# mjq11302010044/TATT

Measured on AMD Instinct MI355X. Metric: LR images/s (train fwd+bwd+clip+Adam) at 16x64->32x128, higher is better.
Workload: dtype fp32 (split-bf16 MFMA operands in conv3 / conv3-wgrad / conv9 / tokgemm / gru-wgrad / query-GRU recurrence and dW_hh / TP-layer backward)

## Files before the change

include/tatt_hip.h:

```cpp
#ifndef TATT_HIP_H
#define TATT_HIP_H

#ifdef __cplusplus
extern "C" {
#endif

typedef struct ihipStream_t* hipStream_t;


int tatt_gemm(const float* A, long sam, long sak, const float* A2, long sa2m, long sa2k, int K1,
              const float* B, long sbk, long sbn, const float* bias, float* C, long scm, long scn,
              int M, int N, int K, int Z, long bsA, long bsA2, long bsB, long bsC, long bsBias,
              float alpha, float beta, int act, int splitk, float* ws, float* rowsum, hipStream_t st);

int tatt_conv2d_fwd(const float* x, long xsn, long xsh, long xsw, long xsc, const float* wpacked,
                    const float* bias, float* y, long ldy, int Bn, int H, int W, int Cin, int Cout,
                    int KH, int KW, int act, float beta, int splitk, float* ws, hipStream_t st);

int tatt_conv2d_fwd_partials(const float* x, long xsn, long xsh, long xsw, long xsc, const float* wpacked, int Bn, int H,
                             int W, int Cin, int Cout, int KH, int KW, int splitk, float* ws, int* splits, hipStream_t st);

int tatt_conv2d_wgrad(const float* x, long xsn, long xsh, long xsw, long xsc, const float* dy,
                      long lddy, float* dw_oihw, int Bn, int H, int W, int Cin, int Cout, int KH,
                      int KW, float beta, int splitk, float* ws, hipStream_t st);

int tatt_repack_conv_weight(const float* w_oihw, float* out, int Cout, int Cin, int KH, int KW,
                            int mode, hipStream_t st);
int tatt_repack_words(int Cout, int Cin, int KH, int KW, int mode);
int tatt_repack_conv_weight_batch(const float* const* ws, float* const* outs, const int* dims, int n, hipStream_t st);

int tatt_gru_wgrad_sb(const float* dgi, const float* dgh, const float* x, const float* xb, const float* hprev,
                      float* ws1, float* ws2, int M, int G, hipStream_t st);

int tatt_splitk_reduce(const float* partial, float* C, int M, int N, int S, int remap_cin, int remap_taps,
                       float beta, float* vec, int vec_len, hipStream_t st);
int tatt_reduce_defer(int on, hipStream_t st);
int tatt_reduce_flush(hipStream_t st);

int tatt_conv3_c64_fwd_t(const float* x, const float* wt, const float* bias, float* y, int B, int H, int W, int Cin,
                         int Cout, int act, float beta, hipStream_t st);
int tatt_conv3_c64_fwd_ws16(const float* x, const float* wl, const float* bias, float* y, int B, int H, int W,
                            int Cout, int act, float beta, hipStream_t st);
int tatt_conv3_c64_fwd_ws16_bn(const float* x, const float* wl, const float* bias, float* y, int B, int H, int W,
                               int Cout, int act, float beta, const float* in_scale, const float* in_shift, int in_act,
                               double* stats, hipStream_t st);
int tatt_conv3_c64_fwd_sb(const float* x, int cin_total, int ci0, const float* wl, const float* bias, float* y, int B, int H,
                          int W, int Cout, int act, float beta, const float* in_scale, const float* in_shift, int in_act,
                          double* stats, hipStream_t st);
int tatt_conv3_c64_dgrad_bn_sb(const float* x, const float* x2, const float* in_scale, const float* in_scale2,
                               const float* in_shift, const float* wl, float* y, int B, int H, int W, const float* ep_x,
                               const float* ep_mean, const float* ep_rstd, const float* ep_gamma, const float* ep_beta,
                               int ep_act, double* stats, hipStream_t st);
int tatt_conv3_sb_generation(int gen);
int tatt_conv3_sb_packing(int B, int H, int W, int cin_total, int Cout, int act, int ep_act);
int tatt_conv3_sb_route(int B, int H, int W, int cin_total, int Cout, int act, int ep_act);
int tatt_conv3_c64_wgrad_partial(const float* x, const float* dy, float* part, float* pdb, int B, int H, int W,
                                 int Cin, int Cout, int G, hipStream_t st);
int tatt_conv3_c64_wgrad_partial_sb(const float* x, const float* dy, float* part, float* pdb, int B, int H, int W,
                                    int Cin, int Cout, int G, hipStream_t st);
int tatt_conv3_wgrad_sb_generation(int gen);
int tatt_conv3_wgrad_sb_route(int B, int H, int W, int Cin, int Cout);

int tatt_conv9_c64_to_c4(const float* x, const float* wpacked, const float* bias, float* y, int B, int H, int W,
                         int C, hipStream_t st);
int tatt_conv9_c64_to_c4_mfma(const float* x, const float* wt, const float* bias, float* y, int B, int H, int W,
                              hipStream_t st);
int tatt_conv9_c64_to_c4_sb(const float* x, const float* wt, const float* bias, float* y, int B, int H, int W,
                            hipStream_t st);
int tatt_conv9_c4_to_c64(const float* in, const float* wp, const float* bias, float* out, int B, int H, int W, int act,
                         hipStream_t st);
int tatt_conv9_c4_to_c64_sb(const float* in, const float* wp, const float* bias, float* out, int B, int H, int W, int act,
                            hipStream_t st);
int tatt_conv9_c64_c4_wgrad(const float* x, const float* dy, float* dw, float* part, int B, int H, int W,
                            hipStream_t st);
int tatt_conv9_c4_c64_wgrad(const float* x, const float* dy, float* dw, float* part, int B, int H, int W,
                            hipStream_t st);
int tatt_conv9_c64_c4_wgrad_sb(const float* x, const float* dy, float* dw, float* part, int B, int H, int W,
                               hipStream_t st);
int tatt_conv9_c4_c64_wgrad_sb(const float* x, const float* dy, float* dw, float* part, int B, int H, int W,
                               hipStream_t st);


int tatt_colsum(const float* X, long ld, int M, int C, float* out, float scale, float beta,
                double* ws, hipStream_t st);

int tatt_bn_stats(const float* X, long ld, int M, int C, float eps, float momentum, float* mean,
                  float* rstd, float* running_mean, float* running_var, double* ws, hipStream_t st);
int tatt_bn_stats_finish(const double* part, int G, int C, int M, float eps, float momentum, const float* gamma,
                         const float* beta, float* mean, float* rstd, float* running_mean, float* running_var, float* scale,
                         float* shift, hipStream_t st);
int tatt_bn_rstd(const float* var, float* rstd, int C, float eps, hipStream_t st);
int tatt_bn_apply(const float* X, long ldx, float* Y, long ldy, int M, int C, const float* mean,
                  const float* rstd, const float* gamma, const float* beta, int act, hipStream_t st);
int tatt_bn_bwd(const float* X, long ldx, const float* dY, long lddy, float* dX, long lddx, int M, int C,
                const float* mean, const float* rstd, const float* gamma, const float* beta, int act,
                int training, float* dgamma, float* dbeta, float* sums, double* ws, hipStream_t st);
int tatt_bn_bwd_groups(int M);
int tatt_bn_bwd_partials(const float* X, long ldx, const float* dY, long lddy, int M, int C, const float* mean,
                         const float* rstd, const float* gamma, const float* beta, int act, double* part, hipStream_t st);
int tatt_bn_bwd_finish(const double* part, int G, int C, int M, const float* mean, const float* rstd, const float* gamma,
                       float* dgamma, float* dbeta, float* coef, hipStream_t st);
int tatt_bn_bwd_affine(const float* X, const float* dU, float* dX, int M, int C, const float* coef, hipStream_t st);

int tatt_ln_fwd(const float* A, const float* Bres, float* Y, float* stats, int M, int C,
                const float* gamma, const float* beta, float eps, int mode, float pdrop,
                const unsigned long long* seed, unsigned site, hipStream_t st);
int tatt_ln_bwd(const float* A, const float* Bres, const float* dY, const float* stats, float* dX, float* dB, int M,
                int C, const float* gamma, float* dgamma, float* dbeta, float* part, double* ws, float eps, int mode,
                float pdrop, const unsigned long long* seed, unsigned site, hipStream_t st);


int tatt_prelu_fwd(const float* x, float* y, const float* alpha, long n, hipStream_t st);
int tatt_prelu_bwd(const float* x, const float* dy, float* dx, const float* alpha, long n, float* part,
                   hipStream_t st);
int tatt_act_fwd(const float* x, float* y, long n, int act, hipStream_t st);
int tatt_act_bwd(const float* ref, const float* dy, float* dx, long n, int act, int from_output,
                 hipStream_t st);
int tatt_axpby(const float* a, const float* b, float* y, float alpha, float beta, long n, hipStream_t st);
int tatt_add_n(const float* const* srcs, int n, float* y, long numel, hipStream_t st);
int tatt_add_rowbcast(const float* a, const float* b, float* y, long rows, int C, long period,
                      hipStream_t st);
int tatt_pixel_shuffle_fwd(const float* in, float* out, int B, int H, int W, int C, int act,
                           hipStream_t st);
int tatt_pixel_shuffle_bwd(const float* in, const float* dout, float* din, int B, int H, int W, int C,
                           int act, hipStream_t st);
int tatt_maxpool_fwd(const float* in, float* out, int B, int H, int W, int C, int kh, int kw, int sh, int sw,
                     int ph, int pw, hipStream_t st);
int tatt_maxpool_bwd(const float* in, const float* dout, float* din, int B, int H, int W, int C, int kh,
                     int kw, int sh, int sw, int ph, int pw, hipStream_t st);
int tatt_dropout(const float* x, float* y, long n, float p, const unsigned long long* seed, unsigned site,
                 hipStream_t st);
int tatt_bump_seed(unsigned long long* seed, unsigned long long* snap, hipStream_t st);
int tatt_stamp(unsigned long long* out, hipStream_t st);
int tatt_copy4d(const float* src, float* dst, int n0, int n1, int n2, int n3, long s0, long s1, long s2,
                long s3, long d0, long d1, long d2, long d3, float beta, hipStream_t st);


int tatt_l2norm(const float* g, long n, float* out, double* ws, hipStream_t st);
int tatt_adam_step(float* p, const float* g, float* m, float* v, long n, float lr, float b1, float b2,
                   float eps, const float* gnorm, float max_norm, float gscale, const long long* step,
                   hipStream_t st);


int tatt_gru32_fwd(const float* gi, const float* whh_f, const float* bhh_f, const float* whh_r,
                   const float* bhh_r, float* out, float* gates, int nseq, int T, int s_in, long stride_hi,
                   long stride_lo, long stride_t, hipStream_t st);
int tatt_gru32_bwd(const float* gates, const float* out, const float* dout, const float* whh_f,
                   const float* whh_r, float* dgi, float* dgh, float* hprev, int nseq, int T, int s_in,
                   long stride_hi, long stride_lo, long stride_t, hipStream_t st);

int tatt_gru32_fwd2(const float* gi, const float* whh_f, const float* bhh_f, const float* whh_r,
                    const float* bhh_r, float* out, float* gates, int nseq, int T, int s_in, long stride_hi,
                    long stride_lo, long stride_t, hipStream_t st);
int tatt_gru32_bwd2(const float* gates, const float* out, const float* dout, const float* whh_f,
                    const float* whh_r, float* dgi, float* dgh, float* hprev, float* frag, int nseq, int T, int s_in,
                    long stride_hi, long stride_lo, long stride_t, hipStream_t st);
int tatt_gru_wgrad_frag(const float* frag, const float* x, const float* xb, float* ws1, float* ws2, int nseq, int T,
                        int s_in, long stride_hi, long stride_lo, long stride_t, int G, hipStream_t st);
int tatt_gru_wgrad_frag_in(const float* frag, const float* x, const float* xb, float* ws1, float* ws2, int nseq, int T,
                           int s_in, long stride_hi, long stride_lo, long stride_t, int G, const float* in_mean,
                           const float* in_rstd, const float* in_gamma, const float* in_beta, const float* in_add,
                           hipStream_t st);

int tatt_qgru_bwd_fused(const float* dgh_cur0, const float* dgh_cur1, const float* whhT0, const float* whhT1,
                        const float* dhseq_next0, const float* dhseq_next1, const float* gsave_next0,
                        const float* gsave_next1, const float* hprev_next0, const float* hprev_next1,
                        float* dhcarry0, float* dhcarry1, float* dgi_acc0, float* dgi_acc1, float* dgh_next0,
                        float* dgh_next1, int Wb, int HID, hipStream_t st);

int tatt_gru_compose(const float* wih_f, const float* wih_r, const float* bih_f, const float* bih_r,
                     const float* Wc, const float* bc, float* Wp, float* bp, int K, hipStream_t st);
int tatt_gru_compose_batch(const float* const* ptrs, const int* Ks, int n, hipStream_t st);
int tatt_gru_tail(const float* dWp, const float* dbp, const float* Wc, const float* bc, const float* wih_f,
                  const float* wih_r, float* dwih_f, float* dwih_r, float* dWc, float* dbc, int K,
                  const float* dWhh, float* dwhh_f, float* dwhh_r, hipStream_t st);

int tatt_gru_tail_c(const float* dWp, const float* dbp, const float* Wc, const float* bc, const float* wih_f,
                    const float* wih_r, float* dwih_f, float* dwih_r, float* dWc, float* dbc, int K,
                    const float* dWhh_c, float* dwhh_f, float* dwhh_r, hipStream_t st);

int tatt_qgru_fwd_step(const float* gi0, const float* gi1, const float* whh0, const float* whh1,
                       const float* bhh0, const float* bhh1, const float* hprev0, const float* hprev1,
                       float* hnew0, float* hnew1, float* gsave0, float* gsave1, int Wb, int HID,
                       hipStream_t st);
// ... 290 lines not shown
```

tatt_amd/csrc/conv3.hip:

```cpp
#include "common.h"
#include <mutex>
#include <stdlib.h>
#include <type_traits>

#define C3_PX 64
#define C3_HW 66

struct Conv3P {
    const float* x; const float* w; const float* bias; float* y;
    int B, H, W, Cin, Cout, act;
    float beta;
    const float* in_scale; const float* in_shift; int in_act;
    double* stats;
};
template <int CK>
struct C5 {
    static constexpr int XP = CK + 4;
    static constexpr int HALO = 3 * C3_HW * XP;
    static constexpr int WT = 64 * XP;
    static constexpr int LDS = (2 * HALO + 2 * WT) * 4;
    static constexpr int Q4 = CK / 4;
    static constexpr int SLICE = 22 * Q4;
    static constexpr int WF4 = 64 * Q4;
};
template <int CK>
__global__ __launch_bounds__(256, (CK == 64 ? 1 : (CK == 32 ? 2 : 3))) void conv3_c64_fwd_v5_kernel(Conv3P p) {
    constexpr int C5_XP = C5<CK>::XP, C5_HALO = C5<CK>::HALO, C5_WT = C5<CK>::WT, Q4 = C5<CK>::Q4;
    constexpr int SLICE = C5<CK>::SLICE, WF4 = C5<CK>::WF4, QS = (CK == 64 ? 4 : 5);
    constexpr int Q4S = (CK == 64 ? 4 : (CK == 32 ? 3 : 2));
    (void)QS;
    extern __shared__ __attribute__((aligned(16))) float smem[];
    float* XsB = smem;
    float* WsB = smem + 2 * C5_HALO;
    const int t = threadIdx.x, lane = t & 63, wave = t >> 6;
    const int wm = wave & 1, wn = wave >> 1;
    const int segs = p.W / C3_PX, cob = p.Cout / 64, nch = p.Cin / CK;
    const int ntiles = p.B * p.H * segs * cob;
    const int G = gridDim.x;
    auto decode = [&](int tile, int& n, int& h, int& w0, int& co0) {
        int bid = tile;
        const int cb = bid % cob; bid /= cob;
        const int seg = bid % segs; bid /= segs;
        h = bid % p.H; n = bid / p.H;
        w0 = seg * C3_PX; co0 = cb * 64;
    };
    auto halo_load = [&](int n, int hh, int w0, int ci0, int pxb, int idx) -> f32x4 {
        const int ww = w0 + pxb + (idx >> Q4S) - 1;
        f32x4 v = (f32x4){0.f, 0.f, 0.f, 0.f};
        if (hh >= 0 && hh < p.H && ww >= 0 && ww < p.W)
            v = *reinterpret_cast<const f32x4*>(p.x + (((long)n * p.H + hh) * p.W + ww) * p.Cin + ci0 + 4 * (idx & (Q4 - 1)));
        return v;
    };
    auto halo_store = [&](float* Xs, int r, int pxb, int idx, f32x4 v) {
        *reinterpret_cast<f32x4*>(Xs + (r * C3_HW + pxb + (idx >> Q4S)) * C5_XP + 4 * (idx & (Q4 - 1))) = v;
    };
    constexpr int WQ = WF4 / 256;
    f32x4 wreg[WQ];
    auto load_w = [&](int tap, int ci0, int co0) {
        const float* src = p.w + ((long)tap * p.Cout + co0) * p.Cin + ci0;
#pragma unroll
        for (int q = 0; q < WQ; ++q) {
            const int idx = t + 256 * q;
            wreg[q] = *reinterpret_cast<const f32x4*>(src + (long)(idx >> Q4S) * p.Cin + 4 * (idx & (Q4 - 1)));
        }
    };
    auto store_w = [&](float* Ws) {
#pragma unroll
        for (int q = 0; q < WQ; ++q) {
            const int idx = t + 256 * q;
            *reinterpret_cast<f32x4*>(Ws + (idx >> Q4S) * C5_XP + 4 * (idx & (Q4 - 1))) = wreg[q];
        }
    };
    int tile = blockIdx.x;
    if (tile >= ntiles) return;
    int n, h, w0, co0;
    decode(tile, n, h, w0, co0);
    for (int s9 = 0; s9 < 9; ++s9) {
        const int r = s9 / 3, pxb = (s9 - 3 * r) * 22;
        for (int i = t; i < SLICE; i += 256) halo_store(XsB, r, pxb, i, halo_load(n, h + r - 1, w0, 0, pxb, i));
    }
    load_w(0, 0, co0);
    store_w(WsB);
    __syncthreads();
// ... 637 lines not shown
        unsigned nnorg, nnte;
        decode(pt + 2 * stride, nnorg, nnte);
#pragma unroll
        for (int st = 0; st < 18; ++st) {
            if (st + 1 < 18) { S3_LD(st + 1) }
            if (FIRST && st % 2 == 0 && st / 2 + 3 < 9) w_issue(st / 2 + 3);
            __builtin_amdgcn_sched_barrier(0);
            const bf16x8 wh = __builtin_bit_cast(bf16x8, wq[2 * st]), wl = __builtin_bit_cast(bf16x8, wq[2 * st + 1]);
            const bf16x8 b0h = __builtin_bit_cast(bf16x8, vb[st % 2][0]), b0l = __builtin_bit_cast(bf16x8, vb[st % 2][1]);
            const bf16x8 b1h = __builtin_bit_cast(bf16x8, vb[st % 2][2]), b1l = __builtin_bit_cast(bf16x8, vb[st % 2][3]);
            accM[0] = __builtin_amdgcn_mfma_f32_32x32x16_bf16(wh, b0h, accM[0], 0, 0, 0);
            accM[1] = __builtin_amdgcn_mfma_f32_32x32x16_bf16(wh, b1h, accM[1], 0, 0, 0);
            accC[0] = __builtin_amdgcn_mfma_f32_32x32x16_bf16(wl, b0h, accC[0], 0, 0, 0);
            accC[1] = __builtin_amdgcn_mfma_f32_32x32x16_bf16(wl, b1h, accC[1], 0, 0, 0);
            accC[0] = __builtin_amdgcn_mfma_f32_32x32x16_bf16(wh, b0l, accC[0], 0, 0, 0);
            accC[1] = __builtin_amdgcn_mfma_f32_32x32x16_bf16(wh, b1l, accC[1], 0, 0, 0);
            if (st % 2 == 1 && st / 2 < S3_NIT) {
                halo_put(imgN, nte, st / 2);
                halo_issue1(nnorg, nnte, had_next && pt + 2 * stride < npt, st / 2);
                S3_INTERLEAVE(INMODE == 1 ? 14 : 8)
            }
            if (st % 4 == 2 && st / 4 < S3_NEP) { epilogue(epi_pending, st / 4); S3_INTERLEAVE(8) }
            if (st % 4 == 0 && st > 0 && st / 4 - 1 < S3_NEP) epi_request(org, st / 4 - 1);
            __builtin_amdgcn_sched_barrier(0);
        }
#if S2_STAMP
        { const unsigned long long now = __builtin_amdgcn_s_memtime();
          if (tix == 0) ts[3] = now; else if (tix == 1) ts[6] = now; else if (tix == 2) ts[9] = now; }
#endif
        has_next = had_next && pt + 2 * stride < npt;
        {
            unsigned* xw = XCH + xbuf * S2_XCH + (kh * 64 + lj) * S2_XP + 32 * coh + 4 * kb;
#pragma unroll
            for (int pp = 0; pp < 2; ++pp)
#pragma unroll
                for (int g = 0; g < 4; ++g) {
                    f32x4 v;
#pragma unroll
                    for (int r = 0; r < 4; ++r) v[r] = accM[pp][4 * g + r] + accC[pp][4 * g + r];
                    *reinterpret_cast<f32x4*>(xw + 32 * pp * S2_XP + 8 * g) = v;
                }
        }
        eorg = org; ebuf = xbuf; epi_pending = true;
#if S2_STAMP
        { const unsigned long long now = __builtin_amdgcn_s_memtime();
          if (tix == 0) ts[4] = now; else if (tix == 1) ts[7] = now; else if (tix == 2) ts[10] = now; }
        ++tix;
#endif
        __syncthreads();
        if (had_next) { pt += stride; org = norg; te = nte; norg = nnorg; nte = nnte; xbuf ^= 1; }
    };
    tile_body(std::true_type{});
    while (had_next) tile_body(std::false_type{});
    S2_STAMP_AT(11)
#pragma unroll
    for (int e = 0; e < S3_NEP; ++e) epilogue(true, e);
    S2_STAMP_AT(12)
#if S2_STAMP
    ts[31] = wall_clock64();
    if (lane == 0 && sbuf) {
#pragma unroll
        for (int i = 0; i < 32; ++i) sbuf[(blockIdx.x * 8 + wave) * 32 + i] = ts[i];
    }
#endif
    if (p.stats) {
#pragma unroll
        for (int r = 0; r < 4; ++r) {
            st_s[r] += __shfl_xor(st_s[r], 16, 64); st_s[r] += __shfl_xor(st_s[r], 32, 64);
            st_q[r] += __shfl_xor(st_q[r], 16, 64); st_q[r] += __shfl_xor(st_q[r], 32, 64);
        }
        if (lane < 16) {
#pragma unroll
            for (int r = 0; r < 4; ++r) { st_red[wave][0][ec4 + r] = st_s[r]; st_red[wave][1][ec4 + r] = st_q[r]; }
        }
        __syncthreads();
        if (t < 128) {
            double a = 0.0;
#pragma unroll
            for (int w = 0; w < 4; ++w) a += (double)st_red[w][t >> 6][t & 63];
            p.stats[(long)blockIdx.x * 128 + t] = a;
        }
    }
}
template <int INMODE, bool EPBN>
__global__ __launch_bounds__(512, 2) void conv3_c64_sb4_kernel(Conv3SB q) {
    const Conv3P& p = q.c;
    extern __shared__ __attribute__((aligned(16))) unsigned smem_u[];
    unsigned* const XCH = smem_u + 4 * S3_IMG;
    const unsigned t = threadIdx.x, lane = t & 63, wave = t >> 6;
    const unsigned W = p.W, H = p.H, tws = (W + 15) / 16, ths = H / 4, cob = p.Cout / 64;
    const unsigned npt = p.B * ths * tws;
    const unsigned stride = gridDim.x / cob;
    unsigned cb = blockIdx.x % cob, pt = blockIdx.x / cob;
    if (gridDim.x % 8 == 0 && 8 % cob == 0 && stride % (8 / cob) == 0) {
        const unsigned x = blockIdx.x & 7, m = blockIdx.x >> 3, xg = 8 / cob;
        cb = x % cob;
        pt = (x / cob) * (stride / xg) + m;
    }
    __shared__ float st_red[4][2][64];
    __shared__ __attribute__((aligned(16))) float cst[7][64];
    __shared__ __attribute__((aligned(16))) float cbias[64];
    if (pt >= npt) {
        if (p.stats && t < 128) p.stats[(long)blockIdx.x * 128 + t] = 0.0;
        return;
    }
    const unsigned ntile = (npt - pt + stride - 1) / stride;
    auto decode = [&](unsigned tile, unsigned& org, unsigned& te) {
        const unsigned tw = tile % tws; tile /= tws;
        const unsigned th = tile % ths, n = tile / ths;
        org = (n * H + th * 4) * W + tw * 16;
        const unsigned cin = min(18u, W - tw * 16 + 1);
        te = (th == 0 ? 1u : 0u) | (th == ths - 1 ? 2u : 0u) | (tw == 0 ? 4u : 0u) | (cin << 8);
    };
    if (wave >= 4) {
        const unsigned h = t - 256;
        const unsigned npix = p.B * H * W;
        const __amdgpu_buffer_rsrc_t rs_x = __builtin_amdgcn_make_buffer_rsrc(const_cast<float*>(p.x), 0, npix * q.cin_total * 4, 0x00020000);
        const __amdgpu_buffer_rsrc_t rs_x2 = __builtin_amdgcn_make_buffer_rsrc(const_cast<float*>(INMODE == 2 ? q.x2 : p.x), 0, npix * 256, 0x00020000);
        const __amdgpu_buffer_rsrc_t rs_y = __builtin_amdgcn_make_buffer_rsrc(p.y, 0, npix * p.Cout * 4, 0x00020000);
        const __amdgpu_buffer_rsrc_t rs_e = __builtin_amdgcn_make_buffer_rsrc(const_cast<float*>(EPBN ? q.ep_x : p.y), 0, npix * (EPBN ? 64 : p.Cout) * 4, 0x00020000);
        const bool in_relu = p.in_act == ACT_RELU;
        const unsigned xps = q.cin_total * 4, yps = p.Cout * 4, eps_ = EPBN ? 256u : yps;
        unsigned boff[S3_NIT], poff[S3_NIT], edge[2] = {0, 0}, colk[2] = {0, 0};
#pragma unroll
        for (int k = 0; k < S3_NIT; ++k) {
            const unsigned pix = (h >> 4) + 16 * k, r = pix / S2_HW, c = pix - r * S2_HW;
            boff[k] = (unsigned)(((int)r - 1) * (int)W + (int)c - 1) * xps + (q.ci0 + 4 * (h & 15)) * 4;
            poff[k] = r * S3_RP + c * SB_PW + 2 * (h & 15);
            edge[k >> 2] |= ((r == 0 ? 1u : 0u) | (r == 5 ? 2u : 0u) | (c == 0 ? 4u : 0u) | (pix >= S2_NPX ? 8u : 0u)) << (8 * (k & 3));
            colk[k >> 2] |= c << (8 * (k & 3));
        }
        auto outside = [&](int k, unsigned te) -> bool {
            return (((edge[k >> 2] >> (8 * (k & 3))) & (te | 8u) & 15u) != 0) || (((colk[k >> 2] >> (8 * (k & 3))) & 255u) >= (te >> 8));
        };
        f32x4 hp[S3_NIT], hp2[S3_NIT];
        auto halo_issue = [&](unsigned tile, bool valid) {
            unsigned org, te;
            decode(tile, org, te);
#if S2_DEBUG
            if (s2_wrep & 4) valid = false;
#endif
#pragma unroll
            for (int k = 0; k < S3_NIT; ++k) {
                const unsigned a = (org * xps + boff[k]) | (outside(k, te) ? S2_OOB : (valid ? 0u : S2_OOB));
                hp[k] = s2_ld(rs_x, a);
                if (INMODE == 2) hp2[k] = s2_ld(rs_x2, a);
            }
        };
        auto halo_put = [&](unsigned* img, unsigned tile) {
            unsigned org, te;
            decode(tile, org, te);
            f32x4 isc, ish, isc2;
            if (INMODE != 0) { isc = *reinterpret_cast<const f32x4*>(&cst[0][4 * (h & 15)]); ish = *reinterpret_cast<const f32x4*>(&cst[1][4 * (h & 15)]); }
            if (INMODE == 2) isc2 = *reinterpret_cast<const f32x4*>(&cst[2][4 * (h & 15)]);
#pragma unroll
            for (int k = 0; k < S3_NIT; ++k) {
                const bool ok = !outside(k, te);
                f32x4 v = hp[k];
                if (INMODE == 2) {
#pragma unroll
                    for (int e = 0; e < 4; ++e) v[e] = fmaf(v[e], isc[e], fmaf(hp2[k][e], isc2[e], ish[e]));
                } else if (INMODE == 1) {
#pragma unroll
                    for (int e = 0; e < 4; ++e) v[e] = mish_f(fmaf(v[e], isc[e], ish[e]));
                } else if (INMODE == 3) {
#pragma unroll
                    for (int e = 0; e < 4; ++e) {
                        const float u = fmaf(v[e], isc[e], ish[e]);
                        v[e] = in_relu ? fmaxf(u, 0.f) : u;
                    }
                }
                if (INMODE != 0) {
#pragma unroll
                    for (int e = 0; e < 4; ++e) v[e] = ok ? v[e] : 0.f;
                }
                if (k < S3_NIT - 1 || h < S2_NPX * 16 - 256 * (S3_NIT - 1)) {
                    uint2 hi, lo;
                    sb_split(v, hi, lo);
                    unsigned* d = img + poff[k];
                    *reinterpret_cast<uint2*>(d) = hi;
                    *reinterpret_cast<uint2*>(d + S3_IMG) = lo;
                }
            }
        };
        halo_issue(pt, true);
// ... 6 lines not shown
        __syncthreads();
        halo_put(smem_u, pt);
        halo_issue(pt + stride, ntile > 1);
        __syncthreads();
        const bool use_beta = p.beta != 0.f, out_relu = p.act == ACT_RELU;
        const bool ep_mish = q.ep_act == ACT_MISH, ep_relu = q.ep_act == ACT_RELU;
        const unsigned ecol = h >> 4, ec4 = 4 * (h & 15);
        f32x4 epx[S3_NEP], st_s = (f32x4){0.f, 0.f, 0.f, 0.f}, st_q = st_s;
        auto epi_request = [&](unsigned tile) {
            unsigned org, te;
            decode(tile, org, te);
            const bool in_map = ecol + 1 < (te >> 8);
#pragma unroll
            for (int e = 0; e < S3_NEP; ++e)
                epx[e] = s2_ld(rs_e, ((org + e * W + ecol) * eps_ + (cb * 64 + ec4) * 4) | (((EPBN || use_beta) && in_map) ? 0u : S2_OOB));
        };
        auto epilogue = [&](unsigned tile, unsigned xb) {
            unsigned org, te;
            decode(tile, org, te);
            const f32x4 bj = *reinterpret_cast<const f32x4*>(&cbias[ec4]);
            const bool in_map = ecol + 1 < (te >> 8);
            f32x4 ep_mu, ep_rs, ep_g, ep_b;
            if (EPBN) {
                ep_mu = *reinterpret_cast<const f32x4*>(&cst[3][ec4]); ep_rs = *reinterpret_cast<const f32x4*>(&cst[4][ec4]);
                ep_g = *reinterpret_cast<const f32x4*>(&cst[5][ec4]); ep_b = *reinterpret_cast<const f32x4*>(&cst[6][ec4]);
            }
#pragma unroll
            for (int e = 0; e < S3_NEP; ++e) {
                const unsigned* X = XCH + xb * S2_XCH + ((h >> 4) + 16 * e) * S2_XP + ec4;
                const f32x4 v0 = *reinterpret_cast<const f32x4*>(X), v1 = *reinterpret_cast<const f32x4*>(X + 64 * S2_XP);
                f32x4 v;
#pragma unroll
                for (int r = 0; r < 4; ++r) {
                    v[r] = (v0[r] + v1[r]) + bj[r];
                    if (EPBN) {
                        const float xh = (epx[e][r] - ep_mu[r]) * ep_rs[r], u = fmaf(ep_g[r], xh, ep_b[r]);
                        const float g = ep_mish ? mish_grad_f(u) : 1.f;
                        v[r] *= ep_relu ? (u > 0.f ? 1.f : 0.f) : g;
                        v[r] = in_map ? v[r] : 0.f;
                        st_s[r] += v[r]; st_q[r] += v[r] * xh;
                    } else {
                        v[r] = fmaf(p.beta, epx[e][r], v[r]);
                        v[r] = out_relu ? fmaxf(v[r], 0.f) : v[r];
                        v[r] = in_map ? v[r] : 0.f;
                        st_s[r] += v[r]; st_q[r] += v[r] * v[r];
                    }
                }
#if S2_DEBUG
                if (s2_wrep & 8) continue;
#endif
                __builtin_amdgcn_raw_buffer_store_b128(__builtin_bit_cast(u32x4_s2, v), rs_y, ((org + e * W + ecol) * yps + (cb * 64 + ec4) * 4) | (in_map ? 0u : S2_OOB), 0, 0);
            }
        };
        for (unsigned i = 0; i < ntile; ++i) {
            const unsigned tile = pt + i * stride;
#if S2_DEBUG
            if (s2_wrep & 1) { __syncthreads(); continue; }
#endif
#if S2_DEBUG
            if (!(s2_wrep & 32))
#endif
            if (i > 0) epilogue(tile - stride, (i - 1) & 1);
#if S2_DEBUG
            if (!(s2_wrep & 16))
#endif
            if (i + 1 < ntile) halo_put(smem_u + ((i + 1) & 1) * 2 * S3_IMG, tile + stride);
            halo_issue(tile + 2 * stride, i + 2 < ntile);
            epi_request(tile);
            __syncthreads();
        }
        epilogue(pt + (ntile - 1) * stride, (ntile - 1) & 1);
        if (p.stats) {
#pragma unroll
            for (int r = 0; r < 4; ++r) {
                st_s[r] += __shfl_xor(st_s[r], 16, 64); st_s[r] += __shfl_xor(st_s[r], 32, 64);
                st_q[r] += __shfl_xor(st_q[r], 16, 64); st_q[r] += __shfl_xor(st_q[r], 32, 64);
            }
            if (lane < 16) {
#pragma unroll
                for (int r = 0; r < 4; ++r) { st_red[wave - 4][0][ec4 + r] = st_s[r]; st_red[wave - 4][1][ec4 + r] = st_q[r]; }
            }
        }
        __syncthreads();
        if (p.stats && h < 128) {
            double a = 0.0;
#pragma unroll
            for (int w = 0; w < 4; ++w) a += (double)st_red[w][h >> 6][h & 63];
            p.stats[(long)blockIdx.x * 128 + h] = a;
        }
        return;
    }
    const unsigned coh = wave & 1, kh = wave >> 1, lj = lane & 31, kb = lane >> 5;
    f32x4 wq[36];
    {
        const f32x4* const wsrc = reinterpret_cast<const f32x4*>(p.w) + (cb * 2 + coh) * 72 * 64 + lane;
#pragma unroll
        for (int tap = 0; tap < 9; ++tap)
#pragma unroll
            for (int f = 0; f < 4; ++f) wq[4 * tap + f] = wsrc[((tap * 2 + kh) * 4 + f) * 64];
    }
    const unsigned bbase = (lj >> 4) * S3_RP + (lj & 15) * SB_PW + 16 * kh + 4 * kb;
    __syncthreads();
    __syncthreads();
    for (unsigned i = 0; i < ntile; ++i) {
#if S2_DEBUG
        if (s2_wrep & 2) { __syncthreads(); continue; }
#endif
        const unsigned* Xs = smem_u + (i & 1) * 2 * S3_IMG + bbase;
        f32x16_s3 acc[2];
#pragma unroll
        for (int pp = 0; pp < 2; ++pp)
#pragma unroll
            for (int v = 0; v < 16; ++v) acc[pp][v] = 0.f;
        f32x4 vb[2][4];
        S3_LD(0)
#pragma unroll
        for (int st = 0; st < 18; ++st) {
            if (st + 1 < 18) { S3_LD(st + 1) }
            __builtin_amdgcn_sched_barrier(0);
            const bf16x8 wh = __builtin_bit_cast(bf16x8, wq[2 * st]), wl = __builtin_bit_cast(bf16x8, wq[2 * st + 1]);
            const bf16x8 b0h = __builtin_bit_cast(bf16x8, vb[st % 2][0]), b0l = __builtin_bit_cast(bf16x8, vb[st % 2][1]);
            const bf16x8 b1h = __builtin_bit_cast(bf16x8, vb[st % 2][2]), b1l = __builtin_bit_cast(bf16x8, vb[st % 2][3]);
            acc[0] = __builtin_amdgcn_mfma_f32_32x32x16_bf16(wh, b0h, acc[0], 0, 0, 0);
            acc[1] = __builtin_amdgcn_mfma_f32_32x32x16_bf16(wh, b1h, acc[1], 0, 0, 0);
            acc[0] = __builtin_amdgcn_mfma_f32_32x32x16_bf16(wl, b0h, acc[0], 0, 0, 0);
            acc[1] = __builtin_amdgcn_mfma_f32_32x32x16_bf16(wl, b1h, acc[1], 0, 0, 0);
            acc[0] = __builtin_amdgcn_mfma_f32_32x32x16_bf16(wh, b0l, acc[0], 0, 0, 0);
            acc[1] = __builtin_amdgcn_mfma_f32_32x32x16_bf16(wh, b1l, acc[1], 0, 0, 0);
            __builtin_amdgcn_sched_barrier(0);
        }
        unsigned* xw = XCH + (i & 1) * S2_XCH + (kh * 64 + lj) * S2_XP + 32 * coh + 4 * kb;
#pragma unroll
        for (int pp = 0; pp < 2; ++pp)
#pragma unroll
            for (int g = 0; g < 4; ++g) {
                f32x4 v;
#pragma unroll
                for (int r = 0; r < 4; ++r) v[r] = acc[pp][4 * g + r];
                *reinterpret_cast<f32x4*>(xw + 32 * pp * S2_XP + 8 * g) = v;
            }
        __syncthreads();
    }
    __syncthreads();
}
static int conv3_sb_generation = 4;
TATT_API int tatt_conv3_sb_generation(int gen) {
    const int old = conv3_sb_generation;
    if (gen == 1 || gen == 3 || gen == 4) conv3_sb_generation = gen;
    return old;
}
template <int INMODE, bool EPBN>
static void conv3_sb4_go(const Conv3SB& q, dim3 grid, hipStream_t st) {
    static TattPerDevice attr_once;
    tatt_per_device(attr_once, [&] {
        (void)hipFuncSetAttribute(reinterpret_cast<const void*>(conv3_c64_sb4_kernel<INMODE, EPBN>), hipFuncAttributeMaxDynamicSharedMemorySize, S3_LDS);
    });
    hipLaunchKernelGGL((conv3_c64_sb4_kernel<INMODE, EPBN>), grid, dim3(512), S3_LDS, st, q);
}
template <int INMODE, bool EPBN>
static void conv3_sb3_go(const Conv3SB& q, dim3 grid, hipStream_t st) {
    static TattPerDevice attr_once;
    tatt_per_device(attr_once, [&] {
        (void)hipFuncSetAttribute(reinterpret_cast<const void*>(conv3_c64_sb3_kernel<INMODE, EPBN>), hipFuncAttributeMaxDynamicSharedMemorySize, S3_LDS);
    });
    hipLaunchKernelGGL((conv3_c64_sb3_kernel<INMODE, EPBN>), grid, dim3(256), S3_LDS, st, q);
}
static int conv3_sb_pick(int B, int H, int W, int cin_total, int Cout, int act, int ep_act) {
    const long maxb = (long)B * H * W * (cin_total > Cout ? cin_total : Cout) * 4;
    if (conv3_sb_generation < 3 || H % 4 || maxb >= 0x7fffffffL || ep_act == ACT_TANH) return 1;
    if (conv3_sb_generation == 4 && (act == ACT_NONE || (act == ACT_RELU && ep_act == ACT_NONE))) return 4;
    return (conv3_sb_generation == 3 && W % 16 == 0 && act == ACT_NONE) ? 3 : 1;
}
TATT_API int tatt_conv3_sb_packing(int B, int H, int W, int cin_total, int Cout, int act, int ep_act) {
    return conv3_sb_pick(B, H, W, cin_total, Cout, act, ep_act) >= 3 ? 14 : 10;
}
TATT_API int tatt_conv3_sb_route(int B, int H, int W, int cin_total, int Cout, int act, int ep_act) {
    const int pick = conv3_sb_pick(B, H, W, cin_total, Cout, act, ep_act);
    return pick == 1 && W % C3_PX ? 0 : pick;
}
static int conv3_sb_launch(const Conv3SB& q, hipStream_t st) {
    const Conv3P& p = q.c;
    const int pick = conv3_sb_pick(p.B, p.H, p.W, q.cin_total, p.Cout, p.act, q.ep_act);
    if (pick >= 3) {
        const int cob = p.Cout / 64, npt = p.B * (p.H / 4) * ((p.W + 15) / 16);
        int per = 256 / cob;
        if (per > npt) per = npt;
        const dim3 grid(per * cob);
        const bool ep = q.ep_x != nullptr;
        const int inmode = q.x2 ? 2 : (p.in_scale ? (p.in_act == ACT_MISH ? 1 : 3) : 0);
        if (pick == 4) {
            if (inmode == 2) { if (ep) conv3_sb4_go<2, true>(q, grid, st); else conv3_sb4_go<2, false>(q, grid, st); }
            else if (inmode == 1) { if (ep) conv3_sb4_go<1, true>(q, grid, st); else conv3_sb4_go<1, false>(q, grid, st); }
            else if (inmode == 3) { if (ep) conv3_sb4_go<3, true>(q, grid, st); else conv3_sb4_go<3, false>(q, grid, st); }
            else { if (ep) conv3_sb4_go<0, true>(q, grid, st); else conv3_sb4_go<0, false>(q, grid, st); }
            return LAUNCH_CHECK();
        }
        if (pick == 3) {
            if (inmode == 2) { if (ep) conv3_sb3_go<2, true>(q, grid, st); else conv3_sb3_go<2, false>(q, grid, st); }
            else if (inmode == 1) { if (ep) conv3_sb3_go<1, true>(q, grid, st); else conv3_sb3_go<1, false>(q, grid, st); }
            else if (inmode == 3) { if (ep) conv3_sb3_go<3, true>(q, grid, st); else conv3_sb3_go<3, false>(q, grid, st); }
            else { if (ep) conv3_sb3_go<0, true>(q, grid, st); else conv3_sb3_go<0, false>(q, grid, st); }
            return LAUNCH_CHECK();
        }
        return LAUNCH_CHECK();
    }
    if (p.W % C3_PX) return 1;
    static TattPerDevice attr_once;
    tatt_per_device(attr_once, [&] {
        (void)hipFuncSetAttribute(reinterpret_cast<const void*>(conv3_c64_sb_kernel<false, false>), hipFuncAttributeMaxDynamicSharedMemorySize, SB_LDS);
        (void)hipFuncSetAttribute(reinterpret_cast<const void*>(conv3_c64_sb_kernel<true, false>), hipFuncAttributeMaxDynamicSharedMemorySize, SB_LDS);
        (void)hipFuncSetAttribute(reinterpret_cast<const void*>(conv3_c64_sb_kernel<false, true>), hipFuncAttributeMaxDynamicSharedMemorySize, SB_LDS);
        (void)hipFuncSetAttribute(reinterpret_cast<const void*>(conv3_c64_sb_kernel<true, true>), hipFuncAttributeMaxDynamicSharedMemorySize, SB_LDS);
    });
    const int cob = p.Cout / 64, npt = p.B * p.H * (p.W / C3_PX);
    int per = 256 / cob;
    if (per > npt) per = npt;
    const dim3 grid(per * cob), block(512);
    const bool in2 = q.x2 != nullptr, ep = q.ep_x != nullptr;
    if (in2 && ep) hipLaunchKernelGGL((conv3_c64_sb_kernel<true, true>), grid, block, SB_LDS, st, q);
    else if (in2) hipLaunchKernelGGL((conv3_c64_sb_kernel<true, false>), grid, block, SB_LDS, st, q);
    else if (ep) hipLaunchKernelGGL((conv3_c64_sb_kernel<false, true>), grid, block, SB_LDS, st, q);
    else hipLaunchKernelGGL((conv3_c64_sb_kernel<false, false>), grid, block, SB_LDS, st, q);
    return LAUNCH_CHECK();
}
TATT_API int tatt_conv3_c64_fwd_sb(const float* x, int cin_total, int ci0, const float* wl, const float* bias, float* y, int B, int H,
                                   int W, int Cout, int act, float beta, const float* in_scale, const float* in_shift, int in_act,
                                   double* stats, hipStream_t st) {
    if (Cout % 64 || cin_total % 4 || ci0 % 4 || ci0 + 64 > cin_total) return 1;
    if (stats && (Cout != 64 || act != ACT_NONE || beta != 0.f)) return 2;
    if (in_scale && (!in_shift || in_act == ACT_TANH)) return 3;
    Conv3SB q = {{x, wl, bias, y, B, H, W, 64, Cout, act, beta, in_scale, in_shift, in_act, stats}, cin_total, ci0,
                 nullptr, nullptr, nullptr, nullptr, nullptr, nullptr, nullptr, 0};
    return conv3_sb_launch(q, st);
}
TATT_API int tatt_conv3_c64_dgrad_bn_sb(const float* x, const float* x2, const float* in_scale, const float* in_scale2,
                                        const float* in_shift, const float* wl, float* y, int B, int H, int W, const float* ep_x,
                                        const float* ep_mean, const float* ep_rstd, const float* ep_gamma, const float* ep_beta,
                                        int ep_act, double* stats, hipStream_t st) {
    if (x2 && (!in_scale || !in_scale2 || !in_shift)) return 2;
    if (ep_x && (!ep_mean || !ep_rstd || !ep_gamma || !ep_beta || !stats)) return 3;
    if (!ep_x && stats) return 4;
    Conv3SB q = {{x, wl, nullptr, y, B, H, W, 64, 64, ACT_NONE, 0.f, x2 ? in_scale : nullptr, x2 ? in_shift : nullptr, ACT_NONE, stats}, 64, 0,
                 x2, in_scale2, ep_x, ep_mean, ep_rstd, ep_gamma, ep_beta, ep_act};
    return conv3_sb_launch(q, st);
}

struct Conv3WP {
    const float* x; const float* dy; float* part;
    int B, H, W, Cin, Cout, nseg;
    float* pdb;
};
#define WG_HALO (3 * C3_HW * 64)
#define WG_BUF (WG_HALO + 64 * 64)
#define C3_WG_LDS (2 * WG_BUF * 4)
#define WG_F4 (WG_BUF / 4)

template <int T0, int NT>
__device__ __forceinline__ void wgrad_segment(f32x16 (&acc)[5], const float* __restrict__ acol, const float* __restrict__ bcol,
                                              const Conv3WP& p, bool has_next, int nn, int nh, int nw0, int ci0, int co0,
                                              float* __restrict__ nbuf, int t, float& dbacc) {
    auto fetch = [&](int idx) -> f32x4 {
        f32x4 v = (f32x4){0.f, 0.f, 0.f, 0.f};
        if (idx < WG_HALO / 4) {
            const int c4 = idx & 15, pp = idx >> 4;
            const int r = pp / C3_HW, px = pp - r * C3_HW;
            const int hh = nh + r - 1, ww = nw0 + px - 1;
            if (hh >= 0 && hh < p.H && ww >= 0 && ww < p.W)
                v = *reinterpret_cast<const f32x4*>(p.x + (((long)nn * p.H + hh) * p.W + ww) * p.Cin + ci0 + 4 * c4);
        } else if (idx < WG_F4) {
            const int j = idx - WG_HALO / 4, c4 = j & 15, px = j >> 4;
            v = *reinterpret_cast<const f32x4*>(p.dy + (((long)nn * p.H + nh) * p.W + nw0 + px) * p.Cout + co0 + 4 * c4);
        }
        return v;
    };
    float wa[2][NT], wb[2];
    f32x4 pf = (f32x4){0.f, 0.f, 0.f, 0.f};
#define C3W_LOAD(buf, k)                                                                   \
    wb[buf] = bcol[(k) * 64];                                                              \
    _Pragma("unroll") for (int tp = 0; tp < NT; ++tp)                                      \
        wa[buf][tp] = acol[(((T0 + tp) / 3) * C3_HW + (k) + ((T0 + tp) % 3)) * 64];
    C3W_LOAD(0, 0)
    __builtin_amdgcn_sched_barrier(0);
#pragma unroll
    for (int k = 0; k < 64; k += 2) {
        const int cur = (k >> 1) & 1;
        if (k + 2 < 64) { C3W_LOAD(cur ^ 1, k + 2) }
        if (has_next && k % 6 == 0 && k / 6 < 9) pf = fetch(t + 512 * (k / 6));
        __builtin_amdgcn_sched_barrier(0);
#pragma unroll
        for (int tp = 0; tp < NT; ++tp)
            acc[tp] = __builtin_amdgcn_mfma_f32_32x32x2f32(wa[cur][tp], wb[cur], acc[tp], 0, 0, 0);
        if (T0 == 0) dbacc += wb[cur];
        __builtin_amdgcn_sched_barrier(0);
        if (has_next && k % 6 == 4 && k / 6 < 9) {
            const int idx = t + 512 * (k / 6);
            if (idx < WG_F4) *reinterpret_cast<f32x4*>(nbuf + 4 * idx) = pf;
        }
    }
#undef C3W_LOAD
}

#define WS_TP 36
#define WS_TT (32 * WS_TP)
__global__ __launch_bounds__(512, 1) void conv3_c64_wgrad_kernel(Conv3WP p) {
    extern __shared__ __attribute__((aligned(16))) float smem[];
    const int t = threadIdx.x, lane = t & 63, wave = t >> 6;
    const int qi = wave & 1, qo = (wave >> 1) & 1, tg = wave >> 2;
    const int cib = blockIdx.y % (p.Cin / 64), cob = blockIdx.y / (p.Cin / 64);
    const int ci0 = cib * 64, co0 = cob * 64;
    const int segs = p.W / C3_PX;
    f32x16 acc[5];
#pragma unroll
    for (int a = 0; a < 5; ++a)
#pragma unroll
        for (int i = 0; i < 16; ++i) acc[a][i] = 0.f;
    auto decode = [&](int s, int& n, int& h, int& w0) {
// ... 91 lines not shown
```

tatt_amd/csrc/norm.hip:

```cpp
#include "common.h"

#define CS_MAXG 256

template <typename T>
__global__ __launch_bounds__(256) void colsum_stage1(const T* __restrict__ X, long ld, int M, int C, int rpb,
                                                     double* __restrict__ part) {
    __shared__ double sh[4][64];
    const int tx = threadIdx.x & 63, ty = threadIdx.x >> 6;
    const int m_begin = blockIdx.x * rpb;
    const int m_end = min(M, m_begin + rpb);
    for (int c0 = 0; c0 < C; c0 += 64) {
        const int c = c0 + tx;
        double s0 = 0.0;
        if (c < C && m_begin + ty < m_end)
            s0 = sum_strided<T, 8>(X + (long)(m_begin + ty) * ld + c, (m_end - m_begin - ty + 3) / 4, 4 * ld);
        sh[ty][tx] = s0;
        __syncthreads();
        if (ty == 0 && c < C) part[(long)blockIdx.x * C + c] = (sh[0][tx] + sh[1][tx]) + (sh[2][tx] + sh[3][tx]);
        __syncthreads();
    }
}
#define S2_L 16
__device__ __forceinline__ double s2_combine(double (*sh)[64], int tx) {
    double s = 0.0;
#pragma unroll
    for (int l = 0; l < S2_L; l += 4) s += (sh[l][tx] + sh[l + 1][tx]) + (sh[l + 2][tx] + sh[l + 3][tx]);
    return s;
}
__global__ __launch_bounds__(64 * S2_L) void colsum_stage2(const double* __restrict__ part, int G, int C, long ldp,
                                                           float* __restrict__ out, float scale, float beta) {
    __shared__ double sh[S2_L][64];
    const int tx = threadIdx.x & 63, ty = threadIdx.x >> 6;
    const int c = blockIdx.x * 64 + tx;
    double s = 0.0;
    if (c < C && ty < G) s = sum_strided<double, 8>(part + (long)ty * ldp + c, (G - ty + S2_L - 1) / S2_L, S2_L * ldp);
    sh[ty][tx] = s;
    __syncthreads();
    if (ty == 0 && c < C) {
        float v = (float)(s2_combine(sh, tx) * scale);
        out[c] = beta != 0.f ? v + beta * out[c] : v;
    }
}
#define V4_U 12
static inline bool v4_ok(const void* p, long ld, int C) {
    return C % 4 == 0 && C <= 1024 && ld % 4 == 0 && (((uintptr_t)p) & 15) == 0 && (256 % (C / 4) == 0 || (C / 4) % 256 == 0);
}
template <typename F>
__device__ __forceinline__ void v4_rows(const float* __restrict__ X, long ld, int m_begin, int m_end, int rl, int rpar, int c4,
                                        F&& f) {
    int m = m_begin + rl;
    for (; m + (V4_U - 1) * rpar < m_end; m += V4_U * rpar) {
        f32x4 v[V4_U];
#pragma unroll
        for (int u = 0; u < V4_U; ++u) v[u] = *reinterpret_cast<const f32x4*>(X + (long)(m + u * rpar) * ld + c4);
#pragma unroll
        for (int u = 0; u < V4_U; ++u) f(v[u]);
    }
    for (; m < m_end; m += rpar) f(*reinterpret_cast<const f32x4*>(X + (long)m * ld + c4));
}
template <typename F>
__device__ __forceinline__ void v4_rows2(const float* __restrict__ X, long ldx, const float* __restrict__ Y, long ldy,
                                         int m_begin, int m_end, int rl, int rpar, int c4, F&& f) {
    constexpr int U = V4_U / 2;
    int m = m_begin + rl;
    for (; m + (U - 1) * rpar < m_end; m += U * rpar) {
        f32x4 a[U], b[U];
#pragma unroll
        for (int u = 0; u < U; ++u) {
            a[u] = *reinterpret_cast<const f32x4*>(X + (long)(m + u * rpar) * ldx + c4);
            b[u] = *reinterpret_cast<const f32x4*>(Y + (long)(m + u * rpar) * ldy + c4);
        }
#pragma unroll
        for (int u = 0; u < U; ++u) f(a[u], b[u]);
    }
    for (; m < m_end; m += rpar)
        f(*reinterpret_cast<const f32x4*>(X + (long)m * ldx + c4), *reinterpret_cast<const f32x4*>(Y + (long)m * ldy + c4));
}
template <int NQ>
__device__ __forceinline__ void v4_block_partials(const double (&acc)[NQ][4], int C, int cv, int cl, int rl, int rpar,
                                                  int c_base, double* __restrict__ part, double* sh) {
    const int t = threadIdx.x;
#pragma unroll
    for (int q = 0; q < NQ; ++q)
#pragma unroll
        for (int e = 0; e < 4; ++e) sh[q * 1024 + rl * (4 * cv) + 4 * cl + e] = acc[q][e];
    __syncthreads();
    const int width = 4 * cv;
    for (int c = t; c < width; c += 256) {
#pragma unroll
        for (int q = 0; q < NQ; ++q) {
            double s = 0.0;
            for (int r = 0; r < rpar; ++r) s += sh[q * 1024 + r * width + c];
            part[((long)blockIdx.x * NQ + q) * C + c_base + c] = s;
        }
    }
    __syncthreads();
}
__global__ __launch_bounds__(256) void colsum_stage1_v4(const float* __restrict__ X, long ld, int M, int C, int rpb,
                                                        double* __restrict__ part) {
    __shared__ double sh[1024];
    const int t = threadIdx.x;
    const int cv = min(C >> 2, 256), rpar = 256 / cv, cl = t % cv, rl = t / cv;
    const int m_begin = blockIdx.x * rpb, m_end = min(M, m_begin + rpb);
    for (int c0 = 0; c0 < C; c0 += 4 * cv) {
        double acc[1][4] = {{0.0, 0.0, 0.0, 0.0}};
        v4_rows(X, ld, m_begin, m_end, rl, rpar, c0 + 4 * cl, [&](const f32x4& v) {
#pragma unroll
            for (int e = 0; e < 4; ++e) acc[0][e] += (double)v[e];
        });
        v4_block_partials<1>(acc, C, cv, cl, rl, rpar, c0, part, sh);
    }
}
static inline int cs_groups(int M) { int g = cdiv(M, 64); return g > CS_MAXG ? CS_MAXG : (g < 1 ? 1 : g); }
TATT_API int tatt_colsum(const float* X, long ld, int M, int C, float* out, float scale, float beta,
                         double* ws, hipStream_t st) {
    int G = cs_groups(M);
    int rpb = cdiv(M, G);
    if (v4_ok(X, ld, C)) hipLaunchKernelGGL(colsum_stage1_v4, dim3(G), dim3(256), 0, st, X, ld, M, C, rpb, ws);
    else hipLaunchKernelGGL((colsum_stage1<float>), dim3(G), dim3(256), 0, st, X, ld, M, C, rpb, ws);
    hipLaunchKernelGGL(colsum_stage2, dim3(cdiv(C, 64)), dim3(64 * S2_L), 0, st, ws, G, C, (long)C, out, scale, beta);
    return LAUNCH_CHECK();
}

__global__ void bn_stats_stage1(const float* __restrict__ X, long ld, int M, int C, int rows_per_block,
                                double* __restrict__ part) {
    __shared__ double sh[2][256];
    const int cpb = C < 256 ? C : 256;
    const int rpar = 256 / cpb;
    const int t = threadIdx.x;
    const int cl = t % cpb, rl = t / cpb;
    const int m_begin = blockIdx.x * rows_per_block;
    const int m_end = min(M, m_begin + rows_per_block);
    for (int c0 = 0; c0 < C; c0 += cpb) {
        const int c = c0 + cl;
        double s = 0.0, q = 0.0;
        if (rl < rpar && c < C) {
            int m = m_begin + rl;
            for (; m + 3 * rpar < m_end; m += 4 * rpar) {
                float v0 = X[(long)m * ld + c], v1 = X[(long)(m + rpar) * ld + c];
                float v2 = X[(long)(m + 2 * rpar) * ld + c], v3 = X[(long)(m + 3 * rpar) * ld + c];
                s += ((double)v0 + (double)v1) + ((double)v2 + (double)v3);
                q += ((double)v0 * v0 + (double)v1 * v1) + ((double)v2 * v2 + (double)v3 * v3);
            }
            for (; m < m_end; m += rpar) { double v = (double)X[(long)m * ld + c]; s += v; q += v * v; }
        }
        sh[0][t] = s; sh[1][t] = q;
        __syncthreads();
        if (t < cpb && c < C) {
            double ss = 0.0, qq = 0.0;
            for (int r = 0; r < rpar; ++r) { ss += sh[0][r * cpb + t]; qq += sh[1][r * cpb + t]; }
            part[((long)blockIdx.x * 2 + 0) * C + c] = ss;
            part[((long)blockIdx.x * 2 + 1) * C + c] = qq;
        }
        __syncthreads();
    }
}
__global__ __launch_bounds__(256) void bn_stats_stage1_v4(const float* __restrict__ X, long ld, int M, int C, int rpb,
                                                          double* __restrict__ part) {
    __shared__ double sh[2 * 1024];
    const int t = threadIdx.x;
    const int cv = min(C >> 2, 256), rpar = 256 / cv, cl = t % cv, rl = t / cv;
    const int m_begin = blockIdx.x * rpb, m_end = min(M, m_begin + rpb);
    for (int c0 = 0; c0 < C; c0 += 4 * cv) {
        double acc[2][4] = {{0.0, 0.0, 0.0, 0.0}, {0.0, 0.0, 0.0, 0.0}};
        v4_rows(X, ld, m_begin, m_end, rl, rpar, c0 + 4 * cl, [&](const f32x4& v) {
#pragma unroll
            for (int e = 0; e < 4; ++e) { const double d = (double)v[e]; acc[0][e] += d; acc[1][e] += d * d; }
        });
        v4_block_partials<2>(acc, C, cv, cl, rl, rpar, c0, part, sh);
    }
}
__global__ __launch_bounds__(64 * S2_L) void bn_stats_stage2(const double* __restrict__ part, int G, int C, int M, float eps,
                                                             float momentum, float* __restrict__ mean, float* __restrict__ rstd,
                                                             float* __restrict__ running_mean, float* __restrict__ running_var,
                                                             const float* __restrict__ gamma = nullptr,
                                                             const float* __restrict__ beta = nullptr,
                                                             float* __restrict__ scale = nullptr, float* __restrict__ shift = nullptr) {
    __shared__ double sh[2][S2_L][64];
    const int tx = threadIdx.x & 63, ty = threadIdx.x >> 6;
    const int c = blockIdx.x * 64 + tx;
    double s = 0.0, q = 0.0;
    if (c < C && ty < G) {
        s = sum_strided<double, 8>(part + ((long)ty * 2 + 0) * C + c, (G - ty + S2_L - 1) / S2_L, (long)2 * S2_L * C);
        q = sum_strided<double, 8>(part + ((long)ty * 2 + 1) * C + c, (G - ty + S2_L - 1) / S2_L, (long)2 * S2_L * C);
    }
    sh[0][ty][tx] = s; sh[1][ty][tx] = q;
    __syncthreads();
    if (ty != 0 || c >= C) return;
    s = s2_combine(sh[0], tx);
    q = s2_combine(sh[1], tx);
    double mu = s / M;
    double var = q / M - mu * mu;
    if (var < 0.0) var = 0.0;
    mean[c] = (float)mu;
    rstd[c] = (float)(1.0 / sqrt(var + (double)eps));
    if (scale) {
        const float sc = gamma[c] * rstd[c];
        scale[c] = sc;
        shift[c] = beta[c] - mean[c] * sc;
    }
    if (running_mean) {
        double unb = M > 1 ? var * ((double)M / (M - 1)) : var;
        running_mean[c] = (float)((1.0 - momentum) * running_mean[c] + momentum * mu);
        running_var[c] = (float)((1.0 - momentum) * running_var[c] + momentum * unb);
    }
}
TATT_API int tatt_bn_stats(const float* X, long ld, int M, int C, float eps, float momentum, float* mean,
                           float* rstd, float* running_mean, float* running_var, double* ws, hipStream_t st) {
    int G = cs_groups(M);
    int rpb = cdiv(M, G);
    if (v4_ok(X, ld, C)) hipLaunchKernelGGL(bn_stats_stage1_v4, dim3(G), dim3(256), 0, st, X, ld, M, C, rpb, ws);
    else hipLaunchKernelGGL(bn_stats_stage1, dim3(G), dim3(256), 0, st, X, ld, M, C, rpb, ws);
    hipLaunchKernelGGL(bn_stats_stage2, dim3(cdiv(C, 64)), dim3(64 * S2_L), 0, st, ws, G, C, M, eps, momentum, mean, rstd,
                       running_mean, running_var);
    return LAUNCH_CHECK();
}
TATT_API int tatt_bn_stats_finish(const double* part, int G, int C, int M, float eps, float momentum, const float* gamma,
                                  const float* beta, float* mean, float* rstd, float* running_mean, float* running_var,
                                  float* scale, float* shift, hipStream_t st) {
    if (scale && (!gamma || !beta || !shift)) return 1;
    hipLaunchKernelGGL(bn_stats_stage2, dim3(cdiv(C, 64)), dim3(64 * S2_L), 0, st, part, G, C, M, eps, momentum, mean, rstd,
                       running_mean, running_var, gamma, beta, scale, shift);
    return LAUNCH_CHECK();
}
__global__ void bn_rstd_kernel(const float* __restrict__ var, float* __restrict__ rstd, int C, float eps) {
    int c = blockIdx.x * blockDim.x + threadIdx.x;
    if (c < C) rstd[c] = 1.f / sqrtf(var[c] + eps);
}
TATT_API int tatt_bn_rstd(const float* var, float* rstd, int C, float eps, hipStream_t st) {
    hipLaunchKernelGGL(bn_rstd_kernel, dim3(cdiv(C, 64)), dim3(64), 0, st, var, rstd, C, eps);
    return LAUNCH_CHECK();
}

__global__ void bn_apply_kernel(const float* __restrict__ X, long ldx, float* __restrict__ Y, long ldy, int M, int C,
                                const float* __restrict__ mean, const float* __restrict__ rstd,
                                const float* __restrict__ gamma, const float* __restrict__ beta, int act) {
    long idx = (long)blockIdx.x * blockDim.x + threadIdx.x;
    long total = (long)M * C;
    if (idx >= total) return;
    int c = idx % C;
    long m = idx / C;
    float u = (X[m * ldx + c] - mean[c]) * rstd[c] * gamma[c] + beta[c];
    Y[m * ldy + c] = apply_act(u, act);
}
#define BA_R 4
__global__ __launch_bounds__(256) void bn_apply_v4_kernel(const float* __restrict__ X, long ldx, float* __restrict__ Y, long ldy,
                                                          int M, int C, const float* __restrict__ mean,
                                                          const float* __restrict__ rstd, const float* __restrict__ gamma,
                                                          const float* __restrict__ beta, int act) {
    const int cv = C >> 2;
    const long idx = (long)blockIdx.x * 256 + threadIdx.x;
    const int c4 = (int)(idx % cv) * 4;
    const long m0 = (idx / cv) * BA_R;
    if (m0 >= M) return;
    const f32x4 mu = *reinterpret_cast<const f32x4*>(mean + c4), rs = *reinterpret_cast<const f32x4*>(rstd + c4);
    const f32x4 g = *reinterpret_cast<const f32x4*>(gamma + c4), b = *reinterpret_cast<const f32x4*>(beta + c4);
    f32x4 v[BA_R];
#pragma unroll
    for (int r = 0; r < BA_R; ++r) v[r] = *reinterpret_cast<const f32x4*>(X + min(m0 + r, (long)M - 1) * ldx + c4);
#pragma unroll
    for (int r = 0; r < BA_R; ++r) {
        if (m0 + r >= M) break;
        f32x4 o;
#pragma unroll
        for (int e = 0; e < 4; ++e) o[e] = apply_act((v[r][e] - mu[e]) * rs[e] * g[e] + b[e], act);
        *reinterpret_cast<f32x4*>(Y + (m0 + r) * ldy + c4) = o;
    }
}
TATT_API int tatt_bn_apply(const float* X, long ldx, float* Y, long ldy, int M, int C, const float* mean,
                           const float* rstd, const float* gamma, const float* beta, int act, hipStream_t st) {
    long total = (long)M * C;
    if (C % 4 == 0 && ldx % 4 == 0 && ldy % 4 == 0 && !((((uintptr_t)X) | ((uintptr_t)Y) | ((uintptr_t)mean) | ((uintptr_t)rstd) |
                                                          ((uintptr_t)gamma) | ((uintptr_t)beta)) & 15)) {
        const long items = (long)cdiv(M, BA_R) * (C / 4);
        hipLaunchKernelGGL(bn_apply_v4_kernel, dim3(cdiv(items, 256)), dim3(256), 0, st, X, ldx, Y, ldy, M, C, mean, rstd, gamma,
                           beta, act);
        return LAUNCH_CHECK();
    }
    hipLaunchKernelGGL(bn_apply_kernel, dim3(cdiv(total, 256)), dim3(256), 0, st, X, ldx, Y, ldy, M, C, mean, rstd,
                       gamma, beta, act);
    return LAUNCH_CHECK();
}

__global__ void bn_bwd_stage1(const float* __restrict__ X, long ldx, const float* __restrict__ dY, long lddy, int M,
                              int C, int rows_per_block, const float* __restrict__ mean,
                              const float* __restrict__ rstd, const float* __restrict__ gamma,
                              const float* __restrict__ beta, int act, double* __restrict__ part) {
    __shared__ double sh[2][256];
    const int cpb = C < 256 ? C : 256;
    const int rpar = 256 / cpb;
    const int t = threadIdx.x;
    const int cl = t % cpb, rl = t / cpb;
    const int m_begin = blockIdx.x * rows_per_block;
    const int m_end = min(M, m_begin + rows_per_block);
    for (int c0 = 0; c0 < C; c0 += cpb) {
        const int c = c0 + cl;
        double s = 0.0, q = 0.0;
        if (rl < rpar && c < C) {
            const float mu = mean[c], rs = rstd[c], g = gamma[c], b = beta[c];
            int m = m_begin + rl;
            for (; m + 3 * rpar < m_end; m += 4 * rpar) {
                float xv[4], dv[4];
#pragma unroll
                for (int u = 0; u < 4; ++u) { xv[u] = X[(long)(m + u * rpar) * ldx + c]; dv[u] = dY[(long)(m + u * rpar) * lddy + c]; }
#pragma unroll
                for (int u = 0; u < 4; ++u) {
                    float xh = (xv[u] - mu) * rs;
                    float du = dv[u];
                    if (act != ACT_NONE) du *= act_grad(g * xh + b, act);
                    s += (double)du; q += (double)du * xh;
                }
            }
            for (; m < m_end; m += rpar) {
                float xh = (X[(long)m * ldx + c] - mu) * rs;
                float du = dY[(long)m * lddy + c];
                if (act != ACT_NONE) du *= act_grad(g * xh + b, act);
                s += (double)du; q += (double)du * xh;
            }
        }
        sh[0][t] = s; sh[1][t] = q;
        __syncthreads();
        if (t < cpb && c < C) {
            double ss = 0.0, qq = 0.0;
            for (int r = 0; r < rpar; ++r) { ss += sh[0][r * cpb + t]; qq += sh[1][r * cpb + t]; }
            part[((long)blockIdx.x * 2 + 0) * C + c] = ss;
            part[((long)blockIdx.x * 2 + 1) * C + c] = qq;
        }
        __syncthreads();
    }
}
__global__ __launch_bounds__(256) void bn_bwd_stage1_v4(const float* __restrict__ X, long ldx, const float* __restrict__ dY,
                                                        long lddy, int M, int C, int rpb, const float* __restrict__ mean,
                                                        const float* __restrict__ rstd, const float* __restrict__ gamma,
                                                        const float* __restrict__ beta, int act, double* __restrict__ part) {
    __shared__ double sh[2 * 1024];
    const int t = threadIdx.x;
    const int cv = min(C >> 2, 256), rpar = 256 / cv, cl = t % cv, rl = t / cv;
    const int m_begin = blockIdx.x * rpb, m_end = min(M, m_begin + rpb);
    for (int c0 = 0; c0 < C; c0 += 4 * cv) {
        const int c4 = c0 + 4 * cl;
        const f32x4 mu = *reinterpret_cast<const f32x4*>(mean + c4), rs = *reinterpret_cast<const f32x4*>(rstd + c4);
        const f32x4 g = *reinterpret_cast<const f32x4*>(gamma + c4), b = *reinterpret_cast<const f32x4*>(beta + c4);
        double acc[2][4] = {{0.0, 0.0, 0.0, 0.0}, {0.0, 0.0, 0.0, 0.0}};
        v4_rows2(X, ldx, dY, lddy, m_begin, m_end, rl, rpar, c4, [&](const f32x4& xv, const f32x4& dv) {
#pragma unroll
            for (int e = 0; e < 4; ++e) {
                const float xh = (xv[e] - mu[e]) * rs[e];
                float du = dv[e];
                if (act != ACT_NONE) du *= act_grad(g[e] * xh + b[e], act);
                acc[0][e] += (double)du; acc[1][e] += (double)du * xh;
            }
        });
        v4_block_partials<2>(acc, C, cv, cl, rl, rpar, c0, part, sh);
    }
}
__global__ __launch_bounds__(64 * S2_L) void bn_bwd_stage2(const double* __restrict__ part, int G, int C,
                                                           float* __restrict__ dgamma, float* __restrict__ dbeta,
                                                           float* __restrict__ sums) {
    __shared__ double sh[2][S2_L][64];
    const int tx = threadIdx.x & 63, ty = threadIdx.x >> 6;
    const int c = blockIdx.x * 64 + tx;
    double s = 0.0, q = 0.0;
    if (c < C && ty < G) {
        s = sum_strided<double, 8>(part + ((long)ty * 2 + 0) * C + c, (G - ty + S2_L - 1) / S2_L, (long)2 * S2_L * C);
        q = sum_strided<double, 8>(part + ((long)ty * 2 + 1) * C + c, (G - ty + S2_L - 1) / S2_L, (long)2 * S2_L * C);
    }
    sh[0][ty][tx] = s; sh[1][ty][tx] = q;
    __syncthreads();
    if (ty != 0 || c >= C) return;
    s = s2_combine(sh[0], tx);
    q = s2_combine(sh[1], tx);
    dbeta[c] = (float)s; dgamma[c] = (float)q;
    sums[c] = (float)s; sums[C + c] = (float)q;
}
__global__ void bn_bwd_apply_kernel(const float* __restrict__ X, long ldx, const float* __restrict__ dY, long lddy,
                                    float* __restrict__ dX, long lddx, int M, int C,
                                    const float* __restrict__ mean, const float* __restrict__ rstd,
                                    const float* __restrict__ gamma, const float* __restrict__ beta, int act,
                                    const float* __restrict__ sums, int training) {
    long idx = (long)blockIdx.x * blockDim.x + threadIdx.x;
    long total = (long)M * C;
    if (idx >= total) return;
    int c = idx % C;
    long m = idx / C;
    float rs = rstd[c], g = gamma[c];
    float xh = (X[m * ldx + c] - mean[c]) * rs;
    float du = dY[m * lddy + c];
    if (act != ACT_NONE) du *= act_grad(g * xh + beta[c], act);
    float v = du;
    if (training) {
        float inv = 1.f / (float)M;
        v = du - sums[c] * inv - xh * sums[C + c] * inv;
    }
    dX[m * lddx + c] = g * rs * v;
}
__global__ __launch_bounds__(256) void bn_bwd_apply_v4_kernel(const float* __restrict__ X, long ldx, const float* __restrict__ dY,
                                                              long lddy, float* __restrict__ dX, long lddx, int M, int C,
                                                              const float* __restrict__ mean, const float* __restrict__ rstd,
                                                              const float* __restrict__ gamma, const float* __restrict__ beta,
                                                              int act, const float* __restrict__ sums, int training) {
    const int cv = C >> 2;
    const long idx = (long)blockIdx.x * 256 + threadIdx.x;
    const int c4 = (int)(idx % cv) * 4;
    const long m0 = (idx / cv) * BA_R;
    if (m0 >= M) return;
    const f32x4 mu = *reinterpret_cast<const f32x4*>(mean + c4), rs = *reinterpret_cast<const f32x4*>(rstd + c4);
    const f32x4 g = *reinterpret_cast<const f32x4*>(gamma + c4), b = *reinterpret_cast<const f32x4*>(beta + c4);
    const f32x4 s1 = *reinterpret_cast<const f32x4*>(sums + c4), s2 = *reinterpret_cast<const f32x4*>(sums + C + c4);
    const float inv = 1.f / (float)M;
    f32x4 xv[BA_R], dv[BA_R];
#pragma unroll
    for (int r = 0; r < BA_R; ++r) {
        const long m = min(m0 + r, (long)M - 1);
        xv[r] = *reinterpret_cast<const f32x4*>(X + m * ldx + c4);
        dv[r] = *reinterpret_cast<const f32x4*>(dY + m * lddy + c4);
    }
#pragma unroll
    for (int r = 0; r < BA_R; ++r) {
        if (m0 + r >= M) break;
        f32x4 o;
#pragma unroll
        for (int e = 0; e < 4; ++e) {
            const float xh = (xv[r][e] - mu[e]) * rs[e];
            float du = dv[r][e];
            if (act != ACT_NONE) du *= act_grad(g[e] * xh + b[e], act);
            float v = du;
            if (training) v = du - s1[e] * inv - xh * s2[e] * inv;
            o[e] = g[e] * rs[e] * v;
        }
        *reinterpret_cast<f32x4*>(dX + (m0 + r) * lddx + c4) = o;
    }
}
TATT_API int tatt_bn_bwd(const float* X, long ldx, const float* dY, long lddy, float* dX, long lddx, int M, int C,
                         const float* mean, const float* rstd, const float* gamma, const float* beta, int act,
                         int training, float* dgamma, float* dbeta, float* sums, double* ws, hipStream_t st) {
    int G = cs_groups(M);
    int rpb = cdiv(M, G);
    const bool v4 = v4_ok(X, ldx, C) && v4_ok(dY, lddy, C) && v4_ok(dX, lddx, C) &&
                    !((((uintptr_t)mean) | ((uintptr_t)rstd) | ((uintptr_t)gamma) | ((uintptr_t)beta) | ((uintptr_t)sums)) & 15);
    if (v4) hipLaunchKernelGGL(bn_bwd_stage1_v4, dim3(G), dim3(256), 0, st, X, ldx, dY, lddy, M, C, rpb, mean, rstd, gamma, beta,
                               act, ws);
    else hipLaunchKernelGGL(bn_bwd_stage1, dim3(G), dim3(256), 0, st, X, ldx, dY, lddy, M, C, rpb, mean, rstd, gamma, beta,
                            act, ws);
    hipLaunchKernelGGL(bn_bwd_stage2, dim3(cdiv(C, 64)), dim3(64 * S2_L), 0, st, ws, G, C, dgamma, dbeta, sums);
    if (v4) {
        const long items = (long)cdiv(M, BA_R) * (C / 4);
        hipLaunchKernelGGL(bn_bwd_apply_v4_kernel, dim3(cdiv(items, 256)), dim3(256), 0, st, X, ldx, dY, lddy, dX, lddx, M, C,
                           mean, rstd, gamma, beta, act, sums, training);
        return LAUNCH_CHECK();
    }
    long total = (long)M * C;
    hipLaunchKernelGGL(bn_bwd_apply_kernel, dim3(cdiv(total, 256)), dim3(256), 0, st, X, ldx, dY, lddy, dX, lddx, M, C,
                       mean, rstd, gamma, beta, act, sums, training);
    return LAUNCH_CHECK();
}

__global__ __launch_bounds__(64 * S2_L) void bn_bwd_finish_kernel(const double* __restrict__ part, int G, int C, int M,
                                                                  const float* __restrict__ mean, const float* __restrict__ rstd,
                                                                  const float* __restrict__ gamma, float* __restrict__ dgamma,
                                                                  float* __restrict__ dbeta, float* __restrict__ coef) {
    __shared__ double sh[2][S2_L][64];
    const int tx = threadIdx.x & 63, ty = threadIdx.x >> 6;
    const int c = blockIdx.x * 64 + tx;
    double s = 0.0, q = 0.0;
    if (c < C && ty < G) {
        s = sum_strided<double, 8>(part + ((long)ty * 2 + 0) * C + c, (G - ty + S2_L - 1) / S2_L, (long)2 * S2_L * C);
        q = sum_strided<double, 8>(part + ((long)ty * 2 + 1) * C + c, (G - ty + S2_L - 1) / S2_L, (long)2 * S2_L * C);
    }
    sh[0][ty][tx] = s; sh[1][ty][tx] = q;
    __syncthreads();
    if (ty != 0 || c >= C) return;
    s = s2_combine(sh[0], tx);
    q = s2_combine(sh[1], tx);
    dbeta[c] = (float)s; dgamma[c] = (float)q;
    const float inv = 1.f / (float)M, g = gamma[c], rs = rstd[c];
    const float a = g * rs;
    const float b = -a * rs * ((float)q * inv);
    coef[c] = a;
    coef[C + c] = b;
    coef[2 * C + c] = -a * ((float)s * inv) - b * mean[c];
}
TATT_API int tatt_bn_bwd_groups(int M) { return cs_groups(M); }
TATT_API int tatt_bn_bwd_partials(const float* X, long ldx, const float* dY, long lddy, int M, int C, const float* mean,
                                  const float* rstd, const float* gamma, const float* beta, int act, double* part, hipStream_t st) {
    const int G = cs_groups(M), rpb = cdiv(M, G);
    const bool v4 = v4_ok(X, ldx, C) && v4_ok(dY, lddy, C) &&
                    !((((uintptr_t)mean) | ((uintptr_t)rstd) | ((uintptr_t)gamma) | ((uintptr_t)beta)) & 15);
    if (v4) hipLaunchKernelGGL(bn_bwd_stage1_v4, dim3(G), dim3(256), 0, st, X, ldx, dY, lddy, M, C, rpb, mean, rstd, gamma, beta, act, part);
    else hipLaunchKernelGGL(bn_bwd_stage1, dim3(G), dim3(256), 0, st, X, ldx, dY, lddy, M, C, rpb, mean, rstd, gamma, beta, act, part);
    return LAUNCH_CHECK();
}
TATT_API int tatt_bn_bwd_finish(const double* part, int G, int C, int M, const float* mean, const float* rstd, const float* gamma,
                                float* dgamma, float* dbeta, float* coef, hipStream_t st) {
    hipLaunchKernelGGL(bn_bwd_finish_kernel, dim3(cdiv(C, 64)), dim3(64 * S2_L), 0, st, part, G, C, M, mean, rstd, gamma, dgamma, dbeta, coef);
    return LAUNCH_CHECK();
}
__global__ __launch_bounds__(256) void bn_bwd_affine_kernel(const float* __restrict__ X, const float* __restrict__ dU, float* __restrict__ dX,
                                                            long n4, int C, const float* __restrict__ coef) {
    const long i = (long)blockIdx.x * 256 + threadIdx.x;
    if (i >= n4) return;
    const int c4 = (int)(i % (C >> 2)) * 4;
    const f32x4 a = *reinterpret_cast<const f32x4*>(coef + c4), b = *reinterpret_cast<const f32x4*>(coef + C + c4);
    const f32x4 c = *reinterpret_cast<const f32x4*>(coef + 2 * C + c4);
    const f32x4 x = reinterpret_cast<const f32x4*>(X)[i], u = reinterpret_cast<const f32x4*>(dU)[i];
    f32x4 o;
#pragma unroll
    for (int e = 0; e < 4; ++e) o[e] = fmaf(a[e], u[e], fmaf(b[e], x[e], c[e]));
    reinterpret_cast<f32x4*>(dX)[i] = o;
}
TATT_API int tatt_bn_bwd_affine(const float* X, const float* dU, float* dX, int M, int C, const float* coef, hipStream_t st) {
    if (C % 4) return 1;
    const long n4 = (long)M * (C / 4);
    hipLaunchKernelGGL(bn_bwd_affine_kernel, dim3(cdiv(n4, 256)), dim3(256), 0, st, X, dU, dX, n4, C, coef);
    return LAUNCH_CHECK();
}

#define LN_MAXPER 4

__device__ __forceinline__ float ln_residual(const float* __restrict__ Bres, long idx, float pdrop, uint64_t seedv, unsigned site,
                                             uint32_t th) {
    const float b = Bres[idx];
    if (pdrop <= 0.f) return b;
    return dropout_keep(seedv, site, (uint64_t)idx, th) ? b * (1.f / (1.f - pdrop)) : 0.f;
}
__global__ void ln_fwd_kernel(const float* __restrict__ A, const float* __restrict__ Bres, float* __restrict__ Y,
                              float* __restrict__ stats, int M, int C, const float* __restrict__ gamma,
                              const float* __restrict__ beta, float eps, int mode, float pdrop,
                              const unsigned long long* __restrict__ seed, unsigned site) {
    const int lane = threadIdx.x & 63;
    const long row = (long)blockIdx.x * (blockDim.x >> 6) + (threadIdx.x >> 6);
    if (row >= M) return;
    const uint64_t seedv = pdrop > 0.f ? seed[0] : 0;
    const uint32_t th = dropout_thresh(pdrop);
    float v[LN_MAXPER];
    float s = 0.f;
#pragma unroll
    for (int k = 0; k < LN_MAXPER; ++k) {
        int c = lane + 64 * k;
        float x = 0.f;
        if (c < C) { x = A[row * C + c]; if (Bres) x += ln_residual(Bres, row * C + c, pdrop, seedv, site, th); }
        v[k] = x; s += x;
    }
    float mu = wave_sum(s) / C;
    float q = 0.f;
#pragma unroll
    for (int k = 0; k < LN_MAXPER; ++k) { int c = lane + 64 * k; if (c < C) { float d = v[k] - mu; q += d * d; } }
    const float ssq = wave_sum(q);
    float rs = mode == 0 ? 1.f / sqrtf(ssq / C + eps) : 1.f / (sqrtf(ssq / (C - 1)) + eps);
#pragma unroll
    for (int k = 0; k < LN_MAXPER; ++k) {
        int c = lane + 64 * k;
        if (c < C) Y[row * C + c] = (v[k] - mu) * rs * gamma[c] + beta[c];
    }
    if (lane == 0 && stats) { stats[row * 2] = mu; stats[row * 2 + 1] = rs; }
}
TATT_API int tatt_ln_fwd(const float* A, const float* Bres, float* Y, float* stats, int M, int C,
                         const float* gamma, const float* beta, float eps, int mode, float pdrop,
                         const unsigned long long* seed, unsigned site, hipStream_t st) {
    if (C > 64 * LN_MAXPER) return 1;
    if (pdrop > 0.f && (!Bres || !seed)) return 2;
    hipLaunchKernelGGL(ln_fwd_kernel, dim3(cdiv(M, 4)), dim3(256), 0, st, A, Bres, Y, stats, M, C, gamma, beta, eps, mode,
                       pdrop, seed, site);
    return LAUNCH_CHECK();
}

#define LN_BWD_ROWS 64
__global__ void ln_bwd_kernel(const float* __restrict__ A, const float* __restrict__ Bres,
                              const float* __restrict__ dY, const float* __restrict__ stats, float* __restrict__ dX,
                              float* __restrict__ dB, int M, int C, const float* __restrict__ gamma, float* __restrict__ part,
                              float eps, int mode, float pdrop, const unsigned long long* __restrict__ seed, unsigned site) {
    __shared__ float sh[4][2][64 * LN_MAXPER];
    const int lane = threadIdx.x & 63, wave = threadIdx.x >> 6;
// ... 123 lines not shown
```

tatt_amd/functional.py:

```python
from __future__ import annotations

import math
from typing import Optional

import weakref

import torch
from torch.autograd import Function

from . import ops
from .ops import ACT_NONE, ACT_RELU, ACT_MISH, ACT_TANH

_SEEDS = {}
_CUR_SEED = {}


def seed_tensor(device) -> torch.Tensor:
    key = str(device)
    if key not in _SEEDS:
        _SEEDS[key] = torch.tensor([0x1234ABCD5678EF01 & 0x7FFFFFFFFFFFFFFF], dtype=torch.int64, device=device)
    return _SEEDS[key]


def set_seed(device, value: int):
# ... 135 lines not shown


def _c(t):
    return t if t.is_contiguous() else t.contiguous()


class Conv2dFn(Function):

    @staticmethod
    def forward(ctx, x, weight, bias, act, any_width=False):
        Cout, Cin, KH, KW = weight.shape
        y = ops.conv2d_forward(x, weight, bias, act, any_width)
        ctx.save_for_backward(x, weight, y if act != ACT_NONE else None)
        ctx.act = act
        ctx.any_width = any_width
        ctx.has_bias = bias is not None
        ctx.leaves = (weight, bias)
        return y

    @staticmethod
    def backward(ctx, dy):
        x, weight, y = ctx.saved_tensors
        Cout, Cin, KH, KW = weight.shape
        dy = _c(dy)
        if ctx.act != ACT_NONE:
            dy = ops.act_bwd(y, dy, ctx.act, True)
        dx = None
        if ctx.needs_input_grad[0]:
            dx = ops.conv2d_dgrad(dy, weight, ctx.any_width)
        want_dw, want_db = ctx.needs_input_grad[1], ctx.has_bias and ctx.needs_input_grad[2]
        aw = ctx.any_width

        def param_grads():
            if want_dw and want_db:
                return ops.conv_wgrad(x, dy, Cout, KH, KW, want_db=True, any_width=aw)
            dw = ops.conv_wgrad(x, dy, Cout, KH, KW, any_width=aw) if want_dw else None
            db = ops.colsum(dy.reshape(-1, Cout)) if want_db else None
            return dw, db
        wleaf, bleaf = ctx.leaves
        if want_dw and want_db and SIDE.enabled and (SIDE.due_of.get(id(wleaf)) != SIDE.due_of.get(id(bleaf))
                                                     or (id(wleaf) in SIDE.immediate) != (id(bleaf) in SIDE.immediate)):
            (dw,) = SIDE.submit((wleaf,), lambda: (ops.conv_wgrad(x, dy, Cout, KH, KW, any_width=aw),), x, dy)
            (db,) = SIDE.submit((bleaf,), lambda: (ops.colsum(dy.reshape(-1, Cout)),), dy)
            return dx, dw, db, None, None
        dw, db = SIDE.submit(ctx.leaves, param_grads, x, dy)
        return dx, dw, db, None, None


def conv2d(x, weight, bias, act=ACT_NONE, any_width=False):
    return Conv2dFn.apply(x, weight, bias, act, any_width)


class BatchNormActFn(Function):

    @staticmethod
    def forward(ctx, x, gamma, beta, running_mean, running_var, training, momentum, eps, act):
        C = x.shape[-1]
        x2 = x.reshape(-1, C)
        if training:
            mean, rstd = ops.bn_stats(x2, eps, momentum, running_mean, running_var)
        else:
            mean, rstd = running_mean, ops.bn_rstd(running_var, eps)
        y = ops.bn_apply(x2, mean, rstd, gamma, beta, act).reshape(x.shape)
        ctx.save_for_backward(x, gamma, beta, mean, rstd)
        ctx.act, ctx.training = act, training
        return y

    @staticmethod
    def backward(ctx, dy):
        x, gamma, beta, mean, rstd = ctx.saved_tensors
        C = x.shape[-1]
        dx, dg, db = ops.bn_bwd(x.reshape(-1, C), _c(dy).reshape(-1, C), mean, rstd, gamma, beta, ctx.act, ctx.training)
        return dx.reshape(x.shape), dg, db, None, None, None, None, None, None


def batch_norm_act(x, bn, act=ACT_NONE, count=True):
    training = bn.training
    if count and training and bn.track_running_stats:
        bn.num_batches_tracked += 1
    return BatchNormActFn.apply(x, bn.weight, bn.bias, bn.running_mean, bn.running_var, training, bn.momentum, bn.eps,
                                act)


class ConvBnFn(Function):

    @staticmethod
    def forward(ctx, x, weight, bias, gamma, beta, running_mean, running_var, momentum, eps,
                in_mean, in_rstd, in_gamma, in_beta, in_scale, in_shift, in_act):
        B, H, W, C = x.shape
        y, part, G = ops.conv3_bn_forward(x, weight, bias, in_scale, in_shift, in_act, True)
        mean, rstd, scale, shift = ops.bn_stats_finish(part, G, 64, B * H * W, eps, momentum, gamma, beta, running_mean, running_var)
        folded = in_scale is not None
        ctx.save_for_backward(x, weight, in_mean, in_rstd, in_gamma, in_beta)
        ctx.folded, ctx.in_act, ctx.has_bias = folded, in_act, bias is not None
        ctx.leaves = (weight, bias)
        ctx.mark_non_differentiable(mean, rstd, scale, shift)
        ctx.set_materialize_grads(False)
        return y, mean, rstd, scale, shift

    @staticmethod
    def backward(ctx, dy, *_):
        x, weight, in_mean, in_rstd, in_gamma, in_beta = ctx.saved_tensors
        if dy is None:
            return (None,) * 16
        dy = _c(dy)
        x2 = x.reshape(-1, 64)
        dx = dgi = dbi = None
        need_in = ctx.folded and (ctx.needs_input_grad[0] or ctx.needs_input_grad[11] or ctx.needs_input_grad[12])
        if ctx.needs_input_grad[0] or need_in:
            dr = ops.conv2d_dgrad(dy, weight)
            if ctx.folded:
                dx, dgi, dbi = ops.bn_bwd(x2, dr.reshape(-1, 64), in_mean, in_rstd, in_gamma, in_beta, ctx.in_act, True)
                dx = dx.reshape(x.shape)
            else:
                dx = dr
        want_dw, want_db = ctx.needs_input_grad[1], ctx.has_bias and ctx.needs_input_grad[2]

        def param_grads():
            xin = x if not ctx.folded else ops.bn_apply(x2, in_mean, in_rstd, in_gamma, in_beta, ctx.in_act).reshape(x.shape)
            if want_dw and want_db:
                return ops.conv_wgrad(xin, dy, 64, 3, 3, want_db=True)
            dw = ops.conv_wgrad(xin, dy, 64, 3, 3) if want_dw else None
            db = ops.colsum(dy.reshape(-1, 64)) if want_db else None
            return dw, db
        dw, db = SIDE.submit(ctx.leaves, param_grads, x, dy, in_mean, in_rstd, in_gamma, in_beta, weight)
        return (dx, dw, db) + (None,) * 8 + (dgi, dbi, None, None, None)


class BatchNormApplyFn(Function):

    @staticmethod
    def forward(ctx, x, mean, rstd, gamma, beta, act):
        C = x.shape[-1]
        y = ops.bn_apply(x.reshape(-1, C), mean, rstd, gamma, beta, act).reshape(x.shape)
        ctx.save_for_backward(x, mean, rstd, gamma, beta)
        ctx.act = act
        return y

    @staticmethod
    def backward(ctx, dy):
        x, mean, rstd, gamma, beta = ctx.saved_tensors
        C = x.shape[-1]
        dx, dg, db = ops.bn_bwd(x.reshape(-1, C), _c(dy).reshape(-1, C), mean, rstd, gamma, beta, ctx.act, True)
        return dx.reshape(x.shape), None, None, dg, db, None


def conv_bn(x, conv, bn, prev=None):
    if prev is None:
        ins = (None,) * 6 + (ACT_NONE,)
    else:
        (pm, pr, ps, psh), pbn, pact = prev
        ins = (pm, pr, pbn.weight, pbn.bias, ps, psh, pact)
    out = ConvBnFn.apply(x, conv.weight, conv.bias, bn.weight, bn.bias, bn.running_mean, bn.running_var, bn.momentum, bn.eps, *ins)
    return out[0], tuple(out[1:])


def bn_apply_stats(y, stats, bn, act=ACT_NONE):
    return BatchNormApplyFn.apply(y, stats[0], stats[1], bn.weight, bn.bias, act)


SRB_BWD_FUSED = False


class SrbTrunkFn(Function):

    @staticmethod
    def forward(ctx, x, w1, b1, g1, be1, rm1, rv1, mom1, eps1, w2, b2, g2, be2, rm2, rv2, mom2, eps2):
        B, H, W, C = x.shape
        M = B * H * W
        y1, part1, G1 = ops.conv3_bn_forward(x, w1, b1, None, None, ACT_NONE, True)
        mean1, rstd1, sc1, sh1 = ops.bn_stats_finish(part1, G1, 64, M, eps1, mom1, g1, be1, rm1, rv1)
        y2, part2, G2 = ops.conv3_bn_forward(y1, w2, b2, sc1, sh1, ACT_MISH, True)
        mean2, rstd2, _, _ = ops.bn_stats_finish(part2, G2, 64, M, eps2, mom2, g2, be2, rm2, rv2)
        r = ops.bn_apply(y2.reshape(-1, 64), mean2, rstd2, g2, be2, ACT_NONE).reshape(x.shape)
        ctx.save_for_backward(x, y1, y2, w1, w2, g1, be1, g2, be2, mean1, rstd1, mean2, rstd2)
        ctx.has_b = (b1 is not None, b2 is not None)
        ctx.leaves = (w1, b1, w2, b2)
        return r

    @staticmethod
    def backward(ctx, d):
        x, y1, y2, w1, w2, g1, be1, g2, be2, mean1, rstd1, mean2, rstd2 = ctx.saved_tensors
        B, H, W, C = x.shape
        M = B * H * W
        d = _c(d)
        y1f, y2f = y1.reshape(M, 64), y2.reshape(M, 64)
        part2, G2 = ops.bn_bwd_partials(y2f, d.reshape(M, 64), mean2, rstd2, g2, be2, ACT_NONE)
        dg2, dbe2, coef2 = ops.bn_bwd_finish(part2, G2, 64, M, mean2, rstd2, g2)
        du1, part1, G1 = ops.conv3_dgrad_bn(d, w2, y2, coef2, ep=(y1, mean1, rstd1, g1, be1, ACT_MISH))
        dg1, dbe1, coef1 = ops.bn_bwd_finish(part1, G1, 64, M, mean1, rstd1, g1)
        dx = None
        if ctx.needs_input_grad[0]:
            dx, _, _ = ops.conv3_dgrad_bn(du1, w1, y1, coef1)
        want_b1, want_b2 = ctx.has_b

        def param_grads():
            dy2 = ops.bn_bwd_affine(y2f, d.reshape(M, 64), coef2).reshape(x.shape)
            a1 = ops.bn_apply(y1f, mean1, rstd1, g1, be1, ACT_MISH).reshape(x.shape)
            r2 = ops.conv_wgrad(a1, dy2, 64, 3, 3, want_db=want_b2)
            dy1 = ops.bn_bwd_affine(y1f, du1.reshape(M, 64), coef1).reshape(x.shape)
            r1 = ops.conv_wgrad(x, dy1, 64, 3, 3, want_db=want_b1)
            dw2, db2 = r2 if want_b2 else (r2, None)
            dw1, db1 = r1 if want_b1 else (r1, None)
            return dw1, db1, dw2, db2
        dw1, db1, dw2, db2 = SIDE.submit(ctx.leaves, param_grads, x, y1, y2, d, du1, coef1, coef2, mean1, rstd1, g1, be1, w1, w2)
        return (dx, dw1, db1, dg1, dbe1, None, None, None, None, dw2, db2, dg2, dbe2, None, None, None, None)


def srb_trunk(x, blk):
    c1, n1, c2, n2 = blk.conv1, blk.bn1, blk.conv2, blk.bn2
    return SrbTrunkFn.apply(x, c1.weight, c1.bias, n1.weight, n1.bias, n1.running_mean, n1.running_var, n1.momentum, n1.eps,
                            c2.weight, c2.bias, n2.weight, n2.bias, n2.running_mean, n2.running_var, n2.momentum, n2.eps)


class _PackedLinears:

    def __init__(self):
        self.table = {}


_PKL = _PackedLinears()
_TOKGEMM_NK = {(192, 128), (192, 64), (128, 192), (128, 128), (128, 64), (64, 192), (64, 64), (64, 128)}


def linear_prepack(linears):
    import ctypes
    _PKL.table = {}
    if not TOKGEMM_SB:
        return
    pk_ptrs, pk_dims, outs = [], [], {}
    for l in linears:
        W = l.weight
        N, K = W.shape
        if not W.is_cuda or (N, K) not in _TOKGEMM_NK or (K, N) not in _TOKGEMM_NK or W.data_ptr() in outs:
            continue
        Wfk, Wbk = ops.new(W, N * K), ops.new(W, N * K)
        pk_ptrs += [W.data_ptr(), Wfk.data_ptr(), W.data_ptr(), Wbk.data_ptr()]
        pk_dims += [N, K, K, 0, K, N, K, 1]
        outs[W.data_ptr()] = (Wfk, Wbk, W._version)
    if pk_ptrs:
        ops.call("tatt_tokgemm_pack_batch", (ctypes.c_void_p * len(pk_ptrs))(*pk_ptrs), (ctypes.c_int * len(pk_dims))(*pk_dims),
                 len(pk_ptrs) // 2, ops.stream())
    _PKL.table = outs


def linear_prepack_done():
    _PKL.table = {}


def _packed_linear(weight, M):
    e = _PKL.table.get(weight.data_ptr()) if TOKGEMM_SB else None
    if e is None or e[2] != weight._version or M % 64 or M < 64:
        return None
    return e[0], e[1]


def _tokgemm_ex(X, Wpk, bias, N, K, act=ACT_NONE, out=None, accum=False):
    ops._check_dev(X)
    M = X.shape[0]
    Y = ops.new(X, M, N) if out is None else out
    ops.call("tatt_tokgemm_sb_ex", ops.P(X), None, K, ops.P(Wpk), ops.P(bias), ops.P(Y), None, N, M, N, K, int(act), int(bool(accum)),
             ops.stream())
    return Y


def _linear_wgrad(dy2, x2, dw, db):
    if TOK_WGRAD_SB and ops.tok_wgrad_takes(dy2, x2) and dw.is_contiguous():
        ops.tok_wgrad_sb(dy2, x2, dw, db)
    else:
        ops.linear_bwd_weight(dy2, x2, out=dw, out_ld=dw.shape[1], rowsum=db)


TOK_WGRAD_SB = True


class LinearFn(Function):

    @staticmethod
    def forward(ctx, x, xb, weight, bias, act, alpha):
        K1 = x.shape[-1]
        x2 = x.reshape(-1, K1)
        xb2 = xb.reshape(-1, xb.shape[-1]) if xb is not None else None
        pk = _packed_linear(weight, x2.shape[0]) if (xb is None and alpha == 1.0 and act in (ACT_NONE, ACT_RELU)) else None
        if pk is not None:
            y = _tokgemm_ex(x2, pk[0], bias, weight.shape[0], K1, act)
        else:
            y = ops.linear_fwd(x2, weight, bias, act=act, alpha=alpha, x2b=xb2)
        ctx.save_for_backward(x, xb, weight, y if act != ACT_NONE else None)
        ctx.act, ctx.alpha, ctx.has_bias = act, alpha, bias is not None
        ctx.leaves = (weight, bias)
        ctx.wbk = pk[1] if pk is not None else None
        return y.reshape(*x.shape[:-1], weight.shape[0])

    @staticmethod
    def backward(ctx, dy):
# ... 235 lines not shown
        C = x.shape[-1]
        x2 = x.reshape(-1, C)
        dgi, dgh, hprev = ops.gru32_bwd(gates, out, _c(dout).reshape(-1, 64), whh_f, whh_r, ctx.geom)
        dx = ops.linear_bwd_input(dgi[:, :96], wih_f)
        ops.linear_bwd_input(dgi[:, 96:], wih_r, out=dx, beta=1.0)
        g = []
        for d in range(2):
            gi_d, gh_d = dgi[:, 96 * d:96 * (d + 1)], dgh[:, 96 * d:96 * (d + 1)]
            g.append((ops.linear_bwd_weight(gi_d, x2), ops.linear_bwd_weight(gh_d, hprev[:, 32 * d:32 * (d + 1)]),
                      ops.colsum(gi_d), ops.colsum(gh_d)))
        (dwih_f, dwhh_f, dbih_f, dbhh_f), (dwih_r, dwhh_r, dbih_r, dbhh_r) = g
        return dx.reshape(x.shape), dwih_f, dwhh_f, dbih_f, dbhh_f, dwih_r, dwhh_r, dbih_r, dbhh_r, None


def bigru32(x, gru, vertical):
    return BiGRU32Fn.apply(_c(x), gru.weight_ih_l0, gru.weight_hh_l0, gru.bias_ih_l0, gru.bias_hh_l0,
                           gru.weight_ih_l0_reverse, gru.weight_hh_l0_reverse, gru.bias_ih_l0_reverse,
                           gru.bias_hh_l0_reverse, vertical)


class _Precomposed:

    def __init__(self):
        self.table = {}


_PRE = _Precomposed()


def gru_precompose(blocks):
    import ctypes
    blocks = [b for b in blocks if b.conv1.weight.is_cuda]
    _PRE.table = {}
    if not blocks:
        return
    ptrs, Ks, outs = [], [], {}
    pk_ptrs, pk_dims = [], []
    for b in blocks:
        g, Wc = b.gru, b.conv1.weight
        K = Wc.numel() // Wc.shape[0]
        Wp, bp = ops.new(Wc, 192, K), ops.new(Wc, 192)
        ptrs += [t.data_ptr() for t in (g.weight_ih_l0, g.weight_ih_l0_reverse, g.bias_ih_l0, g.bias_ih_l0_reverse, Wc, b.conv1.bias, Wp, bp)]
        Ks.append(K)
        Wfk = Wbk = None
        if TOKGEMM_SB and K in (64, 128):
            Wfk, Wbk = ops.new(Wc, 192 * K), ops.new(Wc, 192 * K)
            pk_ptrs += [Wp.data_ptr(), Wfk.data_ptr(), Wp.data_ptr(), Wbk.data_ptr()]
            pk_dims += [192, K, K, 0, K, 192, K, 1]
        outs[Wc.data_ptr()] = (Wp, bp, Wc._version, Wfk, Wbk)
    ops.call("tatt_gru_compose_batch", (ctypes.c_void_p * len(ptrs))(*ptrs), (ctypes.c_int * len(Ks))(*Ks), len(Ks), ops.stream())
    if pk_ptrs:
        ops.call("tatt_tokgemm_pack_batch", (ctypes.c_void_p * len(pk_ptrs))(*pk_ptrs), (ctypes.c_int * len(pk_dims))(*pk_dims),
                 len(pk_ptrs) // 2, ops.stream())
    _PRE.table = outs


def gru_precompose_done():
    _PRE.table = {}


TOKGEMM_SB = True
GRU_WGRAD_SB = True
GRU_WGRAD_FRAG = True
SRB_IN_FOLD = True


def _tokgemm(X1, X2, Wpk, bias, N, K, N1=None, in_bn=None, in_add=None):
    M, K1 = X1.shape
    N1 = N if N1 is None else N1
    Y1 = ops.new(X1, M, N1)
    Y2 = ops.new(X1, M, N - N1) if N1 < N else None
    if in_bn is None and in_add is None:
        ops.call("tatt_tokgemm_sb", ops.P(X1), ops.P(X2), K1, ops.P(Wpk), ops.P(bias), ops.P(Y1), ops.P(Y2), N1, M, N, K, ops.stream())
    else:
        ops.call("tatt_tokgemm_sb_in", ops.P(X1), ops.P(X2), K1, ops.P(Wpk), ops.P(bias), ops.P(Y1), ops.P(Y2), N1, M, N, K,
                 *[ops.P(t) for t in (in_bn or (None,) * 4)], ops.P(in_add), ops.stream())
    return Y1, Y2


class GruBlockFn(Function):

    @staticmethod
    def forward(ctx, x, xb, conv_w, conv_b, wih_f, whh_f, bih_f, bhh_f, wih_r, whh_r, bih_r, bhh_r, vertical,
                in_mean=None, in_rstd=None, in_gamma=None, in_beta=None, in_add=None):
        B, H, W, K1 = x.shape
        in_bn = (in_mean, in_rstd, in_gamma, in_beta) if in_mean is not None else None
        Wc = conv_w.reshape(conv_w.shape[0], -1)
        K = Wc.shape[1]
        x2 = x.reshape(-1, K1)
        xb2 = xb.reshape(-1, K - K1) if xb is not None else None
        pre = _PRE.table.pop(conv_w.data_ptr(), None)
        Wfk = Wbk = None
        if pre is not None and pre[2] == conv_w._version and pre[0].device == x.device:
            Wp, bp, Wfk, Wbk = pre[0], pre[1], pre[3], pre[4]
        else:
            Wp = ops.new(x, 192, K)
            bp = ops.new(x, 192)
            ops.call("tatt_gru_compose", ops.P(wih_f), ops.P(wih_r), ops.P(bih_f), ops.P(bih_r), ops.P(Wc), ops.P(conv_b),
                     ops.P(Wp), ops.P(bp), K, ops.stream())
        use_tg = TOKGEMM_SB and x2.shape[0] % 64 == 0 and K in (64, 128) and K1 % 4 == 0
        if use_tg and Wfk is None:
            Wfk, Wbk = ops.new(x, 192 * K), ops.new(x, 192 * K)
            ops.call("tatt_tokgemm_pack", ops.P(Wp), ops.P(Wfk), 192, K, K, 0, ops.stream())
            ops.call("tatt_tokgemm_pack", ops.P(Wp), ops.P(Wbk), K, 192, K, 1, ops.stream())
        assert use_tg or (in_bn is None and in_add is None)
        if use_tg:
            gi, _ = _tokgemm(x2, xb2, Wfk, bp, 192, K, in_bn=in_bn, in_add=None if in_add is None else in_add.reshape(-1, K1))
        else:
            gi = ops.linear_fwd(x2, Wp, bp, x2b=xb2)
            Wbk = None
        geom = ops.seq_geom(B, H, W, vertical)
        out, gates = ops.gru32_fwd(gi, whh_f, bhh_f, whh_r, bhh_r, geom, save=any(ctx.needs_input_grad))
        ctx.save_for_backward(x, xb, Wc, Wp, gates, out, wih_f, whh_f, wih_r, whh_r, conv_b, Wbk, in_mean, in_rstd, in_gamma, in_beta, in_add)
        ctx.geom = geom
        ctx.wshape = conv_w.shape
        ctx.leaves = (conv_w, conv_b, wih_f, whh_f, bih_f, bhh_f, wih_r, whh_r, bih_r, bhh_r)
        return out.reshape(B, H, W, 64)

    @staticmethod
    def backward(ctx, dout):
        x, xb, Wc, Wp, gates, out, wih_f, whh_f, wih_r, whh_r, conv_b, Wbk, in_mean, in_rstd, in_gamma, in_beta, in_add = ctx.saved_tensors
        K1 = x.shape[-1]
        K = Wc.shape[1]
        x2 = x.reshape(-1, K1)
        xb2 = xb.reshape(-1, K - K1) if xb is not None else None
        in_bn = (in_mean, in_rstd, in_gamma, in_beta) if in_mean is not None else None
        add2 = in_add.reshape(-1, K1) if in_add is not None else None
        folded = in_bn is not None or in_add is not None
        need_dx = ctx.needs_input_grad[0] or any(ctx.needs_input_grad[13:])
        use_frag = folded or (GRU_WGRAD_FRAG and GRU_WGRAD_SB and K in (64, 128) and K1 == 64 and ops.gru_frag_ok(ctx.geom)
                              and x2.is_contiguous() and (xb2 is None or xb2.is_contiguous()))
        dgh = hprev = frag = None
        if use_frag:
            dgi, frag = ops.gru32_bwd_frag(gates, out, _c(dout).reshape(-1, 64), whh_f, whh_r, ctx.geom)
        else:
            dgi, dgh, hprev = ops.gru32_bwd(gates, out, _c(dout).reshape(-1, 64), whh_f, whh_r, ctx.geom)
        dxb = None
        if Wbk is not None and need_dx and (xb is None or ctx.needs_input_grad[1]):
            dx, dxb = _tokgemm(dgi, None, Wbk, None, K, 192, K1)
            dx = dx.reshape(x.shape)
            dxb = dxb.reshape(xb.shape) if xb is not None else None
        elif xb is not None and need_dx and ctx.needs_input_grad[1] and K == 2 * K1:
            dx, dxb = ops.linear_bwd_input_halves(dgi, Wp)
            dx, dxb = dx.reshape(x.shape), dxb.reshape(xb.shape)
        else:
            dx = ops.linear_bwd_input(dgi, Wp, col0=0, ncols=K1).reshape(x.shape) if need_dx else None
            if xb is not None and ctx.needs_input_grad[1]:
                dxb = ops.linear_bwd_input(dgi, Wp, col0=K1, ncols=K - K1).reshape(xb.shape)
        dgam = dbet = dadd = None
        if in_bn is not None and dx is not None:
            dx, dgam, dbet = ops.bn_bwd(x2, dx.reshape(-1, K1), in_mean, in_rstd, in_gamma, in_beta, ACT_NONE, True)
            dx = dx.reshape(x.shape)
        elif in_add is not None:
            dadd = dx
        geom = ctx.geom

        def param_grads():
            dbp, dbhh = ops.new(dgi, 192), ops.new(dgi, 192)
            dWp = ops.new(dgi, 192, K)
            if use_frag:
                dWhh = ops.new(dgi, 192, 32)
                ops.gru_wgrad_frag(frag, x2, xb2, geom, dWp, dWhh, dbp, dbhh, in_bn=in_bn, in_add=add2)
            elif GRU_WGRAD_SB and K in (64, 128) and K1 == 64 and ops.gru_wgrad_fusable(dgi, dgh, x2, xb2, hprev):
                dWhh = ops.new(dgi, 192, 64)
                ops.gru_wgrad_sb(dgi, dgh, x2, xb2, hprev, dWp, dWhh, dbp, dbhh)
            else:
                ops.linear_bwd_weight(dgi, x2, out=dWp, out_ld=K, rowsum=dbp)
                if xb is not None:
                    ops.linear_bwd_weight(dgi, xb2, out=dWp.reshape(-1)[K1:], out_ld=K)
                dWhh = ops.linear_bwd_weight(dgh, hprev, rowsum=dbhh)
            yield
            dwih_f, dwih_r = ops.new(dgi, 96, 64), ops.new(dgi, 96, 64)
            dwhh_f, dwhh_r = ops.new(dgi, 96, 32), ops.new(dgi, 96, 32)
            dWc, dbc = ops.new(dgi, 64, K), ops.new(dgi, 64)
            ops.call("tatt_gru_tail_c" if use_frag else "tatt_gru_tail", ops.P(dWp), ops.P(dbp), ops.P(Wc), ops.P(conv_b),
                     ops.P(wih_f), ops.P(wih_r), ops.P(dwih_f), ops.P(dwih_r), ops.P(dWc), ops.P(dbc), K, ops.P(dWhh),
                     ops.P(dwhh_f), ops.P(dwhh_r), ops.stream())
            return (dWc.reshape(ctx.wshape), dbc, dwih_f, dwhh_f, dbp[:96], dbhh[:96], dwih_r, dwhh_r, dbp[96:], dbhh[96:])
        pg = SIDE.submit(ctx.leaves, param_grads, dgi, dgh, hprev, frag, x, xb, Wp, Wc, in_mean, in_rstd, in_gamma, in_beta, in_add)
        return (dx, dxb) + tuple(pg) + (None, None, None, dgam, dbet, dadd)


def _gru_in_foldable(x, xb, blk, vertical, is_sum):
    if not (SRB_IN_FOLD and TOKGEMM_SB and GRU_WGRAD_FRAG and GRU_WGRAD_SB) or not x.is_cuda or x.dtype != torch.float32:
        return False
    B, H, W, K1 = x.shape
    Wc = blk.conv1.weight
    K = Wc.numel() // Wc.shape[0]
    if K1 != 64 or K != K1 + (0 if xb is None else xb.shape[-1]) or K not in (64, 128) or (is_sum and xb is not None):
        return False
    return (B * H * W) % 64 == 0 and ops.gru_frag_ok(ops.seq_geom(B, H, W, vertical))


def gru_block(x, blk, vertical, xb=None):
    g = blk.gru
    xb = None if xb is None else _c(xb)
    extra = (None,) * 5
    if isinstance(x, tuple):
        x0 = _c(x[0])
        if _gru_in_foldable(x0, xb, blk, vertical, len(x) == 2):
            extra = (x[1], x[2], x[3], x[4], None) if len(x) == 5 else (None, None, None, None, _c(x[1]))
            x = x0
        else:
            x = BatchNormApplyFn.apply(x[0], x[1], x[2], x[3], x[4], ACT_NONE) if len(x) == 5 else add(x[0], x[1])
    return GruBlockFn.apply(_c(x), xb, blk.conv1.weight, blk.conv1.bias,
                            g.weight_ih_l0, g.weight_hh_l0, g.bias_ih_l0, g.bias_hh_l0,
                            g.weight_ih_l0_reverse, g.weight_hh_l0_reverse, g.bias_ih_l0_reverse, g.bias_hh_l0_reverse,
                            vertical, *extra)


class AddFn(Function):
    @staticmethod
    def forward(ctx, a, b):
        return ops.axpby(a, b, 1.0, 1.0)

    @staticmethod
    def backward(ctx, dy):
        return dy, dy


def add(a, b):
    return AddFn.apply(_c(a), _c(b))


class Fork2Fn(Function):

    @staticmethod
    def forward(ctx, x):
        return x.view_as(x), x.view_as(x)

    @staticmethod
    def backward(ctx, ga, gb):
        if ga is None or gb is None:
            return ga if gb is None else gb
        if ga.is_cuda and ga.dtype == torch.float32 and ga.shape == gb.shape:
            return ops.add_n([_c(ga), _c(gb)])
        return ga + gb


def fork2(x):
    return Fork2Fn.apply(x) if (x.requires_grad and torch.is_grad_enabled()) else (x, x)


class AddRowBcastFn(Function):

    @staticmethod
    def forward(ctx, a, b):
        return ops.add_rowbcast(a, b, b.shape[0])

    @staticmethod
    def backward(ctx, dy):
        return dy, None


class ScaleFn(Function):
    @staticmethod
    def forward(ctx, a, s):
        ctx.s = s
        return ops.axpby(a, None, s, 0.0)

    @staticmethod
    def backward(ctx, dy):
        return ops.axpby(_c(dy), None, ctx.s, 0.0), None


class MeanOf2Fn(Function):
    @staticmethod
    def forward(ctx, a, b):
        return ops.axpby(a, b, 0.5, 0.5)

    @staticmethod
    def backward(ctx, dy):
        h = ops.axpby(_c(dy), None, 0.5, 0.0)
        return h, h


class ActFn(Function):

    @staticmethod
    def forward(ctx, x, act):
        y = ops.act_fwd(x, act)
        ctx.save_for_backward(y)
        ctx.act = act
        return y

    @staticmethod
    def backward(ctx, dy):
# ... 1166 lines not shown
```

tatt_amd/ops.py:

```python
from __future__ import annotations

import ctypes
import weakref
from typing import Optional

import os

import torch

from ._lib import LIB

ACT_NONE, ACT_RELU, ACT_MISH, ACT_TANH = 0, 1, 2, 3
_vp = ctypes.c_void_p


def _check_dev(t: torch.Tensor):
    if not t.is_cuda:
        raise RuntimeError("tatt_amd kernels need tensors on an AMD GPU (HIP device); got %s. "
                           "There is no CPU fallback in the product path." % t.device)
    if t.dtype != torch.float32:
        raise RuntimeError("tatt_amd kernels are fp32; got %s" % t.dtype)


def P(t: Optional[torch.Tensor]):
# ... 304 lines not shown
CONV_SPLIT_TILES, CONV_SPLIT_WGS = 256, 768


def conv_fwd(x_bhwc, wpacked, bias, Cout, KH, KW, *, act=ACT_NONE, out=None, beta=0.0):
    _check_dev(x_bhwc)
    B, H, W, Cin = x_bhwc.shape
    sn, sh, sw, sc = x_bhwc.stride()
    y = out if out is not None else new(x_bhwc, B, H, W, Cout)
    contig = x_bhwc.is_contiguous()
    if contig and KH == 9 and KW == 9 and Cout == 4 and Cin % 16 == 0 and H % 8 == 0 and W % 32 == 0 \
            and act == ACT_NONE and beta == 0.0:
        call("tatt_conv9_c64_to_c4", P(x_bhwc), P(wpacked), P(bias), P(y), B, H, W, Cin, stream())
        return y
    if contig and KH == 9 and KW == 9 and Cout == 64 and Cin == 4 and H % 4 == 0 and W % 64 == 0 and beta == 0.0 \
            and y.is_contiguous():
        call("tatt_conv9_c4_to_c64_sb" if CONV9_SB and CONV9_SB_C4 else "tatt_conv9_c4_to_c64", P(x_bhwc), P(wpacked), P(bias), P(y), B, H, W, act, stream())
        return y
    M = B * H * W
    splitk, ws = conv_split(x_bhwc, Cout, KH, KW), None
    if splitk > 1:
        ws = _split_ws(new(x_bhwc, splitk * M * Cout))
    call("tatt_conv2d_fwd", P(x_bhwc), sn, sh, sw, sc, P(wpacked), P(bias), P(y), Cout, B, H, W, Cin, Cout, KH, KW,
         act, beta, splitk, P(ws), stream())
    return y


def conv_split(x_bhwc, Cout, KH, KW):
    B, H, W, Cin = x_bhwc.shape
    tiles, nchunks = cdiv(B * H * W, 64) * cdiv(Cout, 64), cdiv(KH * KW * Cin, 16)
    if tiles < CONV_SPLIT_TILES and nchunks >= 32:
        return max(1, min(CONV_SPLIT_WGS // tiles, nchunks // 8))
    return 1


def conv_partials(x_bhwc, wpacked, Cout, KH, KW):
    _check_dev(x_bhwc)
    B, H, W, Cin = x_bhwc.shape
    sn, sh, sw, sc = x_bhwc.stride()
    splitk = conv_split(x_bhwc, Cout, KH, KW)
    ws = new(x_bhwc, splitk, B, H, W, Cout)
    got = ctypes.c_int(0)
    call("tatt_conv2d_fwd_partials", P(x_bhwc), sn, sh, sw, sc, P(wpacked), B, H, W, Cin, Cout, KH, KW, splitk, P(ws),
         ctypes.byref(got), stream())
    return ws, int(got.value)


CONV3_SB_NARROW_MAPS = False


def _conv3_geom_ok(x_bhwc, any_width=False):
    H, W = x_bhwc.shape[1], x_bhwc.shape[2]
    return W % 64 == 0 or (CONV3_SB and H % 4 == 0 and ((CONV3_SB_NARROW_MAPS and W % 16 == 0) or (any_width and CONV3_SB_GENERATION == 4)))


def _conv3_fast_ok(x_bhwc, Cin, Cout, KH, KW, any_width=False):
    return (x_bhwc.is_contiguous() and KH == 3 and KW == 3 and Cin % 64 == 0 and Cout % 64 == 0
            and _conv3_geom_ok(x_bhwc, any_width))


_WS_ENTRY, _WS_FWD_MODE, _WS_DGRAD_MODE = "tatt_conv3_c64_fwd_ws16", 6, 7


CONV3_SB = True
CONV3_SB_GENERATION = 4


def _batch_slices(B, takes):
    nb = B
    while nb > 1 and not takes(nb):
        nb = (nb + 1) // 2
    if not takes(nb):
        return None
    return [(b, min(B, b + nb)) for b in range(0, B, nb)]


def _conv3_sb_slices(x_bhwc, cin, cout, act):
    B, H, W, _ = x_bhwc.shape
    if LIB.tatt_conv3_sb_generation(0) != CONV3_SB_GENERATION:
        LIB.tatt_conv3_sb_generation(int(CONV3_SB_GENERATION))
    return _batch_slices(B, lambda nb: LIB.tatt_conv3_sb_route(nb, H, W, cin, cout, int(act), ACT_NONE) != 0)


def _conv3_sb_groups(nb, H, W):
    return min(256, nb * H * W // 64)


def _conv3_sb(x_bhwc, w_oihw, mode, bias, act=ACT_NONE, in_scale=None, in_shift=None, in_act=ACT_NONE, stats=None):
    B, H, W, cin = x_bhwc.shape
    cout = w_oihw.shape[0] if mode == 10 else w_oihw.shape[1]
    assert cin == (w_oihw.shape[1] if mode == 10 else w_oihw.shape[0])
    slices = _conv3_sb_slices(x_bhwc, cin, cout, act)
    if slices is None:
        raise RuntimeError("tatt_conv3_c64_fwd_sb takes no slice of a (%d, %d, %d, %d) map" % (B, H, W, cin))
    nb0 = slices[0][1]
    wl = repack_weight(w_oihw, LIB.tatt_conv3_sb_packing(nb0, H, W, cin, cout, int(act), ACT_NONE) + (mode - 10))
    y = new(x_bhwc, B, H, W, cout)
    nchunk = cin // 64
    assert nchunk == 1 or stats is None
    g0 = 0
    for b0, b1 in slices:
        xs, ys = x_bhwc[b0:b1], y[b0:b1]
        st = stats[g0 * 128:] if stats is not None else None
        for c in range(nchunk):
            call("tatt_conv3_c64_fwd_sb", P(xs), cin, 64 * c, P(wl[c * cout * 576:]), P(bias) if c == 0 else None, P(ys), b1 - b0, H, W,
                 cout, int(act) if c == nchunk - 1 else ACT_NONE, 0.0 if c == 0 else 1.0, P(in_scale), P(in_shift), int(in_act), P(st),
                 stream())
        g0 += _conv3_sb_groups(b1 - b0, H, W)
    return y


CONV9_SB = True
CONV9_SB_C4 = True
CONV9_SB_WGRAD = True


def _conv9_mfma_ok(x_bhwc):
    return x_bhwc.is_contiguous() and x_bhwc.shape[1] % 4 == 0 and x_bhwc.shape[2] % 64 == 0 and x_bhwc.shape[3] == 64


def conv2d_forward(x_bhwc, weight_oihw, bias, act=ACT_NONE, any_width=False):
    Cout, Cin, KH, KW = weight_oihw.shape
    if KH == 9 and KW == 9 and Cout == 4 and Cin == 64 and act == ACT_NONE and _conv9_mfma_ok(x_bhwc):
        B, H, W, _ = x_bhwc.shape
        y = new(x_bhwc, B, H, W, 4)
        if CONV9_SB:
            call("tatt_conv9_c64_to_c4_sb", P(x_bhwc), P(repack_weight(weight_oihw, 12)), P(bias), P(y), B, H, W, stream())
        else:
            call("tatt_conv9_c64_to_c4_mfma", P(x_bhwc), P(repack_weight(weight_oihw, 8)), P(bias), P(y), B, H, W, stream())
        return y
    if _conv3_fast_ok(x_bhwc, Cin, Cout, KH, KW, any_width):
        B, H, W, _ = x_bhwc.shape
        if CONV3_SB and _conv3_sb_slices(x_bhwc, Cin, Cout, act) is not None:
            return _conv3_sb(x_bhwc, weight_oihw, 10, bias, act)
        if W % 64 == 0:
            y = new(x_bhwc, B, H, W, Cout)
            if Cin == 64:
                wl = repack_weight(weight_oihw, _WS_FWD_MODE)
                call(_WS_ENTRY, P(x_bhwc), P(wl), P(bias), P(y), B, H, W, Cout, act, 0.0, stream())
                return y
            wt = repack_weight(weight_oihw, 2)
            call("tatt_conv3_c64_fwd_t", P(x_bhwc), P(wt), P(bias), P(y), B, H, W, Cin, Cout, act, 0.0, stream())
            return y
    return conv_fwd(x_bhwc, repack_weight(weight_oihw, 0), bias, Cout, KH, KW, act=act)


def conv3_bn_fusable(x_bhwc, weight_oihw, bn=None):
    if bn is not None and (bn.momentum is None or not bn.affine or not bn.track_running_stats or bn.running_mean is None):
        return False
    return (tuple(weight_oihw.shape) == (64, 64, 3, 3) and x_bhwc.is_contiguous()
            and x_bhwc.shape[3] == 64 and _conv3_geom_ok(x_bhwc))


def conv3_bn_forward(x_bhwc, weight_oihw, bias, in_scale=None, in_shift=None, in_act=ACT_NONE, want_stats=True):
    _check_dev(x_bhwc)
    B, H, W, _ = x_bhwc.shape
    if CONV3_SB:
        slices = _conv3_sb_slices(x_bhwc, 64, 64, ACT_NONE) or [(0, B)]
        G = sum(_conv3_sb_groups(b1 - b0, H, W) for b0, b1 in slices)
        part = new(x_bhwc, G * 128, dtype=torch.float64) if want_stats else None
        return _conv3_sb(x_bhwc, weight_oihw, 10, bias, ACT_NONE, in_scale, in_shift, in_act, part), part, G
    G = min(256, B * H * W // 64)
    part = new(x_bhwc, G * 128, dtype=torch.float64) if want_stats else None
    y = new(x_bhwc, B, H, W, 64)
    call("tatt_conv3_c64_fwd_ws16_bn", P(x_bhwc), P(repack_weight(weight_oihw, 6)), P(bias), P(y), B, H, W, 64, ACT_NONE, 0.0,
         P(in_scale), P(in_shift), int(in_act), P(part), stream())
    return y, part, G


def bn_stats_finish(part, G, C, M, eps, momentum, gamma, beta, running_mean, running_var):
    mean, rstd, scale, shift = new(gamma, C), new(gamma, C), new(gamma, C), new(gamma, C)
    call("tatt_bn_stats_finish", P(part), G, C, M, float(eps), float(momentum), P(gamma), P(beta), P(mean), P(rstd),
         P(running_mean), P(running_var), P(scale), P(shift), stream())
    return mean, rstd, scale, shift


def conv2d_dgrad(dy_bhwc, weight_oihw, any_width=False):
    Cout, Cin, KH, KW = weight_oihw.shape
    if KH == 9 and KW == 9 and Cout == 64 and Cin == 4 and _conv9_mfma_ok(dy_bhwc):
        B, H, W, _ = dy_bhwc.shape
        dx = new(dy_bhwc, B, H, W, 4)
        if CONV9_SB:
            call("tatt_conv9_c64_to_c4_sb", P(dy_bhwc), P(repack_weight(weight_oihw, 13)), None, P(dx), B, H, W, stream())
        else:
            call("tatt_conv9_c64_to_c4_mfma", P(dy_bhwc), P(repack_weight(weight_oihw, 9)), None, P(dx), B, H, W, stream())
        return dx
    if _conv3_fast_ok(dy_bhwc, Cout, Cin, KH, KW, any_width):
        B, H, W, _ = dy_bhwc.shape
        if CONV3_SB and _conv3_sb_slices(dy_bhwc, Cout, Cin, ACT_NONE) is not None:
            return _conv3_sb(dy_bhwc, weight_oihw, 11, None)
        if W % 64:
            return conv_fwd(dy_bhwc, repack_weight(weight_oihw, 1), None, Cin, KH, KW)
        dx = new(dy_bhwc, B, H, W, Cin)
        if Cout == 64:
            wl = repack_weight(weight_oihw, _WS_DGRAD_MODE)
            call(_WS_ENTRY, P(dy_bhwc), P(wl), None, P(dx), B, H, W, Cin, ACT_NONE, 0.0, stream())
            return dx
        wt = repack_weight(weight_oihw, 3)
        call("tatt_conv3_c64_fwd_t", P(dy_bhwc), P(wt), None, P(dx), B, H, W, Cout, Cin, ACT_NONE, 0.0, stream())
        return dx
    return conv_fwd(dy_bhwc, repack_weight(weight_oihw, 1), None, Cin, KH, KW)


def conv_wgrad(x_bhwc, dy_bhwc, Cout, KH, KW, want_db=False, any_width=False):
    B, H, W, Cin = x_bhwc.shape
    sn, sh, sw, sc = x_bhwc.stride()
    dw = new(x_bhwc, Cout, Cin, KH, KW)
    contig = x_bhwc.is_contiguous() and dy_bhwc.is_contiguous()
    if contig and KH == 3 and KW == 3 and Cin % 64 == 0 and Cout % 64 == 0 and (W % 64 == 0 or (CONV3_WGRAD_SB and H % 4 == 0 and ((CONV3_SB_NARROW_MAPS and W % 16 == 0) or any_width))):
        slices = (_batch_slices(B, lambda nb: LIB.tatt_conv3_wgrad_sb_route(nb, H, W, Cin, Cout) != 0) if CONV3_WGRAD_SB else None) \
            or [(0, B)]
        nblk = (Cin // 64) * (Cout // 64)
        groups = []
        for b0, b1 in slices:
            nseg = (b1 - b0) * (H // 4) * ((W + 15) // 16) if W % 64 else (b1 - b0) * H * W // 64
            groups.append(min(nseg, max(1, (CONV3_WGRAD_GROUPS if nblk == 1 else 256) // nblk)))
        G = sum(groups)
        n = G * 9 * Cin * Cout
        part = _split_ws(new(x_bhwc, n + (G * Cout if want_db else 0)))
        db = new(x_bhwc, Cout) if want_db else None
        g0 = 0
        for (b0, b1), g in zip(slices, groups):
            call("tatt_conv3_c64_wgrad_partial_sb" if CONV3_WGRAD_SB else "tatt_conv3_c64_wgrad_partial", P(x_bhwc[b0:b1]), P(dy_bhwc[b0:b1]),
                 P(part[g0 * 9 * Cin * Cout:]), P(part[n + g0 * Cout:]) if want_db else None, b1 - b0, H, W, Cin, Cout, g, stream())
            g0 += g
        call("tatt_splitk_reduce", P(part), P(dw), 9 * Cin, Cout, G, Cin, 9, 0.0, P(db), Cout, stream())
        return (dw, db) if want_db else dw
    if want_db:
        return _conv_wgrad_general(x_bhwc, dy_bhwc, dw, Cout, KH, KW, contig), colsum(dy_bhwc.reshape(-1, Cout))
    return _conv_wgrad_general(x_bhwc, dy_bhwc, dw, Cout, KH, KW, contig)


CONV_WGRAD_SPLIT_CAP = 256


def _conv_wgrad_general(x_bhwc, dy_bhwc, dw, Cout, KH, KW, contig):
    B, H, W, Cin = x_bhwc.shape
    sn, sh, sw, sc = x_bhwc.stride()
    if contig and KH == 9 and KW == 9 and Cout == 4 and Cin == 64 and H % 4 == 0 and W % 64 == 0:
        G = min(B * (H // 4) * (W // 64), 256)
        part = new(x_bhwc, G * 64 * 336)
        call("tatt_conv9_c64_c4_wgrad_sb" if CONV9_SB and CONV9_SB_WGRAD else "tatt_conv9_c64_c4_wgrad", P(x_bhwc), P(dy_bhwc), P(dw), P(part), B, H, W, stream())
        return dw
    if contig and KH == 9 and KW == 9 and Cout == 64 and Cin == 4 and H % 4 == 0 and W % 64 == 0:
        G = min(B * (H // 4) * (W // 64), 256)
        part = new(x_bhwc, G * 64 * 336)
        call("tatt_conv9_c4_c64_wgrad_sb" if CONV9_SB and CONV9_SB_WGRAD else "tatt_conv9_c4_c64_wgrad", P(x_bhwc), P(dy_bhwc), P(dw), P(part), B, H, W, stream())
        return dw
    Mo, Kred = KH * KW * Cin, B * H * W
    splitk = max(2, _auto_split(Mo, Cout, Kred, cap=CONV_WGRAD_SPLIT_CAP))
    ws = _split_ws(new(x_bhwc, (splitk + 1) * Mo * Cout))
    call("tatt_conv2d_wgrad", P(x_bhwc), sn, sh, sw, sc, P(dy_bhwc), Cout, P(dw), B, H, W, Cin, Cout, KH, KW, 0.0,
         splitk, P(ws), stream())
    return dw


def bn_stats(x2, eps, momentum, running_mean, running_var):
    M, C = x2.shape
    mean, rstd = new(x2, C), new(x2, C)
    ws = new(x2, 256 * 2 * C, dtype=torch.float64)
    call("tatt_bn_stats", P(x2), x2.stride(0), M, C, eps, momentum, P(mean), P(rstd), P(running_mean), P(running_var),
         P(ws), stream())
    return mean, rstd


def bn_rstd(var, eps):
    rstd = torch.empty_like(var)
    call("tatt_bn_rstd", P(var), P(rstd), var.numel(), eps, stream())
    return rstd


def bn_apply(x2, mean, rstd, gamma, beta, act, out=None):
    M, C = x2.shape
    y = out if out is not None else new(x2, M, C)
    call("tatt_bn_apply", P(x2), x2.stride(0), P(y), y.stride(0), M, C, P(mean), P(rstd), P(gamma), P(beta), act, stream())
    return y


def bn_bwd(x2, dy2, mean, rstd, gamma, beta, act, training):
    M, C = x2.shape
    dx = new(x2, M, C)
    dgamma, dbeta, sums = new(x2, C), new(x2, C), new(x2, 2 * C)
    ws = new(x2, 256 * 2 * C, dtype=torch.float64)
    call("tatt_bn_bwd", P(x2), x2.stride(0), P(dy2), dy2.stride(0), P(dx), C, M, C, P(mean), P(rstd), P(gamma), P(beta),
         act, int(training), P(dgamma), P(dbeta), P(sums), P(ws), stream())
    return dx, dgamma, dbeta


def bn_bwd_partials(x2, dy2, mean, rstd, gamma, beta, act):
    M, C = x2.shape
    G = LIB.tatt_bn_bwd_groups(int(M))
    part = new(x2, G * 2 * C, dtype=torch.float64)
    call("tatt_bn_bwd_partials", P(x2), x2.stride(0), P(dy2), dy2.stride(0), M, C, P(mean), P(rstd), P(gamma), P(beta), int(act),
         P(part), stream())
    return part, G


def bn_bwd_finish(part, G, C, M, mean, rstd, gamma):
    dgamma, dbeta, coef = new(gamma, C), new(gamma, C), new(gamma, 3, C)
    call("tatt_bn_bwd_finish", P(part), G, C, M, P(mean), P(rstd), P(gamma), P(dgamma), P(dbeta), P(coef), stream())
    return dgamma, dbeta, coef


def bn_bwd_affine(x2, du2, coef):
    M, C = x2.shape
    dx = new(x2, M, C)
    call("tatt_bn_bwd_affine", P(x2), P(du2), P(dx), M, C, P(coef), stream())
    return dx


def conv3_dgrad_bn(du_bhwc, weight_oihw, x2_bhwc=None, coef=None, ep=None):
    _check_dev(du_bhwc)
    B, H, W, _ = du_bhwc.shape
    if LIB.tatt_conv3_sb_generation(0) != CONV3_SB_GENERATION:
        LIB.tatt_conv3_sb_generation(int(CONV3_SB_GENERATION))
    wl = repack_weight(weight_oihw, LIB.tatt_conv3_sb_packing(B, H, W, 64, 64, ACT_NONE, int(ep[5]) if ep is not None else ACT_NONE) + 1)
    out = new(du_bhwc, B, H, W, 64)
    G = min(256, B * H * W // 64)
    part = new(du_bhwc, G * 128, dtype=torch.float64) if ep is not None else None
    a = b = c = None
    if x2_bhwc is not None:
        a, b, c = coef[0], coef[1], coef[2]
    e = ep if ep is not None else (None,) * 5 + (ACT_NONE,)
    call("tatt_conv3_c64_dgrad_bn_sb", P(du_bhwc), P(x2_bhwc), P(a), P(b), P(c), P(wl), P(out), B, H, W, P(e[0]), P(e[1]), P(e[2]),
         P(e[3]), P(e[4]), int(e[5]), P(part), stream())
    return out, part, G


def ln_fwd(a2, b2, gamma, beta, eps=1e-5, mode=0, pdrop=0.0, seed=None, site=0):
    M, C = a2.shape
    y, stats = new(a2, M, C), new(a2, M, 2)
    call("tatt_ln_fwd", P(a2), P(b2), P(y), P(stats), M, C, P(gamma), P(beta), eps, mode, float(pdrop), P(seed), int(site),
         stream())
    return y, stats


def ln_bwd(a2, b2, dy2, stats, gamma, eps=1e-5, mode=0, pdrop=0.0, seed=None, site=0):
    M, C = a2.shape
    dx, dgb = new(a2, M, C), new(a2, 2 * C)
    db2 = new(a2, M, C) if (pdrop > 0.0 and b2 is not None) else None
    dgamma, dbeta = dgb[:C], dgb[C:]
    G = cdiv(M, 64)
    part = new(a2, G * 2 * C)
    ws = new(a2, 256 * 2 * C, dtype=torch.float64)
    call("tatt_ln_bwd", P(a2), P(b2), P(dy2), P(stats), P(dx), P(db2), M, C, P(gamma), P(dgamma), P(dbeta), P(part), P(ws),
         eps, mode, float(pdrop), P(seed), int(site), stream())
    if db2 is None and b2 is not None:
        db2 = dx
    return dx, db2, dgamma, dbeta


def prelu_fwd(x, alpha):
    _check_dev(x)
    y = torch.empty_like(x)
    call("tatt_prelu_fwd", P(x), P(y), P(alpha), x.numel(), stream())
    return y


def prelu_bwd(x, dy, alpha):
    dx = torch.empty_like(x)
    G = cdiv(x.numel(), 256)
    part = new(x, G, 1)
    call("tatt_prelu_bwd", P(x), P(dy), P(dx), P(alpha), x.numel(), P(part), stream())
    return dx, colsum(part)


def act_fwd(x, act):
    y = torch.empty_like(x)
    call("tatt_act_fwd", P(x), P(y), x.numel(), act, stream())
    return y


def act_bwd(ref, dy, act, from_output):
    dx = torch.empty_like(dy)
    call("tatt_act_bwd", P(ref), P(dy), P(dx), dy.numel(), act, int(from_output), stream())
    return dx


def axpby(a, b, alpha=1.0, beta=1.0):
    _check_dev(a)
    y = torch.empty_like(a)
    call("tatt_axpby", P(a), P(b), P(y), alpha, beta, a.numel(), stream())
    return y
# ... 339 lines not shown
```

tatt_amd/tsrn.py:

```python
from __future__ import annotations

import copy
import math

import numpy as np
import torch
from torch import nn

from . import functional as Fh
from .ops import ACT_NONE, ACT_RELU, ACT_MISH, ACT_TANH
from . import ops


def _nchw(x_nhwc):
    return x_nhwc.permute(0, 3, 1, 2)


class _Holder(nn.Module):
    def forward(self, *a, **k):
        raise RuntimeError("parameter holder: the computation runs in tatt_amd's HIP kernels")


class GruBlock(_Holder):

# ... 156 lines not shown

    def __init__(self, output_image_size, num_control_points, margins):
        super().__init__()
        self.output_image_size = output_image_size
        self.num_control_points = num_control_points
        H, W = output_image_size
        N = num_control_points
        k = N // 2
        xs = np.linspace(margins[0], 1.0 - margins[0], k)
        pts = np.concatenate([np.stack([xs, np.full(k, margins[1])], 1),
                              np.stack([xs, np.full(k, 1.0 - margins[1])], 1)], 0)
        tcp = torch.Tensor(pts)
        fk = torch.zeros(N + 3, N + 3)
        fk[:N, :N].copy_(_tps_phi(tcp, tcp))
        fk[:N, -3].fill_(1)
        fk[-3, :N].fill_(1)
        fk[:N, -2:].copy_(tcp)
        fk[-2:, :N].copy_(tcp.transpose(0, 1))
        inverse_kernel = torch.inverse(fk).contiguous()
        ys, xs_ = torch.meshgrid(torch.arange(H), torch.arange(W), indexing="ij")
        coord = torch.stack([xs_.reshape(-1).float(), ys.reshape(-1).float()], 1)
        Y = coord[:, 1:2] / (H - 1)
        X = coord[:, 0:1] / (W - 1)
        coord = torch.cat([X, Y], 1)
        rep = torch.cat([_tps_phi(coord, tcp), torch.ones(H * W, 1), coord], 1)
        self.register_buffer("inverse_kernel", inverse_kernel)
        self.register_buffer("padding_matrix", torch.zeros(3, 2))
        self.register_buffer("target_coordinate_repr", rep)
        self.register_buffer("target_control_points", tcp)


def _require_gpu(x):
    if not x.is_cuda:
        raise RuntimeError("tatt_amd: inputs must be on an AMD GPU (x.device=%s); the product path has no CPU "
                           "fallback (the CPU restatement lives in oracle/ and is test infrastructure)." % x.device)


STN_FUSED = True


def _stn_forward(x_nchw, stn: STNHead, count=True):
    h = x_nchw.permute(0, 2, 3, 1)
    if STN_FUSED and Fh.stn_head_fusable(h, stn, h.shape[0]):
        if count:
            for bn in [stn.stn_convnet[i][1] for i in (0, 2, 4, 6, 8, 10)] + [stn.stn_fc1[1]]:
                bn.num_batches_tracked += 1
        return Fh.stn_head(h, stn).reshape(h.shape[0], stn.num_ctrlpoints, 2)
    pools = {0: (2, 2), 2: (2, 2), 4: (2, 2), 6: (2, 2), 8: (1, 2)}
    for i in (0, 2, 4, 6, 8, 10):
        conv, bn = stn.stn_convnet[i][0], stn.stn_convnet[i][1]
        h = Fh.conv2d(h, conv.weight, conv.bias)
        h = Fh.batch_norm_act(h, bn, ACT_RELU, count)
        if i in pools:
            h = Fh.max_pool(h, *pools[i])
    B = h.shape[0]
    h = Fh.Permute4dFn.apply(h, (0, 3, 1, 2)).reshape(B, -1)
    fc1, bn1 = stn.stn_fc1[0], stn.stn_fc1[1]
    h = Fh.linear(h, fc1.weight, fc1.bias)
    h = Fh.batch_norm_act(h, bn1, ACT_RELU, count)
    h = Fh.ScaleFn.apply(h, 0.1)
    h = Fh.linear(h, stn.stn_fc2.weight, stn.stn_fc2.bias)
    return h.reshape(B, stn.num_ctrlpoints, 2)


def _tps_forward(x_nchw, ctrl, tps: TPSSpatialTransformer):
    assert ctrl.dim() == 3 and ctrl.size(1) == tps.num_control_points and ctrl.size(2) == 2
    src = Fh.TpsGridFn.apply(ctrl.contiguous(), tps.inverse_kernel, tps.padding_matrix, tps.target_coordinate_repr)
    return Fh.GridSampleFn.apply(x_nchw, src), src


def _gru_block(x, blk: GruBlock, vertical, x_cat=None):
    return Fh.gru_block(x, blk, vertical, xb=x_cat)


def _srb(x, tp_map, blk: RecurrentResidualBlock):
    x, x_res = Fh.fork2(x)
    if blk.bn1.training and blk.bn2.training and ops.conv3_bn_fusable(x, blk.conv1.weight, blk.bn1) and ops.conv3_bn_fusable(x, blk.conv2.weight, blk.bn2):
        if Fh.SRB_BWD_FUSED and ops.CONV3_SB:
            r = Fh.srb_trunk(_cc(x), blk)
        else:
            y1, st1 = Fh.conv_bn(x, blk.conv1, blk.bn1)
            y2, st2 = Fh.conv_bn(y1, blk.conv2, blk.bn2, prev=(st1, blk.bn1, ACT_MISH))
            if Fh.SRB_IN_FOLD:
                r = Fh.gru_block((y2, st2[0], st2[1], blk.bn2.weight, blk.bn2.bias), blk.gru1, True, xb=tp_map)
                return Fh.gru_block((x_res, r), blk.gru2, False)
            r = Fh.bn_apply_stats(y2, st2, blk.bn2, ACT_NONE)
    else:
        r = Fh.conv2d(x, blk.conv1.weight, blk.conv1.bias)
        r = Fh.batch_norm_act(r, blk.bn1, ACT_MISH, False)
        r = Fh.conv2d(r, blk.conv2.weight, blk.conv2.bias)
        r = Fh.batch_norm_act(r, blk.bn2, ACT_NONE, False)
    r = _gru_block(r, blk.gru1, True, x_cat=tp_map)
    return _gru_block(Fh.add(x_res, r), blk.gru2, False)


def _ffn(x, layer, training, site):
    h = Fh.linear(x, layer.linear1.weight, layer.linear1.bias, act=ACT_RELU)
    h = Fh.dropout(h, layer.p, training, site)
    return Fh.linear(h, layer.linear2.weight, layer.linear2.bias)


def _query_pos(ig: TPInterpreter, B, H, W):
    C = ig.init_factor.weight.shape[1]
    return Fh.query_embedding(ig.init_factor.weight, ig.transformer.gru_encoding, B, H, W).reshape(B, H * W, C)


def _enc_params(enc):
    sa = enc.self_attn
    return (sa.in_proj_weight, sa.in_proj_bias, sa.out_proj.weight, sa.out_proj.bias, enc.linear1.weight, enc.linear1.bias,
            enc.linear2.weight, enc.linear2.bias, enc.norm1.weight, enc.norm1.bias, enc.norm2.weight, enc.norm2.bias)


def _dec_params(dec):
    ca = dec.multihead_attn
    return (ca.in_proj_weight, ca.in_proj_bias, ca.out_proj.weight, ca.out_proj.bias, dec.linear1.weight, dec.linear1.bias,
            dec.linear2.weight, dec.linear2.bias, dec.norm2.weight, dec.norm2.bias, dec.norm3.weight, dec.norm3.bias)


DP_QGRU_WITH_TP = False
QGRU_BUCKET = "first"
OUTCONV_BUCKET = "srb0"
OUTCONV_BIAS_BUCKET = "trunk"
PRECOMPOSE_ON_FORK = True
TP_FUSED = True


def _tp_fusable(ig: TPInterpreter, L):
    tr = ig.transformer
    enc, decs = tr.encoder.layers, tr.decoder.layers
    if not TP_FUSED:
        return False
    if len(enc) != 1 or not 1 <= len(decs) <= 2 or L > 32:
        return False
    for m, att in [(enc[0], enc[0].self_attn)] + [(d, d.multihead_attn) for d in decs]:
        if att.embed_dim != 64 or att.num_heads != 4 or tuple(m.linear1.weight.shape) != (64, 64):
            return False
    return True


def _tp_text_side(tp, ig: TPInterpreter, training):
    B, L, C = tp.shape[0], tp.shape[3], ig.fc_in.weight.shape[0]
    x = Fh.Permute4dFn.apply(tp, (0, 3, 2, 1)).reshape(B, L, tp.shape[1])
    x = Fh.prelu(Fh.linear(x, ig.fc_in.weight, ig.fc_in.bias), ig.activation.weight)
    pe = ig.pe.pe[0, :L]
    tr = ig.transformer
    drop = training and ig.dropout_on
    if drop:
        pos = Fh.dropout(pe.unsqueeze(0).expand(B, L, C).contiguous(), ig.pe.p, True, 1)
    else:
        pos = pe
    src = Fh.ScaleFn.apply(x, 2.0)
    if not _tp_fusable(ig, L):
        return src, pos, None
    enc = tr.encoder.layers[0]
    pd = lambda v: float(v) if drop else 0.0
    cfg = Fh.TPStackCfg((2,), pd(enc.self_attn.dropout), pd(enc.p), pd(enc.p), False, False, True, enc.norm1.eps)
    memory, _ = Fh.TPStackFn.apply(_cc(src), _cc(pos), src, pos, cfg, *_enc_params(enc))
    return src, pos, memory


def _tp_interpreter(feat, tp, ig: TPInterpreter, training, qpos=None, text=None):
    B, H, W, C = feat.shape
    L = tp.shape[3]
    tr = ig.transformer
    drop = training and ig.dropout_on
    pd = lambda v: float(v) if drop else 0.0
    if text is None:
# ... 262 lines not shown
```

Baseline: 11770.

## Fuse BN stats finish into conv3 and BN backward via last-block ticket

Adds a last-block-arrives pattern: each block of the conv3 SB forward kernel and of the BN backward partials kernels writes its partial sums, bumps an atomic ticket, and the final block reduces all partials and computes mean/rstd/scale/shift (or dgamma/dbeta/coef). This removes separate finish-kernel launches and their launch gaps in the SRB trunk and GRU input-BN paths. It adds atomic traffic, cache-coherent stores, persistent ticket buffers per BN module, and serialises the tail reduction onto one block.

```diff
diff --git a/include/tatt_hip.h b/include/tatt_hip.h
--- a/include/tatt_hip.h
+++ b/include/tatt_hip.h
@@ -47,6 +47,11 @@
 int tatt_conv3_c64_fwd_sb(const float* x, int cin_total, int ci0, const float* wl, const float* bias, float* y, int B, int H,
                           int W, int Cout, int act, float beta, const float* in_scale, const float* in_shift, int in_act,
                           double* stats, hipStream_t st);
+int tatt_conv3_c64_fwd_sb_bn_la(const float* x, const float* wl, const float* bias, float* y, int B, int H, int W,
+                                const float* in_scale, const float* in_shift, int in_act, double* stats, int G, int M,
+                                float eps, float momentum, const float* gamma, const float* beta, float* mean, float* rstd,
+                                float* running_mean, float* running_var, float* scale, float* shift, unsigned long long* ticket,
+                                hipStream_t st);
 int tatt_conv3_c64_dgrad_bn_sb(const float* x, const float* x2, const float* in_scale, const float* in_scale2,
                                const float* in_shift, const float* wl, float* y, int B, int H, int W, const float* ep_x,
                                const float* ep_mean, const float* ep_rstd, const float* ep_gamma, const float* ep_beta,
@@ -100,6 +105,12 @@
                          const float* rstd, const float* gamma, const float* beta, int act, double* part, hipStream_t st);
 int tatt_bn_bwd_finish(const double* part, int G, int C, int M, const float* mean, const float* rstd, const float* gamma,
                        float* dgamma, float* dbeta, float* coef, hipStream_t st);
+int tatt_bn_bwd_la(const float* X, long ldx, const float* dY, long lddy, float* dX, long lddx, int M, int C,
+                   const float* mean, const float* rstd, const float* gamma, const float* beta, int act,
+                   int training, float* dgamma, float* dbeta, float* sums, double* ws, unsigned long long* ticket, hipStream_t st);
+int tatt_bn_bwd_partials_finish_la(const float* X, long ldx, const float* dY, long lddy, int M, int C, const float* mean,
+                                   const float* rstd, const float* gamma, const float* beta, int act, double* part,
+                                   float* dgamma, float* dbeta, float* coef, unsigned long long* ticket, hipStream_t st);
 int tatt_bn_bwd_affine(const float* X, const float* dU, float* dX, int M, int C, const float* coef, hipStream_t st);
 
 int tatt_ln_fwd(const float* A, const float* Bres, float* Y, float* stats, int M, int C,
diff --git a/tatt_amd/csrc/bn_finish.h b/tatt_amd/csrc/bn_finish.h
--- /dev/null
+++ b/tatt_amd/csrc/bn_finish.h
@@ -0,0 +1,148 @@
+#pragma once
+#include "handoff.h"
+
+typedef double f64x2 __attribute__((ext_vector_type(2)));
+typedef double f64x4 __attribute__((ext_vector_type(4)));
+
+#define S2_L 16
+__device__ __forceinline__ double s2_combine(double (*sh)[64], int tx) {
+    double s = 0.0;
+#pragma unroll
+    for (int l = 0; l < S2_L; l += 4) s += (sh[l][tx] + sh[l + 1][tx]) + (sh[l + 2][tx] + sh[l + 3][tx]);
+    return s;
+}
+template <typename T, bool AHEAD16, typename L>
+__device__ __forceinline__ T s2_lane_sum(int n, L&& load) {
+    T acc[8];
+#pragma unroll
+    for (int u = 0; u < 8; ++u) acc[u] = T(0.0);
+    int i = 0;
+    if constexpr (AHEAD16) {
+        T v[16];
+#pragma unroll
+        for (int u = 0; u < 16; ++u) v[u] = u < n ? load(u) : T(0.0);
+#pragma unroll
+        for (int h = 0; h < 16; h += 8) {
+            if (n >= h + 8) {
+#pragma unroll
+                for (int u = 0; u < 8; ++u) acc[u] += v[h + u];
+            } else {
+#pragma unroll
+                for (int u = 0; u < 8; ++u) if (h + u < n) acc[0] += v[h + u];
+            }
+        }
+        i = 16;
+    }
+    for (; i + 8 <= n; i += 8) {
+        T w[8];
+#pragma unroll
+        for (int u = 0; u < 8; ++u) w[u] = load(i + u);
+#pragma unroll
+        for (int u = 0; u < 8; ++u) acc[u] += w[u];
+    }
+    for (; i < n; ++i) acc[0] += load(i);
+    T s = T(0.0);
+#pragma unroll
+    for (int u = 0; u < 8; ++u) s += acc[u];
+    return s;
+}
+__device__ __forceinline__ bool s2_reduce(const double* __restrict__ part, int G, int C, int c, int tx, int ty,
+                                          double (*sh)[S2_L][64], double& s, double& q) {
+    s = 0.0; q = 0.0;
+    if (c < C && ty < G) {
+        const double* p0 = part + ((long)ty * 2 + 0) * C + c;
+        const long stride = (long)2 * S2_L * C;
+        const int n = (G - ty + S2_L - 1) / S2_L;
+        s = s2_lane_sum<double, false>(n, [&](int i) { return p0[i * stride]; });
+        q = s2_lane_sum<double, false>(n, [&](int i) { return p0[i * stride + C]; });
+    }
+    sh[0][ty][tx] = s; sh[1][ty][tx] = q;
+    __syncthreads();
+    if (ty != 0 || c >= C) return false;
+    s = s2_combine(sh[0], tx);
+    q = s2_combine(sh[1], tx);
+    return true;
+}
+
+struct BnStatsOut {
+    int M;
+    float eps, momentum;
+    float *mean, *rstd, *running_mean, *running_var;
+    const float *gamma, *beta;
+    float *scale, *shift;
+    __device__ __forceinline__ void operator()(int c, int C, double s, double q) const {
+        double mu = s / M;
+        double var = q / M - mu * mu;
+        if (var < 0.0) var = 0.0;
+        mean[c] = (float)mu;
+        rstd[c] = (float)(1.0 / sqrt(var + (double)eps));
+        if (scale) {
+            const float sc = gamma[c] * rstd[c];
+            scale[c] = sc;
+            shift[c] = beta[c] - mean[c] * sc;
+        }
+        if (running_mean) {
+            double unb = M > 1 ? var * ((double)M / (M - 1)) : var;
+            running_mean[c] = (float)((1.0 - momentum) * running_mean[c] + momentum * mu);
+            running_var[c] = (float)((1.0 - momentum) * running_var[c] + momentum * unb);
+        }
+    }
+};
+struct BnBwdOut {
+    int M;
+    const float *mean, *rstd, *gamma;
+    float *dgamma, *dbeta, *sums, *coef;
+    __device__ __forceinline__ void operator()(int c, int C, double s, double q) const {
+        dbeta[c] = (float)s; dgamma[c] = (float)q;
+        if (sums) { sums[c] = (float)s; sums[C + c] = (float)q; }
+        if (coef) {
+            const float inv = 1.f / (float)M, g = gamma[c], rs = rstd[c];
+            const float a = g * rs;
+            const float b = -a * rs * ((float)q * inv);
+            coef[c] = a;
+            coef[C + c] = b;
+            coef[2 * C + c] = -a * ((float)s * inv) - b * mean[c];
+        }
+    }
+};
+
+__device__ __forceinline__ bool bn_ticket_last(unsigned long long* ticket, unsigned G, unsigned* s_last, bool leader) {
+    __syncthreads();
+    if (leader) {
+        const unsigned long long old = __hip_atomic_fetch_add(ticket, 1ull, __ATOMIC_RELAXED, __HIP_MEMORY_SCOPE_AGENT);
+        *s_last = (old + 1ull) % G == 0ull ? 1u : 0u;
+    }
+    __syncthreads();
+    return *s_last != 0u;
+}
+template <int NT, bool WIDE, typename Out>
+__device__ __forceinline__ void bn_tail_finish(const double* part, int G, int C, int th, double* sh, const Out& out) {
+    double (*const sh2)[S2_L][64] = reinterpret_cast<double (*)[S2_L][64]>(sh);
+    const int range = G * 2 * C * 8, stride = 2 * S2_L * C * 8;
+    for (int c0 = 0; c0 < C; c0 += 64) {
+#pragma unroll 1
+        for (int item = th; item < (WIDE ? 1 : 2) * 32 * S2_L; item += NT) {
+            const int k = item >> 9, ty = (item >> 5) & (S2_L - 1), tx = 2 * (item & 31), c = c0 + tx;
+            const int n = (G - ty + S2_L - 1) / S2_L, off0 = ((ty * 2 + k) * C + c) * 8;
+            const bool on = c < C && ty < G;
+            if constexpr (WIDE) {
+                f64x4 a = 0.0;
+                if (on) a = s2_lane_sum<f64x4, true>(n, [&](int i) {
+                    const f64x2 s = __builtin_bit_cast(f64x2, ld16_sc1(part, range, off0 + i * stride));
+                    const f64x2 q = __builtin_bit_cast(f64x2, ld16_sc1(part, range, off0 + i * stride + C * 8));
+                    f64x4 r; r[0] = s[0]; r[1] = s[1]; r[2] = q[0]; r[3] = q[1];
+                    return r;
+                });
+                sh2[0][ty][tx] = a[0]; sh2[0][ty][tx + 1] = a[1];
+                sh2[1][ty][tx] = a[2]; sh2[1][ty][tx + 1] = a[3];
+            } else {
+                f64x2 a = 0.0;
+                if (on) a = s2_lane_sum<f64x2, true>(n, [&](int i) { return __builtin_bit_cast(f64x2, ld16_sc1(part, range, off0 + i * stride)); });
+                sh2[k][ty][tx] = a[0]; sh2[k][ty][tx + 1] = a[1];
+            }
+        }
+        __syncthreads();
+        if (th < 64 && c0 + th < C) out(c0 + th, C, s2_combine(sh2[0], th), s2_combine(sh2[1], th));
+        __syncthreads();
+    }
+}
diff --git a/tatt_amd/csrc/conv3.hip b/tatt_amd/csrc/conv3.hip
--- a/tatt_amd/csrc/conv3.hip
+++ b/tatt_amd/csrc/conv3.hip
@@ -1,4 +1,5 @@
 #include "common.h"
+#include "bn_finish.h"
 #include <mutex>
 #include <stdlib.h>
 #include <type_traits>
@@ -802,8 +803,9 @@
         }
     }
 }
-template <int INMODE, bool EPBN>
-__global__ __launch_bounds__(512, 2) void conv3_c64_sb4_kernel(Conv3SB q) {
+struct Conv3SBT : Conv3SB { unsigned long long* ticket; BnStatsOut fin; };
+template <int INMODE, bool EPBN, bool TAIL = false>
+__global__ __launch_bounds__(512, 2) void conv3_c64_sb4_kernel(typename std::conditional<TAIL, Conv3SBT, Conv3SB>::type q) {
     const Conv3P& p = q.c;
     extern __shared__ __attribute__((aligned(16))) unsigned smem_u[];
     unsigned* const XCH = smem_u + 4 * S3_IMG;
@@ -820,7 +822,21 @@
     __shared__ float st_red[4][2][64];
     __shared__ __attribute__((aligned(16))) float cst[7][64];
     __shared__ __attribute__((aligned(16))) float cbias[64];
+    __shared__ unsigned s_last;
+    auto finish = [&]() {
+        if constexpr (TAIL) {
+            if (bn_ticket_last(q.ticket, gridDim.x, &s_last, t == 0))
+                bn_tail_finish<512, true>(p.stats, (int)gridDim.x, 64, (int)t, reinterpret_cast<double*>(smem_u), q.fin);
+        }
+    };
     if (pt >= npt) {
+        if constexpr (TAIL) {
+            const f64x2 z = 0.0;
+            if (t < 64) st16_sc1(p.stats, (int)gridDim.x * 1024, (int)blockIdx.x * 1024 + (int)t * 16, &z);
+            handoff_drain();
+            finish();
+            return;
+        }
         if (p.stats && t < 128) p.stats[(long)blockIdx.x * 128 + t] = 0.0;
         return;
     }
@@ -993,6 +1009,17 @@
             }
         }
         __syncthreads();
+        if constexpr (TAIL) {
+            if (h < 64) {
+                f64x2 a = 0.0;
+#pragma unroll
+                for (int w = 0; w < 4; ++w) { a[0] += (double)st_red[w][h >> 5][(2 * h) & 63]; a[1] += (double)st_red[w][h >> 5][((2 * h) & 63) + 1]; }
+                st16_sc1(p.stats, (int)gridDim.x * 1024, (int)blockIdx.x * 1024 + (int)h * 16, &a);
+                handoff_drain();
+            }
+            finish();
+            return;
+        }
         if (p.stats && h < 128) {
             double a = 0.0;
 #pragma unroll
@@ -1053,6 +1080,7 @@
         __syncthreads();
     }
     __syncthreads();
+    finish();
 }
 static int conv3_sb_generation = 4;
 TATT_API int tatt_conv3_sb_generation(int gen) {
@@ -1143,6 +1171,35 @@
     Conv3SB q = {{x, wl, bias, y, B, H, W, 64, Cout, act, beta, in_scale, in_shift, in_act, stats}, cin_total, ci0,
                  nullptr, nullptr, nullptr, nullptr, nullptr, nullptr, nullptr, 0};
     return conv3_sb_launch(q, st);
+}
+template <int INMODE>
+static void conv3_sb4_tail_go(const Conv3SBT& q, dim3 grid, hipStream_t st) {
+    static TattPerDevice attr_once;
+    tatt_per_device(attr_once, [&] {
+        (void)hipFuncSetAttribute(reinterpret_cast<const void*>(conv3_c64_sb4_kernel<INMODE, false, true>), hipFuncAttributeMaxDynamicSharedMemorySize, S3_LDS);
+    });
+    hipLaunchKernelGGL((conv3_c64_sb4_kernel<INMODE, false, true>), grid, dim3(512), S3_LDS, st, q);
+}
+TATT_API int tatt_conv3_c64_fwd_sb_bn_la(const float* x, const float* wl, const float* bias, float* y, int B, int H, int W,
+                                         const float* in_scale, const float* in_shift, int in_act, double* stats, int G, int M,
+                                         float eps, float momentum, const float* gamma, const float* beta, float* mean, float* rstd,
+                                         float* running_mean, float* running_var, float* scale, float* shift, unsigned long long* ticket,
+                                         hipStream_t st) {
+    if (!stats || !ticket || (((uintptr_t)ticket) & 7) || (((uintptr_t)stats) & 15) || !mean || !rstd) return 1;
+    if (scale && (!gamma || !beta || !shift)) return 2;
+    if (in_scale && (!in_shift || in_act == ACT_TANH)) return 3;
+    if (conv3_sb_pick(B, H, W, 64, 64, ACT_NONE, ACT_NONE) != 4) return 5;
+    const int npt = B * (H / 4) * ((W + 15) / 16);
+    if (G != (npt < 256 ? npt : 256) || M != B * H * W) return 6;
+    Conv3SBT q = {{{x, wl, bias, y, B, H, W, 64, 64, ACT_NONE, 0.f, in_scale, in_shift, in_act, stats}, 64, 0,
+                   nullptr, nullptr, nullptr, nullptr, nullptr, nullptr, nullptr, 0},
+                  ticket,
+                  {M, eps, momentum, mean, rstd, running_mean, running_var, gamma, beta, scale, shift}};
+    const int inmode = in_scale ? (in_act == ACT_MISH ? 1 : 3) : 0;
+    if (inmode == 1) conv3_sb4_tail_go<1>(q, dim3(G), st);
+    else if (inmode == 3) conv3_sb4_tail_go<3>(q, dim3(G), st);
+    else conv3_sb4_tail_go<0>(q, dim3(G), st);
+    return LAUNCH_CHECK();
 }
 TATT_API int tatt_conv3_c64_dgrad_bn_sb(const float* x, const float* x2, const float* in_scale, const float* in_scale2,
                                         const float* in_shift, const float* wl, float* y, int B, int H, int W, const float* ep_x,
diff --git a/tatt_amd/csrc/norm.hip b/tatt_amd/csrc/norm.hip
--- a/tatt_amd/csrc/norm.hip
+++ b/tatt_amd/csrc/norm.hip
@@ -1,4 +1,5 @@
 #include "common.h"
+#include "bn_finish.h"
 
 #define CS_MAXG 256
 
@@ -20,13 +21,6 @@
         __syncthreads();
     }
 }
-#define S2_L 16
-__device__ __forceinline__ double s2_combine(double (*sh)[64], int tx) {
-    double s = 0.0;
-#pragma unroll
-    for (int l = 0; l < S2_L; l += 4) s += (sh[l][tx] + sh[l + 1][tx]) + (sh[l + 2][tx] + sh[l + 3][tx]);
-    return s;
-}
 __global__ __launch_bounds__(64 * S2_L) void colsum_stage2(const double* __restrict__ part, int G, int C, long ldp,
                                                            float* __restrict__ out, float scale, float beta) {
     __shared__ double sh[S2_L][64];
@@ -76,9 +70,9 @@
     for (; m < m_end; m += rpar)
         f(*reinterpret_cast<const f32x4*>(X + (long)m * ldx + c4), *reinterpret_cast<const f32x4*>(Y + (long)m * ldy + c4));
 }
-template <int NQ>
+template <int NQ, bool SC1 = false>
 __device__ __forceinline__ void v4_block_partials(const double (&acc)[NQ][4], int C, int cv, int cl, int rl, int rpar,
-                                                  int c_base, double* __restrict__ part, double* sh) {
+                                                  int c_base, double* __restrict__ part, double* sh, int part_bytes = 0) {
     const int t = threadIdx.x;
 #pragma unroll
     for (int q = 0; q < NQ; ++q)
@@ -86,6 +80,19 @@
         for (int e = 0; e < 4; ++e) sh[q * 1024 + rl * (4 * cv) + 4 * cl + e] = acc[q][e];
     __syncthreads();
     const int width = 4 * cv;
+    if constexpr (SC1) {
+        for (int c = 2 * t; c < width; c += 512) {
+#pragma unroll
+            for (int q = 0; q < NQ; ++q) {
+                f64x2 s = 0.0;
+                for (int r = 0; r < rpar; ++r) { s[0] += sh[q * 1024 + r * width + c]; s[1] += sh[q * 1024 + r * width + c + 1]; }
+                st16_sc1(part, part_bytes, (int)((((long)blockIdx.x * NQ + q) * C + c_base + c) * 8), &s);
+            }
+        }
+        handoff_drain();
+        __syncthreads();
+        return;
+    }
     for (int c = t; c < width; c += 256) {
 #pragma unroll
         for (int q = 0; q < NQ; ++q) {
@@ -179,31 +186,10 @@
     __shared__ double sh[2][S2_L][64];
     const int tx = threadIdx.x & 63, ty = threadIdx.x >> 6;
     const int c = blockIdx.x * 64 + tx;
-    double s = 0.0, q = 0.0;
-    if (c < C && ty < G) {
-        s = sum_strided<double, 8>(part + ((long)ty * 2 + 0) * C + c, (G - ty + S2_L - 1) / S2_L, (long)2 * S2_L * C);
-        q = sum_strided<double, 8>(part + ((long)ty * 2 + 1) * C + c, (G - ty + S2_L - 1) / S2_L, (long)2 * S2_L * C);
-    }
-    sh[0][ty][tx] = s; sh[1][ty][tx] = q;
-    __syncthreads();
-    if (ty != 0 || c >= C) return;
-    s = s2_combine(sh[0], tx);
-    q = s2_combine(sh[1], tx);
-    double mu = s / M;
-    double var = q / M - mu * mu;
-    if (var < 0.0) var = 0.0;
-    mean[c] = (float)mu;
-    rstd[c] = (float)(1.0 / sqrt(var + (double)eps));
-    if (scale) {
-        const float sc = gamma[c] * rstd[c];
-        scale[c] = sc;
-        shift[c] = beta[c] - mean[c] * sc;
-    }
-    if (running_mean) {
-        double unb = M > 1 ? var * ((double)M / (M - 1)) : var;
-        running_mean[c] = (float)((1.0 - momentum) * running_mean[c] + momentum * mu);
-        running_var[c] = (float)((1.0 - momentum) * running_var[c] + momentum * unb);
-    }
+    double s, q;
+    if (!s2_reduce(part, G, C, c, tx, ty, sh, s, q)) return;
+    const BnStatsOut out = {M, eps, momentum, mean, rstd, running_mean, running_var, gamma, beta, scale, shift};
+    out(c, C, s, q);
 }
 TATT_API int tatt_bn_stats(const float* X, long ld, int M, int C, float eps, float momentum, float* mean,
                            float* rstd, float* running_mean, float* running_var, double* ws, hipStream_t st) {
@@ -329,10 +315,12 @@
         __syncthreads();
     }
 }
-__global__ __launch_bounds__(256) void bn_bwd_stage1_v4(const float* __restrict__ X, long ldx, const float* __restrict__ dY,
-                                                        long lddy, int M, int C, int rpb, const float* __restrict__ mean,
-                                                        const float* __restrict__ rstd, const float* __restrict__ gamma,
-                                                        const float* __restrict__ beta, int act, double* __restrict__ part) {
+template <bool TAIL>
+__device__ __forceinline__ void bn_bwd_stage1_v4_body(const float* __restrict__ X, long ldx, const float* __restrict__ dY, long lddy,
+                                                      int M, int C, int rpb, const float* __restrict__ mean,
+                                                      const float* __restrict__ rstd, const float* __restrict__ gamma,
+                                                      const float* __restrict__ beta, int act, double* __restrict__ part,
+                                                      unsigned long long* ticket, const BnBwdOut& out) {
     __shared__ double sh[2 * 1024];
     const int t = threadIdx.x;
     const int cv = min(C >> 2, 256), rpar = 256 / cv, cl = t % cv, rl = t / cv;
@@ -351,8 +339,25 @@
                 acc[0][e] += (double)du; acc[1][e] += (double)du * xh;
             }
         });
-        v4_block_partials<2>(acc, C, cv, cl, rl, rpar, c0, part, sh);
-    }
+        v4_block_partials<2, TAIL>(acc, C, cv, cl, rl, rpar, c0, part, sh, (int)gridDim.x * 2 * C * 8);
+    }
+    if constexpr (TAIL) {
+        __shared__ unsigned s_last;
+        if (bn_ticket_last(ticket, gridDim.x, &s_last, t == 0)) bn_tail_finish<256, true>(part, (int)gridDim.x, C, t, sh, out);
+    }
+}
+__global__ __launch_bounds__(256) void bn_bwd_stage1_v4(const float* __restrict__ X, long ldx, const float* __restrict__ dY,
+                                                        long lddy, int M, int C, int rpb, const float* __restrict__ mean,
+                                                        const float* __restrict__ rstd, const float* __restrict__ gamma,
+                                                        const float* __restrict__ beta, int act, double* __restrict__ part) {
+    bn_bwd_stage1_v4_body<false>(X, ldx, dY, lddy, M, C, rpb, mean, rstd, gamma, beta, act, part, nullptr, BnBwdOut{});
+}
+__global__ __launch_bounds__(256) void bn_bwd_stage1_v4_la(const float* __restrict__ X, long ldx, const float* __restrict__ dY,
+                                                           long lddy, int M, int C, int rpb, const float* __restrict__ mean,
+                                                           const float* __restrict__ rstd, const float* __restrict__ gamma,
+                                                           const float* __restrict__ beta, int act, double* __restrict__ part,
+                                                           unsigned long long* ticket, BnBwdOut out) {
+    bn_bwd_stage1_v4_body<true>(X, ldx, dY, lddy, M, C, rpb, mean, rstd, gamma, beta, act, part, ticket, out);
 }
 __global__ __launch_bounds__(64 * S2_L) void bn_bwd_stage2(const double* __restrict__ part, int G, int C,
                                                            float* __restrict__ dgamma, float* __restrict__ dbeta,
@@ -360,18 +365,10 @@
     __shared__ double sh[2][S2_L][64];
     const int tx = threadIdx.x & 63, ty = threadIdx.x >> 6;
     const int c = blockIdx.x * 64 + tx;
-    double s = 0.0, q = 0.0;
-    if (c < C && ty < G) {
-        s = sum_strided<double, 8>(part + ((long)ty * 2 + 0) * C + c, (G - ty + S2_L - 1) / S2_L, (long)2 * S2_L * C);
-        q = sum_strided<double, 8>(part + ((long)ty * 2 + 1) * C + c, (G - ty + S2_L - 1) / S2_L, (long)2 * S2_L * C);
-    }
-    sh[0][ty][tx] = s; sh[1][ty][tx] = q;
-    __syncthreads();
-    if (ty != 0 || c >= C) return;
-    s = s2_combine(sh[0], tx);
-    q = s2_combine(sh[1], tx);
-    dbeta[c] = (float)s; dgamma[c] = (float)q;
-    sums[c] = (float)s; sums[C + c] = (float)q;
+    double s, q;
+    if (!s2_reduce(part, G, C, c, tx, ty, sh, s, q)) return;
+    const BnBwdOut out = {0, nullptr, nullptr, nullptr, dgamma, dbeta, sums, nullptr};
+    out(c, C, s, q);
 }
 __global__ void bn_bwd_apply_kernel(const float* __restrict__ X, long ldx, const float* __restrict__ dY, long lddy,
                                     float* __restrict__ dX, long lddx, int M, int C,
@@ -431,18 +428,24 @@
         *reinterpret_cast<f32x4*>(dX + (m0 + r) * lddx + c4) = o;
     }
 }
-TATT_API int tatt_bn_bwd(const float* X, long ldx, const float* dY, long lddy, float* dX, long lddx, int M, int C,
-                         const float* mean, const float* rstd, const float* gamma, const float* beta, int act,
-                         int training, float* dgamma, float* dbeta, float* sums, double* ws, hipStream_t st) {
+static int bn_bwd_run(const float* X, long ldx, const float* dY, long lddy, float* dX, long lddx, int M, int C,
+                      const float* mean, const float* rstd, const float* gamma, const float* beta, int act,
+                      int training, float* dgamma, float* dbeta, float* sums, double* ws, unsigned long long* ticket, hipStream_t st) {
     int G = cs_groups(M);
     int rpb = cdiv(M, G);
     const bool v4 = v4_ok(X, ldx, C) && v4_ok(dY, lddy, C) && v4_ok(dX, lddx, C) &&
                     !((((uintptr_t)mean) | ((uintptr_t)rstd) | ((uintptr_t)gamma) | ((uintptr_t)beta) | ((uintptr_t)sums)) & 15);
-    if (v4) hipLaunchKernelGGL(bn_bwd_stage1_v4, dim3(G), dim3(256), 0, st, X, ldx, dY, lddy, M, C, rpb, mean, rstd, gamma, beta,
-                               act, ws);
-    else hipLaunchKernelGGL(bn_bwd_stage1, dim3(G), dim3(256), 0, st, X, ldx, dY, lddy, M, C, rpb, mean, rstd, gamma, beta,
-                            act, ws);
-    hipLaunchKernelGGL(bn_bwd_stage2, dim3(cdiv(C, 64)), dim3(64 * S2_L), 0, st, ws, G, C, dgamma, dbeta, sums);
+    if (v4 && ticket) {
+        const BnBwdOut out = {0, nullptr, nullptr, nullptr, dgamma, dbeta, sums, nullptr};
+        hipLaunchKernelGGL(bn_bwd_stage1_v4_la, dim3(G), dim3(256), 0, st, X, ldx, dY, lddy, M, C, rpb, mean, rstd, gamma, beta,
+                           act, ws, ticket, out);
+    } else {
+        if (v4) hipLaunchKernelGGL(bn_bwd_stage1_v4, dim3(G), dim3(256), 0, st, X, ldx, dY, lddy, M, C, rpb, mean, rstd, gamma, beta,
+                                   act, ws);
+        else hipLaunchKernelGGL(bn_bwd_stage1, dim3(G), dim3(256), 0, st, X, ldx, dY, lddy, M, C, rpb, mean, rstd, gamma, beta,
+                                act, ws);
+        hipLaunchKernelGGL(bn_bwd_stage2, dim3(cdiv(C, 64)), dim3(64 * S2_L), 0, st, ws, G, C, dgamma, dbeta, sums);
+    }
     if (v4) {
         const long items = (long)cdiv(M, BA_R) * (C / 4);
         hipLaunchKernelGGL(bn_bwd_apply_v4_kernel, dim3(cdiv(items, 256)), dim3(256), 0, st, X, ldx, dY, lddy, dX, lddx, M, C,
@@ -453,6 +456,18 @@
     hipLaunchKernelGGL(bn_bwd_apply_kernel, dim3(cdiv(total, 256)), dim3(256), 0, st, X, ldx, dY, lddy, dX, lddx, M, C,
                        mean, rstd, gamma, beta, act, sums, training);
     return LAUNCH_CHECK();
+}
+TATT_API int tatt_bn_bwd(const float* X, long ldx, const float* dY, long lddy, float* dX, long lddx, int M, int C,
+                         const float* mean, const float* rstd, const float* gamma, const float* beta, int act,
+                         int training, float* dgamma, float* dbeta, float* sums, double* ws, hipStream_t st) {
+    return bn_bwd_run(X, ldx, dY, lddy, dX, lddx, M, C, mean, rstd, gamma, beta, act, training, dgamma, dbeta, sums, ws, nullptr, st);
+}
+TATT_API int tatt_bn_bwd_la(const float* X, long ldx, const float* dY, long lddy, float* dX, long lddx, int M, int C,
+                            const float* mean, const float* rstd, const float* gamma, const float* beta, int act,
+                            int training, float* dgamma, float* dbeta, float* sums, double* ws, unsigned long long* ticket, hipStream_t st) {
+    if (!ticket || (((uintptr_t)ticket) & 7)) return 1;
+    return bn_bwd_run(X, ldx, dY, lddy, dX, lddx, M, C, mean, rstd, gamma, beta, act, training, dgamma, dbeta, sums, ws,
+                      ticket, st);
 }
 
 __global__ __launch_bounds__(64 * S2_L) void bn_bwd_finish_kernel(const double* __restrict__ part, int G, int C, int M,
@@ -462,23 +477,10 @@
     __shared__ double sh[2][S2_L][64];
     const int tx = threadIdx.x & 63, ty = threadIdx.x >> 6;
     const int c = blockIdx.x * 64 + tx;
-    double s = 0.0, q = 0.0;
-    if (c < C && ty < G) {
-        s = sum_strided<double, 8>(part + ((long)ty * 2 + 0) * C + c, (G - ty + S2_L - 1) / S2_L, (long)2 * S2_L * C);
-        q = sum_strided<double, 8>(part + ((long)ty * 2 + 1) * C + c, (G - ty + S2_L - 1) / S2_L, (long)2 * S2_L * C);
-    }
-    sh[0][ty][tx] = s; sh[1][ty][tx] = q;
-    __syncthreads();
-    if (ty != 0 || c >= C) return;
-    s = s2_combine(sh[0], tx);
-    q = s2_combine(sh[1], tx);
-    dbeta[c] = (float)s; dgamma[c] = (float)q;
-    const float inv = 1.f / (float)M, g = gamma[c], rs = rstd[c];
-    const float a = g * rs;
-    const float b = -a * rs * ((float)q * inv);
-    coef[c] = a;
-    coef[C + c] = b;
-    coef[2 * C + c] = -a * ((float)s * inv) - b * mean[c];
+    double s, q;
+    if (!s2_reduce(part, G, C, c, tx, ty, sh, s, q)) return;
+    const BnBwdOut out = {M, mean, rstd, gamma, dgamma, dbeta, nullptr, coef};
+    out(c, C, s, q);
 }
 TATT_API int tatt_bn_bwd_groups(int M) { return cs_groups(M); }
 TATT_API int tatt_bn_bwd_partials(const float* X, long ldx, const float* dY, long lddy, int M, int C, const float* mean,
@@ -488,6 +490,23 @@
                     !((((uintptr_t)mean) | ((uintptr_t)rstd) | ((uintptr_t)gamma) | ((uintptr_t)beta)) & 15);
     if (v4) hipLaunchKernelGGL(bn_bwd_stage1_v4, dim3(G), dim3(256), 0, st, X, ldx, dY, lddy, M, C, rpb, mean, rstd, gamma, beta, act, part);
     else hipLaunchKernelGGL(bn_bwd_stage1, dim3(G), dim3(256), 0, st, X, ldx, dY, lddy, M, C, rpb, mean, rstd, gamma, beta, act, part);
+    return LAUNCH_CHECK();
+}
+TATT_API int tatt_bn_bwd_partials_finish_la(const float* X, long ldx, const float* dY, long lddy, int M, int C, const float* mean,
+                                            const float* rstd, const float* gamma, const float* beta, int act, double* part,
+                                            float* dgamma, float* dbeta, float* coef, unsigned long long* ticket, hipStream_t st) {
+    if (!ticket || (((uintptr_t)ticket) & 7)) return 1;
+    const int G = cs_groups(M), rpb = cdiv(M, G);
+    const bool v4 = v4_ok(X, ldx, C) && v4_ok(dY, lddy, C) &&
+                    !((((uintptr_t)mean) | ((uintptr_t)rstd) | ((uintptr_t)gamma) | ((uintptr_t)beta)) & 15);
+    if (v4) {
+        const BnBwdOut out = {M, mean, rstd, gamma, dgamma, dbeta, nullptr, coef};
+        hipLaunchKernelGGL(bn_bwd_stage1_v4_la, dim3(G), dim3(256), 0, st, X, ldx, dY, lddy, M, C, rpb, mean, rstd, gamma, beta, act, part,
+                           ticket, out);
+        return LAUNCH_CHECK();
+    }
+    hipLaunchKernelGGL(bn_bwd_stage1, dim3(G), dim3(256), 0, st, X, ldx, dY, lddy, M, C, rpb, mean, rstd, gamma, beta, act, part);
+    hipLaunchKernelGGL(bn_bwd_finish_kernel, dim3(cdiv(C, 64)), dim3(64 * S2_L), 0, st, part, G, C, M, mean, rstd, gamma, dgamma, dbeta, coef);
     return LAUNCH_CHECK();
 }
 TATT_API int tatt_bn_bwd_finish(const double* part, int G, int C, int M, const float* mean, const float* rstd, const float* gamma,
diff --git a/tatt_amd/functional.py b/tatt_amd/functional.py
--- a/tatt_amd/functional.py
+++ b/tatt_amd/functional.py
@@ -241,15 +241,42 @@
                                 act)
 
 
+BN_LAST_ARRIVER_BWD = False
+BN_LAST_ARRIVER_FWD = False
+
+
+def _bn_ticket(bn, site, G, ref):
+    if bn is None:
+        return None
+    table = bn.__dict__.setdefault("_tatt_sync", {})
+    key = ("bn_" + site, int(G), ref.device)
+    t = table.get(key)
+    if t is None:
+        t = table[key] = torch.zeros(1, device=ref.device, dtype=torch.int64)
+    return t
+
+
+def _bn_bwd_ticket(bn, x):
+    if not BN_LAST_ARRIVER_BWD or bn is None:
+        return None
+    return _bn_ticket(bn, "bwd", ops.LIB.tatt_bn_bwd_groups(x.numel() // x.shape[-1]), x)
+
+
 class ConvBnFn(Function):
 
     @staticmethod
     def forward(ctx, x, weight, bias, gamma, beta, running_mean, running_var, momentum, eps,
-                in_mean, in_rstd, in_gamma, in_beta, in_scale, in_shift, in_act):
+                in_mean, in_rstd, in_gamma, in_beta, in_scale, in_shift, in_act, bn=None, in_bn=None):
         B, H, W, C = x.shape
-        y, part, G = ops.conv3_bn_forward(x, weight, bias, in_scale, in_shift, in_act, True)
-        mean, rstd, scale, shift = ops.bn_stats_finish(part, G, 64, B * H * W, eps, momentum, gamma, beta, running_mean, running_var)
+        if BN_LAST_ARRIVER_FWD and bn is not None and ops.conv3_bn_la_ok(x):
+            y, mean, rstd, scale, shift = ops.conv3_bn_forward_la(x, weight, bias, in_scale, in_shift, in_act, eps, momentum, gamma, beta,
+                                                                  running_mean, running_var,
+                                                                  _bn_ticket(bn, "fwd", ops._conv3_sb_groups(B, H, W), x))
+        else:
+            y, part, G = ops.conv3_bn_forward(x, weight, bias, in_scale, in_shift, in_act, True)
+            mean, rstd, scale, shift = ops.bn_stats_finish(part, G, 64, B * H * W, eps, momentum, gamma, beta, running_mean, running_var)
         folded = in_scale is not None
+        ctx.in_ticket = _bn_bwd_ticket(in_bn, x) if folded else None
         ctx.save_for_backward(x, weight, in_mean, in_rstd, in_gamma, in_beta)
         ctx.folded, ctx.in_act, ctx.has_bias = folded, in_act, bias is not None
         ctx.leaves = (weight, bias)
@@ -261,7 +288,7 @@
     def backward(ctx, dy, *_):
         x, weight, in_mean, in_rstd, in_gamma, in_beta = ctx.saved_tensors
         if dy is None:
-            return (None,) * 16
+            return (None,) * 18
         dy = _c(dy)
         x2 = x.reshape(-1, 64)
         dx = dgi = dbi = None
@@ -269,7 +296,7 @@
         if ctx.needs_input_grad[0] or need_in:
             dr = ops.conv2d_dgrad(dy, weight)
             if ctx.folded:
-                dx, dgi, dbi = ops.bn_bwd(x2, dr.reshape(-1, 64), in_mean, in_rstd, in_gamma, in_beta, ctx.in_act, True)
+                dx, dgi, dbi = ops.bn_bwd(x2, dr.reshape(-1, 64), in_mean, in_rstd, in_gamma, in_beta, ctx.in_act, True, ctx.in_ticket)
                 dx = dx.reshape(x.shape)
             else:
                 dx = dr
@@ -283,39 +310,42 @@
             db = ops.colsum(dy.reshape(-1, 64)) if want_db else None
             return dw, db
         dw, db = SIDE.submit(ctx.leaves, param_grads, x, dy, in_mean, in_rstd, in_gamma, in_beta, weight)
-        return (dx, dw, db) + (None,) * 8 + (dgi, dbi, None, None, None)
+        return (dx, dw, db) + (None,) * 8 + (dgi, dbi, None, None, None, None, None)
 
 
 class BatchNormApplyFn(Function):
 
     @staticmethod
-    def forward(ctx, x, mean, rstd, gamma, beta, act):
+    def forward(ctx, x, mean, rstd, gamma, beta, act, bn=None):
         C = x.shape[-1]
         y = ops.bn_apply(x.reshape(-1, C), mean, rstd, gamma, beta, act).reshape(x.shape)
         ctx.save_for_backward(x, mean, rstd, gamma, beta)
         ctx.act = act
+        ctx.ticket = _bn_bwd_ticket(bn, x)
         return y
 
     @staticmethod
     def backward(ctx, dy):
         x, mean, rstd, gamma, beta = ctx.saved_tensors
         C = x.shape[-1]
-        dx, dg, db = ops.bn_bwd(x.reshape(-1, C), _c(dy).reshape(-1, C), mean, rstd, gamma, beta, ctx.act, True)
-        return dx.reshape(x.shape), None, None, dg, db, None
+        dx, dg, db = ops.bn_bwd(x.reshape(-1, C), _c(dy).reshape(-1, C), mean, rstd, gamma, beta, ctx.act, True, ctx.ticket)
+        return dx.reshape(x.shape), None, None, dg, db, None, None
 
 
 def conv_bn(x, conv, bn, prev=None):
     if prev is None:
         ins = (None,) * 6 + (ACT_NONE,)
+        pbn = None
     else:
         (pm, pr, ps, psh), pbn, pact = prev
         ins = (pm, pr, pbn.weight, pbn.bias, ps, psh, pact)
-    out = ConvBnFn.apply(x, conv.weight, conv.bias, bn.weight, bn.bias, bn.running_mean, bn.running_var, bn.momentum, bn.eps, *ins)
+    out = ConvBnFn.apply(x, conv.weight, conv.bias, bn.weight, bn.bias, bn.running_mean, bn.running_var, bn.momentum, bn.eps, *ins,
+                         bn, pbn)
     return out[0], tuple(out[1:])
 
 
 def bn_apply_stats(y, stats, bn, act=ACT_NONE):
-    return BatchNormApplyFn.apply(y, stats[0], stats[1], bn.weight, bn.bias, act)
+    return BatchNormApplyFn.apply(y, stats[0], stats[1], bn.weight, bn.bias, act, bn)
 
 
 SRB_BWD_FUSED = False
@@ -324,9 +354,10 @@
 class SrbTrunkFn(Function):
 
     @staticmethod
-    def forward(ctx, x, w1, b1, g1, be1, rm1, rv1, mom1, eps1, w2, b2, g2, be2, rm2, rv2, mom2, eps2):
+    def forward(ctx, x, w1, b1, g1, be1, rm1, rv1, mom1, eps1, w2, b2, g2, be2, rm2, rv2, mom2, eps2, bn2=None):
         B, H, W, C = x.shape
         M = B * H * W
+        ctx.ticket2 = _bn_bwd_ticket(bn2, x)
         y1, part1, G1 = ops.conv3_bn_forward(x, w1, b1, None, None, ACT_NONE, True)
         mean1, rstd1, sc1, sh1 = ops.bn_stats_finish(part1, G1, 64, M, eps1, mom1, g1, be1, rm1, rv1)
         y2, part2, G2 = ops.conv3_bn_forward(y1, w2, b2, sc1, sh1, ACT_MISH, True)
@@ -344,8 +375,11 @@
         M = B * H * W
         d = _c(d)
         y1f, y2f = y1.reshape(M, 64), y2.reshape(M, 64)
-        part2, G2 = ops.bn_bwd_partials(y2f, d.reshape(M, 64), mean2, rstd2, g2, be2, ACT_NONE)
-        dg2, dbe2, coef2 = ops.bn_bwd_finish(part2, G2, 64, M, mean2, rstd2, g2)
+        if ctx.ticket2 is not None:
+            dg2, dbe2, coef2 = ops.bn_bwd_partials_finish(y2f, d.reshape(M, 64), mean2, rstd2, g2, be2, ACT_NONE, ctx.ticket2)
+        else:
+            part2, G2 = ops.bn_bwd_partials(y2f, d.reshape(M, 64), mean2, rstd2, g2, be2, ACT_NONE)
+            dg2, dbe2, coef2 = ops.bn_bwd_finish(part2, G2, 64, M, mean2, rstd2, g2)
         du1, part1, G1 = ops.conv3_dgrad_bn(d, w2, y2, coef2, ep=(y1, mean1, rstd1, g1, be1, ACT_MISH))
         dg1, dbe1, coef1 = ops.bn_bwd_finish(part1, G1, 64, M, mean1, rstd1, g1)
         dx = None
@@ -363,13 +397,13 @@
             dw1, db1 = r1 if want_b1 else (r1, None)
             return dw1, db1, dw2, db2
         dw1, db1, dw2, db2 = SIDE.submit(ctx.leaves, param_grads, x, y1, y2, d, du1, coef1, coef2, mean1, rstd1, g1, be1, w1, w2)
-        return (dx, dw1, db1, dg1, dbe1, None, None, None, None, dw2, db2, dg2, dbe2, None, None, None, None)
+        return (dx, dw1, db1, dg1, dbe1, None, None, None, None, dw2, db2, dg2, dbe2, None, None, None, None, None)
 
 
 def srb_trunk(x, blk):
     c1, n1, c2, n2 = blk.conv1, blk.bn1, blk.conv2, blk.bn2
     return SrbTrunkFn.apply(x, c1.weight, c1.bias, n1.weight, n1.bias, n1.running_mean, n1.running_var, n1.momentum, n1.eps,
-                            c2.weight, c2.bias, n2.weight, n2.bias, n2.running_mean, n2.running_var, n2.momentum, n2.eps)
+                            c2.weight, c2.bias, n2.weight, n2.bias, n2.running_mean, n2.running_var, n2.momentum, n2.eps, n2)
 
 
 class _PackedLinears:
@@ -771,9 +805,10 @@
 
     @staticmethod
     def forward(ctx, x, xb, conv_w, conv_b, wih_f, whh_f, bih_f, bhh_f, wih_r, whh_r, bih_r, bhh_r, vertical,
-                in_mean=None, in_rstd=None, in_gamma=None, in_beta=None, in_add=None):
+                in_mean=None, in_rstd=None, in_gamma=None, in_beta=None, in_add=None, in_bn_mod=None):
         B, H, W, K1 = x.shape
         in_bn = (in_mean, in_rstd, in_gamma, in_beta) if in_mean is not None else None
+        ctx.in_ticket = _bn_bwd_ticket(in_bn_mod, x) if in_bn is not None else None
         Wc = conv_w.reshape(conv_w.shape[0], -1)
         K = Wc.shape[1]
         x2 = x.reshape(-1, K1)
@@ -838,7 +873,7 @@
                 dxb = ops.linear_bwd_input(dgi, Wp, col0=K1, ncols=K - K1).reshape(xb.shape)
         dgam = dbet = dadd = None
         if in_bn is not None and dx is not None:
-            dx, dgam, dbet = ops.bn_bwd(x2, dx.reshape(-1, K1), in_mean, in_rstd, in_gamma, in_beta, ACT_NONE, True)
+            dx, dgam, dbet = ops.bn_bwd(x2, dx.reshape(-1, K1), in_mean, in_rstd, in_gamma, in_beta, ACT_NONE, True, ctx.in_ticket)
             dx = dx.reshape(x.shape)
         elif in_add is not None:
             dadd = dx
@@ -867,7 +902,7 @@
                      ops.P(dwhh_f), ops.P(dwhh_r), ops.stream())
             return (dWc.reshape(ctx.wshape), dbc, dwih_f, dwhh_f, dbp[:96], dbhh[:96], dwih_r, dwhh_r, dbp[96:], dbhh[96:])
         pg = SIDE.submit(ctx.leaves, param_grads, dgi, dgh, hprev, frag, x, xb, Wp, Wc, in_mean, in_rstd, in_gamma, in_beta, in_add)
-        return (dx, dxb) + tuple(pg) + (None, None, None, dgam, dbet, dadd)
+        return (dx, dxb) + tuple(pg) + (None, None, None, dgam, dbet, dadd, None)
 
 
 def _gru_in_foldable(x, xb, blk, vertical, is_sum):
@@ -884,14 +919,15 @@
 def gru_block(x, blk, vertical, xb=None):
     g = blk.gru
     xb = None if xb is None else _c(xb)
-    extra = (None,) * 5
+    extra = (None,) * 6
     if isinstance(x, tuple):
         x0 = _c(x[0])
+        bn = x[5] if len(x) > 5 else None
         if _gru_in_foldable(x0, xb, blk, vertical, len(x) == 2):
-            extra = (x[1], x[2], x[3], x[4], None) if len(x) == 5 else (None, None, None, None, _c(x[1]))
+            extra = (x[1], x[2], x[3], x[4], None, bn) if len(x) >= 5 else (None, None, None, None, _c(x[1]), None)
             x = x0
         else:
-            x = BatchNormApplyFn.apply(x[0], x[1], x[2], x[3], x[4], ACT_NONE) if len(x) == 5 else add(x[0], x[1])
+            x = BatchNormApplyFn.apply(x[0], x[1], x[2], x[3], x[4], ACT_NONE, bn) if len(x) >= 5 else add(x[0], x[1])
     return GruBlockFn.apply(_c(x), xb, blk.conv1.weight, blk.conv1.bias,
                             g.weight_ih_l0, g.weight_hh_l0, g.bias_ih_l0, g.bias_hh_l0,
                             g.weight_ih_l0_reverse, g.weight_hh_l0_reverse, g.bias_ih_l0_reverse, g.bias_hh_l0_reverse,
diff --git a/tatt_amd/ops.py b/tatt_amd/ops.py
--- a/tatt_amd/ops.py
+++ b/tatt_amd/ops.py
@@ -410,7 +410,7 @@
 
 
 def _conv3_sb_groups(nb, H, W):
-    return min(256, nb * H * W // 64)
+    return min(256, nb * (H // 4) * ((W + 15) // 16) if H % 4 == 0 else nb * H * W // 64)
 
 
 def _conv3_sb(x_bhwc, w_oihw, mode, bias, act=ACT_NONE, in_scale=None, in_shift=None, in_act=ACT_NONE, stats=None):
@@ -493,6 +493,29 @@
     call("tatt_conv3_c64_fwd_ws16_bn", P(x_bhwc), P(repack_weight(weight_oihw, 6)), P(bias), P(y), B, H, W, 64, ACT_NONE, 0.0,
          P(in_scale), P(in_shift), int(in_act), P(part), stream())
     return y, part, G
+
+
+def conv3_bn_la_ok(x_bhwc):
+    B, H, W, C = x_bhwc.shape
+    if not (CONV3_SB and CONV3_SB_GENERATION == 4 and C == 64 and x_bhwc.is_contiguous()):
+        return False
+    slices = _conv3_sb_slices(x_bhwc, 64, 64, ACT_NONE)
+    return slices is not None and len(slices) == 1 and LIB.tatt_conv3_sb_route(B, H, W, 64, 64, ACT_NONE, ACT_NONE) == 4
+
+
+def conv3_bn_forward_la(x_bhwc, weight_oihw, bias, in_scale, in_shift, in_act, eps, momentum, gamma, beta, running_mean,
+                        running_var, ticket):
+    _check_dev(x_bhwc)
+    B, H, W, _ = x_bhwc.shape
+    G = _conv3_sb_groups(B, H, W)
+    wl = repack_weight(weight_oihw, LIB.tatt_conv3_sb_packing(B, H, W, 64, 64, ACT_NONE, ACT_NONE))
+    y = new(x_bhwc, B, H, W, 64)
+    part = new(x_bhwc, G * 128, dtype=torch.float64)
+    mean, rstd, scale, shift = new(gamma, 64), new(gamma, 64), new(gamma, 64), new(gamma, 64)
+    call("tatt_conv3_c64_fwd_sb_bn_la", P(x_bhwc), P(wl), P(bias), P(y), B, H, W, P(in_scale), P(in_shift), int(in_act), P(part), G,
+         B * H * W, float(eps), float(momentum), P(gamma), P(beta), P(mean), P(rstd), P(running_mean), P(running_var), P(scale),
+         P(shift), P(ticket), stream())
+    return y, mean, rstd, scale, shift
 
 
 def bn_stats_finish(part, G, C, M, eps, momentum, gamma, beta, running_mean, running_var):
@@ -604,11 +627,15 @@
     return y
 
 
-def bn_bwd(x2, dy2, mean, rstd, gamma, beta, act, training):
+def bn_bwd(x2, dy2, mean, rstd, gamma, beta, act, training, ticket=None):
     M, C = x2.shape
     dx = new(x2, M, C)
     dgamma, dbeta, sums = new(x2, C), new(x2, C), new(x2, 2 * C)
     ws = new(x2, 256 * 2 * C, dtype=torch.float64)
+    if ticket is not None:
+        call("tatt_bn_bwd_la", P(x2), x2.stride(0), P(dy2), dy2.stride(0), P(dx), C, M, C, P(mean), P(rstd), P(gamma), P(beta),
+             act, int(training), P(dgamma), P(dbeta), P(sums), P(ws), P(ticket), stream())
+        return dx, dgamma, dbeta
     call("tatt_bn_bwd", P(x2), x2.stride(0), P(dy2), dy2.stride(0), P(dx), C, M, C, P(mean), P(rstd), P(gamma), P(beta),
          act, int(training), P(dgamma), P(dbeta), P(sums), P(ws), stream())
     return dx, dgamma, dbeta
@@ -626,6 +653,16 @@
 def bn_bwd_finish(part, G, C, M, mean, rstd, gamma):
     dgamma, dbeta, coef = new(gamma, C), new(gamma, C), new(gamma, 3, C)
     call("tatt_bn_bwd_finish", P(part), G, C, M, P(mean), P(rstd), P(gamma), P(dgamma), P(dbeta), P(coef), stream())
+    return dgamma, dbeta, coef
+
+
+def bn_bwd_partials_finish(x2, dy2, mean, rstd, gamma, beta, act, ticket):
+    M, C = x2.shape
+    G = LIB.tatt_bn_bwd_groups(int(M))
+    part = new(x2, G * 2 * C, dtype=torch.float64)
+    dgamma, dbeta, coef = new(gamma, C), new(gamma, C), new(gamma, 3, C)
+    call("tatt_bn_bwd_partials_finish_la", P(x2), x2.stride(0), P(dy2), dy2.stride(0), M, C, P(mean), P(rstd), P(gamma), P(beta),
+         int(act), P(part), P(dgamma), P(dbeta), P(coef), P(ticket), stream())
     return dgamma, dbeta, coef
 
 
diff --git a/tatt_amd/tsrn.py b/tatt_amd/tsrn.py
--- a/tatt_amd/tsrn.py
+++ b/tatt_amd/tsrn.py
@@ -262,7 +262,7 @@
             y1, st1 = Fh.conv_bn(x, blk.conv1, blk.bn1)
             y2, st2 = Fh.conv_bn(y1, blk.conv2, blk.bn2, prev=(st1, blk.bn1, ACT_MISH))
             if Fh.SRB_IN_FOLD:
-                r = Fh.gru_block((y2, st2[0], st2[1], blk.bn2.weight, blk.bn2.bias), blk.gru1, True, xb=tp_map)
+                r = Fh.gru_block((y2, st2[0], st2[1], blk.bn2.weight, blk.bn2.bias, blk.bn2), blk.gru1, True, xb=tp_map)
                 return Fh.gru_block((x_res, r), blk.gru2, False)
             r = Fh.bn_apply_stats(y2, st2, blk.bn2, ACT_NONE)
     else:
```

Result: no change. 11740 (-0.2%).
